# sttts/kcp

Hardware: AMD Instinct MI355X
Metric: object-pair diffs/sec (whole node) + achieved HBM GB/s, 10M objs/100k clusters (higher is better)
Workload: dtype u8; 1 GPU; config3: 10000000 pairs / 100000 logical clusters node-wide, 5% mutated (40% ConfigMap/Secret, 40% Deployment, 20% CRD); pairs_per_rank=10000000, passes_in_flight=2, parallelism=shard-by-logical-cluster x1 (LPT)

## Files before the change

include/gpudiff.h:

```cpp
#ifndef GPUDIFF_H
#define GPUDIFF_H

#include <stddef.h>
#include <stdint.h>

#include "gpudiff_format.h"

#ifdef __cplusplus
extern "C" {
#endif

#define GPUDIFF_ABI_VERSION 6

enum {
    GPUDIFF_OK = 0,
    GPUDIFF_E_INVAL = -1,
    GPUDIFF_E_NOMEM = -2,
    GPUDIFF_E_DEVICE = -3,
    GPUDIFF_E_NODEVICE = -4,
    GPUDIFF_E_CAPACITY = -5,
    GPUDIFF_E_STATE = -6,
    GPUDIFF_E_DECODE = -7,
    GPUDIFF_E_NOTFOUND = -8,
};

#define GPUDIFF_SPEC_DIRTY 0x1u
#define GPUDIFF_STATUS_DIRTY 0x2u
#define GPUDIFF_DECODE_ERROR 0x4u
#define GPUDIFF_SPEC_NOOP 0x8u
#define GPUDIFF_STATUS_NOOP 0x10u

#define GPUDIFF_TOK_OK 0
#define GPUDIFF_TOK_SYNTAX 1
#define GPUDIFF_TOK_NUMBER 2
#define GPUDIFF_TOK_KEY 3
#define GPUDIFF_TOK_STRING 4
#define GPUDIFF_TOK_HASH 5
#define GPUDIFF_TOK_DEPTH 6
#define GPUDIFF_TOK_SIZE 7
#define GPUDIFF_TOK_SPACE 8
#define GPUDIFF_TOK_FLOAT 9
#define GPUDIFF_TOK_WIDE 10
#define GPUDIFF_TOK_FIELD 11
#define GPUDIFF_TOK_LIST 12

#define GPUDIFF_PATH_CHANGED 0u
#define GPUDIFF_PATH_ADDED 1u
#define GPUDIFF_PATH_REMOVED 2u
#define GPUDIFF_PATH_STATUS_ABSENT 3u
#define GPUDIFF_PATH_REGION_STATUS 0x80u

#define GPUDIFF_OPT_TIMING 0x1u
#define GPUDIFF_OPT_K2_ROWS 0x40u
#define GPUDIFF_OPT_ARENA_SHIFT 21u
#define GPUDIFF_OPT_DEVICE_ENCODE 0x2000000u
#define GPUDIFF_OPT_PATH_STRINGS 0x8000000u
#define GPUDIFF_OPT_SMALL_PASS 0x20000000u
#define GPUDIFF_OPT_PATH_VALUES 0x80000000u
#define GPUDIFF_OPT_KNOWN                                                                                         \
    (GPUDIFF_OPT_TIMING | (0xFu << GPUDIFF_OPT_ARENA_SHIFT) | GPUDIFF_OPT_DEVICE_ENCODE | GPUDIFF_OPT_PATH_STRINGS | \
     GPUDIFF_OPT_SMALL_PASS | GPUDIFF_OPT_PATH_VALUES | GPUDIFF_OPT_K2_ROWS)

#define GPUDIFF_SMALL_PASS_MAX_PAIRS 4096u
#define GPUDIFF_SMALL_PASS_MAX_PATHS 32768u

#define GPUDIFF_DEVICE_CURRENT (-1)
#define GPUDIFF_DEVICE_NONE (-2)

typedef struct gpudiff_opts {
    int32_t device;
    uint32_t encode_threads;
    void* stream;
    uint32_t flags;
    uint32_t path_hash_bits;
} gpudiff_opts;

typedef struct gpudiff_json_pair {
    const uint8_t* old_json;
    size_t old_len;
    const uint8_t* new_json;
    size_t new_len;
    uint32_t pair_id;
    uint32_t cluster_id;
} gpudiff_json_pair;

typedef struct gpudiff_ctx gpudiff_ctx;
typedef struct gpudiff_hbatch gpudiff_hbatch;
typedef struct gpudiff_dbatch gpudiff_dbatch;
typedef uint64_t gpudiff_ticket;

typedef struct gpudiff_hbatch_info {
    size_t n_pairs;
    const gpudiff_pair_row* rows;
    const uint8_t* pool;
    uint64_t pool_bytes;
    uint64_t total_leaves;
    uint64_t n_decode_errors;
    uint64_t n_reseeded;
} gpudiff_hbatch_info;

typedef struct gpudiff_result {
    size_t n_pairs;
    const uint8_t* pair_flags;
    size_t n_spec_dirty;
    const uint32_t* spec_dirty_ids;
    size_t n_status_dirty;
    const uint32_t* status_dirty_ids;
    size_t n_dirty;
    const uint32_t* dirty_ids;
    const uint32_t* path_offsets;
    size_t n_paths;
    const uint64_t* path_hashes;
    const uint8_t* path_kinds;
    void* internal_;
} gpudiff_result;

typedef struct gpudiff_path_strings {
    size_t n_paths;
    const uint64_t* offsets;
    const char* bytes;
    size_t n_host;
    size_t n_unresolved;
} gpudiff_path_strings;
int gpudiff_result_path_strings(gpudiff_ctx* ctx, const gpudiff_result* res, gpudiff_path_strings* out);
typedef struct gpudiff_path_stats {
    uint64_t batches;
    uint64_t paths;
    uint64_t bytes;
    uint64_t host_paths;
    double kernel_ms;
    uint64_t timed_batches;
} gpudiff_path_stats;
int gpudiff_path_strings_stats_get(gpudiff_ctx* ctx, gpudiff_path_stats* out);

#define GPUDIFF_VALUE_ABSENT 0xFFu
typedef struct gpudiff_path_values {
    size_t n_paths;
    const uint64_t* offsets;
    const char* bytes;
    const uint8_t* tags;
    size_t n_host;
    size_t n_unresolved;
} gpudiff_path_values;
int gpudiff_result_path_values(gpudiff_ctx* ctx, const gpudiff_result* res, gpudiff_path_values* out);
int gpudiff_path_values_stats_get(gpudiff_ctx* ctx, gpudiff_path_stats* out);
int gpudiff_render_syncs_get(gpudiff_ctx* ctx, uint64_t* out);

typedef struct gpudiff_device_view {
    const uint8_t* pair_flags;
    const uint32_t* spec_dirty_ids;
    const uint32_t* status_dirty_ids;
    const uint32_t* dirty_ids;
    const uint32_t* counts;
} gpudiff_device_view;

typedef struct gpudiff_batch_stats {
    uint64_t n_pairs;
    uint64_t pool_bytes;
    uint64_t total_leaves;
    uint64_t compare_bytes;
    uint64_t value_bytes;
} gpudiff_batch_stats;

typedef struct gpudiff_timings {
    float compare_ms;
    float compact_ms;
    float join_ms;
    float emit_ms;
    float total_ms;
    uint32_t n_passes;
    uint32_t k2_launches;
} gpudiff_timings;

const char* gpudiff_strerror(int err);
int gpudiff_abi_version(void);
const char* gpudiff_build_id(void);
int gpudiff_device_count(int* n);

int gpudiff_open(const gpudiff_opts* opts, gpudiff_ctx** out);
void gpudiff_close(gpudiff_ctx* ctx);

int gpudiff_encode_pairs(gpudiff_ctx* ctx, const gpudiff_json_pair* pairs, size_t n,
                         gpudiff_hbatch** out);
int gpudiff_hbatch_info_get(const gpudiff_hbatch* hb, gpudiff_hbatch_info* info);
int gpudiff_hbatch_create(gpudiff_ctx* ctx, uint64_t pool_bytes, size_t n_pairs, uint64_t total_leaves,
                          gpudiff_hbatch** out, uint8_t** pool, gpudiff_pair_row** rows);
int gpudiff_hbatch_resize(gpudiff_ctx* ctx, gpudiff_hbatch* hb, uint64_t pool_bytes, size_t n_pairs,
                          uint64_t total_leaves, uint8_t** pool, gpudiff_pair_row** rows);
void gpudiff_hbatch_free(gpudiff_ctx* ctx, gpudiff_hbatch* hb);

int gpudiff_dbatch_create(gpudiff_ctx* ctx, uint64_t pool_bytes, uint64_t max_pairs,
                          gpudiff_dbatch** out);
int gpudiff_dbatch_create_view(gpudiff_ctx* ctx, const gpudiff_dbatch* base, gpudiff_dbatch** out);
int gpudiff_dbatch_append(gpudiff_ctx* ctx, gpudiff_dbatch* db, const gpudiff_hbatch* hb);
int gpudiff_dbatch_reset(gpudiff_ctx* ctx, gpudiff_dbatch* db);
int gpudiff_dbatch_stats_get(const gpudiff_dbatch* db, gpudiff_batch_stats* st);
int gpudiff_dbatch_device_view(const gpudiff_dbatch* db, gpudiff_device_view* v);
#define GPUDIFF_EXPORT_COUNTS 0u
#define GPUDIFF_EXPORT_SPEC_IDS 1u
#define GPUDIFF_EXPORT_STATUS_IDS 2u
#define GPUDIFF_EXPORT_DIRTY_IDS 3u
#define GPUDIFF_EXPORT_FLAGS 4u
int gpudiff_dbatch_export(gpudiff_ctx* ctx, const gpudiff_dbatch* db, uint32_t what, void* dst_device,
                          uint64_t max_elems, uint64_t known_count);
int gpudiff_dbatch_bind_gather(gpudiff_ctx* ctx, gpudiff_dbatch* db, void* send_dev, uint32_t cap_spec,
                               uint32_t cap_status);
int gpudiff_dbatch_result_slot(gpudiff_ctx* ctx, gpudiff_dbatch* db, uint32_t slot);
int gpudiff_dbatch_read_pool(gpudiff_ctx* ctx, const gpudiff_dbatch* db, uint64_t off, void* dst,
                             uint64_t bytes);
void gpudiff_dbatch_free(gpudiff_ctx* ctx, gpudiff_dbatch* db);

int gpudiff_cluster_bytes(const gpudiff_pair_row* rows, size_t n, uint32_t n_clusters, uint64_t* out);
int gpudiff_shard_lpt(const uint64_t* weights, uint32_t n_clusters, uint32_t world, int32_t* owner);
int gpudiff_rows_stream_bytes(const gpudiff_pair_row* rows, size_t n, uint64_t* out);
int gpudiff_rows_read_bytes(const gpudiff_pair_row* rows, size_t n, uint64_t* out);

int gpudiff_diff(gpudiff_ctx* ctx, gpudiff_dbatch* db, gpudiff_ticket* ticket);
int gpudiff_wait(gpudiff_ctx* ctx, gpudiff_ticket ticket, gpudiff_result* res);
void gpudiff_result_release(gpudiff_ctx* ctx, gpudiff_result* res);
int gpudiff_last_timings(gpudiff_ctx* ctx, gpudiff_timings* t);
int gpudiff_timing_reset(gpudiff_ctx* ctx);
int gpudiff_sync(gpudiff_ctx* ctx);
typedef struct gpudiff_pass_stats {
    uint64_t passes;
    uint64_t small_passes;
    uint64_t small_redone;
    uint64_t redo_arena, redo_deep, redo_paths;
    uint64_t readback_rounds;
} gpudiff_pass_stats;
int gpudiff_pass_stats_get(gpudiff_ctx* ctx, gpudiff_pass_stats* out);

int gpudiff_submit(gpudiff_ctx* ctx, const gpudiff_json_pair* pairs, size_t n,
                   gpudiff_ticket* ticket);

typedef struct gpudiff_cluster_index {
    size_t n_clusters;
    const uint32_t* cluster_ids;
    const uint32_t* spec_off;
    const uint32_t* status_off;
    size_t n_spec, n_status;
    const uint32_t* spec_ids;
    const uint32_t* status_ids;
    uint32_t sorted_on_device;
    void* internal;
} gpudiff_cluster_index;
int gpudiff_cluster_index_get(gpudiff_ctx* ctx, gpudiff_ticket ticket, gpudiff_cluster_index* out);
void gpudiff_cluster_index_release(gpudiff_ctx* ctx, gpudiff_cluster_index* idx);
int gpudiff_cluster_index_host(const uint8_t* flags, const uint32_t* pair_ids, const uint32_t* cluster_ids, size_t n,
                               gpudiff_cluster_index* out);
typedef struct gpudiff_cluster_index_stats {
    uint64_t calls;
    uint64_t sorted_calls;
    uint64_t syncs;
    uint64_t entries;
    uint64_t d2h_bytes;
    double kernel_ms;
    uint64_t timed_calls;
} gpudiff_cluster_index_stats;
int gpudiff_cluster_index_stats_get(gpudiff_ctx* ctx, gpudiff_cluster_index_stats* out);
int gpudiff_cluster_index_get_final(gpudiff_ctx* ctx, gpudiff_ticket ticket, gpudiff_cluster_index* out);
typedef struct gpudiff_cluster_index_final_stats {
    uint64_t calls;
    uint64_t patched_calls;
    uint64_t compacted_calls;
    uint64_t sorted_calls;
    uint64_t syncs;
    uint64_t entries_in;
    uint64_t entries_live;
    uint64_t patch_rows;
    uint64_t h2d_bytes;
    uint64_t d2h_bytes;
    double kernel_ms;
    uint64_t timed_calls;
} gpudiff_cluster_index_final_stats;
int gpudiff_cluster_index_final_stats_get(gpudiff_ctx* ctx, gpudiff_cluster_index_final_stats* out);

typedef struct gpudiff_store gpudiff_store;

typedef struct gpudiff_event {
    uint32_t slot;
    uint32_t pair_id;
    uint32_t cluster_id;
    uint32_t reserved;
    const uint8_t* new_json;
    size_t new_len;
    const uint8_t* old_json;
    size_t old_len;
} gpudiff_event;

typedef struct gpudiff_store_stats {
    uint64_t max_slots, live_slots;
    uint64_t space_bytes;
    uint64_t used_bytes;
    uint64_t live_bytes;
    uint64_t compactions;
    uint64_t events, old_encoded, reseeded, collisions_unresolved;
    uint64_t last_batch_bytes;
    uint64_t deferred;
// ... 246 lines not shown
```

include/gpudiff_format.h:

```cpp
#ifndef GPUDIFF_FORMAT_H
#define GPUDIFF_FORMAT_H

#include <stdint.h>

#ifdef __HIPCC__
#define GPUDIFF_HD __host__ __device__
#else
#define GPUDIFF_HD
#endif

#define GPUDIFF_TAG_NULL 0u
#define GPUDIFF_TAG_FALSE 1u
#define GPUDIFF_TAG_TRUE 2u
#define GPUDIFF_TAG_INT 3u
#define GPUDIFF_TAG_FLOAT 4u
#define GPUDIFF_TAG_STR 5u
#define GPUDIFF_TAG_EOBJ 6u
#define GPUDIFF_TAG_EARR 7u

#define GPUDIFF_INLINE_MAX 8u
#define GPUDIFF_PATH_HASH_BITS 32u

#define GPUDIFF_OBJ_HAS_STATUS 0x1u
#define GPUDIFF_OBJ_DECODE_ERR 0x2u
#define GPUDIFF_OBJ_FRESH 0x4u
#define GPUDIFF_OBJ_SPEC_KEYS_EQ 0x8u
#define GPUDIFF_OBJ_SPEC_SHAPE_EQ 0x10u
#define GPUDIFF_TAB_INDEX 0x8000000000000000ull
#define GPUDIFF_TAB_NONE 0xFFFFFFFFu
GPUDIFF_HD static inline uint64_t gpudiff_tab_bytes(uint32_t n, uint64_t key_bytes) {
    return (24ull * n + key_bytes + 127u) & ~(uint64_t)127u;
}

#define GPUDIFF_OBJ_SEED_SHIFT 8u

#ifdef __cplusplus
extern "C" {
#endif

typedef struct gpudiff_pair_row {
    uint64_t off_a;
    uint64_t off_b;
    uint32_t spec_l_a, spec_l_b;
    uint32_t spec_ar_a, spec_ar_b;
    uint32_t stat_l_a, stat_l_b;
    uint32_t stat_ar_a, stat_ar_b;
    uint32_t flags_a, flags_b;
    uint32_t pair_id, cluster_id;
} gpudiff_pair_row;

GPUDIFF_HD static inline uint64_t gpudiff_seg_bytes(uint32_t l, uint32_t arena) {
    return (uint64_t)l * 16u + (uint64_t)arena;
}

#define GPUDIFF_BLOB_ALIGN 128u
GPUDIFF_HD static inline uint64_t gpudiff_blob_body(uint32_t sl, uint32_t sar, uint32_t tl, uint32_t tar) {
    return (gpudiff_seg_bytes(sl, sar) + gpudiff_seg_bytes(tl, tar) + (GPUDIFF_BLOB_ALIGN - 1u)) &
           ~(uint64_t)(GPUDIFF_BLOB_ALIGN - 1u);
}

#ifndef GPUDIFF_KEYS_HOLE_UNIT
#define GPUDIFF_KEYS_HOLE_UNIT 128u
#endif
GPUDIFF_HD static inline void gpudiff_keys_hole(uint32_t l, uint32_t* hs, uint32_t* hl) {
    const uint64_t u = GPUDIFF_KEYS_HOLE_UNIT;
    const uint64_t lo = (8ull * l + (u - 1u)) / u * u, hi = 12ull * l / u * u;
    *hs = hi > lo ? (uint32_t)(lo >> 4) : 0u;
    *hl = hi > lo ? (uint32_t)((hi - lo) >> 4) : 0u;
}
GPUDIFF_HD static inline void gpudiff_shape_hole(uint32_t l, uint32_t* hs, uint32_t* hl) {
    const uint64_t u = GPUDIFF_KEYS_HOLE_UNIT;
    const uint64_t lo = (8ull * l + (u - 1u)) / u * u, hi = 16ull * l / u * u;
    *hs = hi > lo ? (uint32_t)(lo >> 4) : 0u;
    *hl = hi > lo ? (uint32_t)((hi - lo) >> 4) : 0u;
}
GPUDIFF_HD static inline uint32_t gpudiff_hole_chunk(uint32_t k, uint32_t hs, uint32_t hl) {
    return k + (k >= hs ? hl : 0u);
}

GPUDIFF_HD static inline uint64_t gpudiff_pair_compare_bytes(const gpudiff_pair_row* r) {
    const uint64_t al = GPUDIFF_BLOB_ALIGN - 1u;
    uint64_t per = 0;
    if ((r->flags_a | r->flags_b) & GPUDIFF_OBJ_DECODE_ERR) return sizeof(gpudiff_pair_row) + 1u;
    {
        const int spec_sz = r->spec_l_a == r->spec_l_b && r->spec_ar_a == r->spec_ar_b;
        const int stat_sz = (r->flags_b & GPUDIFF_OBJ_HAS_STATUS) && r->stat_l_a == r->stat_l_b &&
                            r->stat_ar_a == r->stat_ar_b;
        const uint64_t seg_s = gpudiff_seg_bytes(r->spec_l_a, r->spec_ar_a);
        const uint64_t seg_t = gpudiff_seg_bytes(r->stat_l_a, r->stat_ar_a);
        if (spec_sz && stat_sz) per = (seg_s + seg_t + al) & ~al;
        else if (spec_sz) per = (r->stat_l_a | r->stat_l_b | r->stat_ar_a | r->stat_ar_b) ? seg_s : (seg_s + al) & ~al;
        else if (stat_sz) per = seg_t;
    }
    return sizeof(gpudiff_pair_row) + 1u + 2u * per;
}

#define GPUDIFF_PD_ERR 0x01u
#define GPUDIFF_PD_SPEC_EQ 0x02u
#define GPUDIFF_PD_STAT_EQ 0x04u
#define GPUDIFF_PD_HAS_ST_B 0x08u
#define GPUDIFF_PD_HAS_ST_A 0x10u
#define GPUDIFF_PD_SEED 0x20u
#define GPUDIFF_PD_NO_STAT 0x40u
#define GPUDIFF_PD_SIZE_BITS 19u
#define GPUDIFF_PD_SIZE_MAX 0x7FFFFu
#define GPUDIFF_PD_ESCAPE 0xFFFFFFFFu
#define GPUDIFF_PD_SHAPE_L 0x40000u

typedef struct gpudiff_pair_desc {
    uint32_t w[4];
} gpudiff_pair_desc;

typedef struct gpudiff_pair_geom {
    uint64_t off_a, off_b;
    uint32_t n1, n2, adj_a, adj_b;
    uint32_t bits;
    uint32_t hs, hl;
} gpudiff_pair_geom;

GPUDIFF_HD static inline gpudiff_pair_geom gpudiff_pair_geom_of(uint64_t off_a, uint64_t off_b, uint32_t seg_a,
                                                                uint32_t seg_b, uint32_t seg_t, uint32_t bits,
                                                                uint32_t skip_l, int shape) {
    gpudiff_pair_geom g;
    const int ok = !(bits & GPUDIFF_PD_ERR);
    const int spec_sz = (bits & GPUDIFF_PD_SPEC_EQ) != 0u;
    const int stat_sz = (bits & GPUDIFF_PD_HAS_ST_B) && (bits & GPUDIFF_PD_STAT_EQ);
    const uint32_t r128 = (seg_a + seg_t + 127u) & ~127u;
    g.off_a = off_a;
    g.off_b = off_b;
    g.n1 = (ok && spec_sz) ? ((!stat_sz && (bits & GPUDIFF_PD_NO_STAT)) ? ((seg_a + 127u) & ~127u) : seg_a) >> 4 : 0u;
    g.n2 = (ok && stat_sz) ? (spec_sz ? r128 - seg_a : seg_t) >> 4 : 0u;
    g.hs = g.hl = 0u;
    if (skip_l && (uint64_t)skip_l * (shape ? 16u : 12u) <= 16ull * g.n1) {
        if (shape) gpudiff_shape_hole(skip_l, &g.hs, &g.hl);
        else gpudiff_keys_hole(skip_l, &g.hs, &g.hl);
        g.n1 -= g.hl;
    }
    g.adj_a = seg_a - 16u * g.n1;
    g.adj_b = seg_b - 16u * g.n1;
    g.bits = bits;
    return g;
}

GPUDIFF_HD static inline uint32_t gpudiff_pair_row_bits(const gpudiff_pair_row* r) {
    return (((r->flags_a | r->flags_b) & GPUDIFF_OBJ_DECODE_ERR) ? GPUDIFF_PD_ERR : 0u) |
           ((r->spec_l_a == r->spec_l_b && r->spec_ar_a == r->spec_ar_b) ? GPUDIFF_PD_SPEC_EQ : 0u) |
           ((r->stat_l_a == r->stat_l_b && r->stat_ar_a == r->stat_ar_b) ? GPUDIFF_PD_STAT_EQ : 0u) |
           ((r->flags_b & GPUDIFF_OBJ_HAS_STATUS) ? GPUDIFF_PD_HAS_ST_B : 0u) |
           ((r->flags_a & GPUDIFF_OBJ_HAS_STATUS) ? GPUDIFF_PD_HAS_ST_A : 0u) |
           (((r->flags_a >> GPUDIFF_OBJ_SEED_SHIFT) & 0xFFu) ? GPUDIFF_PD_SEED : 0u) |
           ((r->stat_l_a | r->stat_l_b | r->stat_ar_a | r->stat_ar_b) == 0u ? GPUDIFF_PD_NO_STAT : 0u);
}

GPUDIFF_HD static inline gpudiff_pair_geom gpudiff_pair_row_geom(const gpudiff_pair_row* r) {
    return gpudiff_pair_geom_of(r->off_a, r->off_b, (uint32_t)gpudiff_seg_bytes(r->spec_l_a, r->spec_ar_a),
                                (uint32_t)gpudiff_seg_bytes(r->spec_l_b, r->spec_ar_b),
                                (uint32_t)gpudiff_seg_bytes(r->stat_l_a, r->stat_ar_a), gpudiff_pair_row_bits(r), 0u, 0);
}

GPUDIFF_HD static inline gpudiff_pair_desc gpudiff_pair_desc_pack(const gpudiff_pair_row* r) {
    gpudiff_pair_desc d;
    const uint64_t sa = gpudiff_seg_bytes(r->spec_l_a, r->spec_ar_a), sb = gpudiff_seg_bytes(r->spec_l_b, r->spec_ar_b);
    const uint64_t st = gpudiff_seg_bytes(r->stat_l_a, r->stat_ar_a);
    const uint32_t bits = gpudiff_pair_row_bits(r);
    const uint64_t size_max = (uint64_t)GPUDIFF_PD_SIZE_MAX << 4;
    const int fits = ((r->off_a | r->off_b) & (GPUDIFF_BLOB_ALIGN - 1u)) == 0u && (r->off_a >> 7) <= 0xFFFFFFFFull &&
                     (r->off_b >> 7) <= 0xFFFFFFFFull && ((sa | sb | st) & 15u) == 0u && sa <= size_max &&
                     sb <= size_max && st <= size_max &&
                     ((uint32_t)(r->stat_l_a + r->stat_l_b) == 0u) == ((bits & GPUDIFF_PD_NO_STAT) != 0u);
    if (!fits) {
        d.w[0] = d.w[1] = d.w[2] = d.w[3] = GPUDIFF_PD_ESCAPE;
        return d;
    }
    {
        uint64_t f1 = sb >> 4;
        if (bits & GPUDIFF_PD_SPEC_EQ) {
            uint32_t hs = 0, hl = 0;
            const int keys = (r->flags_b & GPUDIFF_OBJ_SPEC_KEYS_EQ) && !(bits & GPUDIFF_PD_ERR);
            f1 = 0u;
            if (keys && (r->flags_b & GPUDIFF_OBJ_SPEC_SHAPE_EQ) && (sa >> 4) < GPUDIFF_PD_SHAPE_L) {
                gpudiff_shape_hole(r->spec_l_a, &hs, &hl);
                if (hl) f1 = r->spec_l_a | GPUDIFF_PD_SHAPE_L;
            }
            if (keys && !f1) {
                gpudiff_keys_hole(r->spec_l_a, &hs, &hl);
                f1 = hl ? r->spec_l_a : 0u;
            }
        }
        const uint64_t zw = (sa >> 4) | (f1 << GPUDIFF_PD_SIZE_BITS) | ((st >> 4) << (2u * GPUDIFF_PD_SIZE_BITS)) |
                            ((uint64_t)bits << (3u * GPUDIFF_PD_SIZE_BITS));
        d.w[0] = (uint32_t)(r->off_a >> 7);
        d.w[1] = (uint32_t)(r->off_b >> 7);
        d.w[2] = (uint32_t)zw;
        d.w[3] = (uint32_t)(zw >> 32);
    }
    return d;
}

GPUDIFF_HD static inline int gpudiff_pair_desc_is_escape(uint32_t w3) { return w3 == GPUDIFF_PD_ESCAPE; }

GPUDIFF_HD static inline gpudiff_pair_geom gpudiff_pair_desc_unpack(uint32_t w0, uint32_t w1, uint32_t w2, uint32_t w3) {
    const uint64_t zw = ((uint64_t)w3 << 32) | w2;
    const uint32_t bits = w3 >> (3u * GPUDIFF_PD_SIZE_BITS - 32u);
    const uint32_t seg_a = (w2 & GPUDIFF_PD_SIZE_MAX) << 4;
    const uint32_t f1 = (uint32_t)(zw >> GPUDIFF_PD_SIZE_BITS) & GPUDIFF_PD_SIZE_MAX;
    const int eq = (bits & GPUDIFF_PD_SPEC_EQ) != 0u;
    const int shape = eq && f1 >= GPUDIFF_PD_SHAPE_L && (w2 & GPUDIFF_PD_SIZE_MAX) < GPUDIFF_PD_SHAPE_L;
    return gpudiff_pair_geom_of((uint64_t)w0 << 7, (uint64_t)w1 << 7, seg_a, eq ? seg_a : f1 << 4,
                                ((w3 >> (2u * GPUDIFF_PD_SIZE_BITS - 32u)) & GPUDIFF_PD_SIZE_MAX) << 4, bits,
                                eq ? (shape ? f1 & (GPUDIFF_PD_SHAPE_L - 1u) : f1) : 0u, shape);
}

GPUDIFF_HD static inline uint64_t gpudiff_pair_stream_bytes(const gpudiff_pair_row* r) {
    const gpudiff_pair_desc d = gpudiff_pair_desc_pack(r);
    const gpudiff_pair_geom g = gpudiff_pair_desc_is_escape(d.w[3]) ? gpudiff_pair_row_geom(r)
                                                                   : gpudiff_pair_desc_unpack(d.w[0], d.w[1], d.w[2], d.w[3]);
    return sizeof(gpudiff_pair_desc) + 32ull * ((uint64_t)g.n1 + g.n2);
}

GPUDIFF_HD static inline uint32_t gpudiff_meta(uint32_t tag, uint32_t len) { return (len << 3) | tag; }
GPUDIFF_HD static inline uint32_t gpudiff_meta_tag(uint32_t m) { return m & 7u; }
GPUDIFF_HD static inline uint32_t gpudiff_meta_len(uint32_t m) { return m >> 3; }
GPUDIFF_HD static inline int gpudiff_meta_is_long(uint32_t m) {
    return gpudiff_meta_tag(m) == GPUDIFF_TAG_STR && gpudiff_meta_len(m) > GPUDIFF_INLINE_MAX;
}
GPUDIFF_HD static inline uint32_t gpudiff_meta_arena(uint32_t m) {
    return gpudiff_meta_is_long(m) ? ((gpudiff_meta_len(m) - GPUDIFF_INLINE_MAX + 3u) & ~3u) : 0u;
}
GPUDIFF_HD static inline uint32_t gpudiff_arena_bytes(uint32_t sum) { return (sum + 15u) & ~15u; }

#ifdef __cplusplus
}
#endif
#endif
```

integration/go/gpudiff/gpudiff.go:

```go
package gpudiff

import "C"

import (
	"bytes"
	"encoding/json"
	"errors"
	"fmt"
	"math"
	"sort"
	"strconv"
	"sync"
	"time"
	"unicode/utf8"
	"unsafe"

	"k8s.io/apimachinery/pkg/apis/meta/v1/unstructured"
)

type Engine struct {
	mu     sync.Mutex
	ctx    *C.gpudiff_ctx
	devEnc bool
}
// ... 809 lines not shown
	lp := (*[1 << 30]C.size_t)(lens)[:n:n]
	for i, o := range objs {
		dp[i], lp[i] = nil, 0
		if b, ok := jsonOf(o); ok {
			dp[i], lp[i] = cmem(b)
		}
	}
	defer func() {
		for i := range dp {
			C.free(unsafe.Pointer(dp[i]))
		}
	}()
	e.mu.Lock()
	defer e.mu.Unlock()
	var out C.gpudiff_bodies
	if err := errOf(C.gpudiff_upsert_bodies(e.ctx, (**C.uint8_t)(docs), (*C.size_t)(lens), C.size_t(n),
		C.uint32_t(mode), &out)); err != nil {
		return nil, nil, nil, err
	}
	defer C.gpudiff_bodies_release(e.ctx, &out)
	var rv C.gpudiff_rv_splice
	if err := errOf(C.gpudiff_bodies_rv_splice(e.ctx, &out, &rv)); err != nil {
		return nil, nil, nil, err
	}
	offs := (*[1 << 30]C.uint64_t)(unsafe.Pointer(out.offsets))[: n+1 : n+1]
	st := (*[1 << 30]C.int32_t)(unsafe.Pointer(out.status))[:n:n]
	res := make([][]byte, n)
	rvOff, rvForm = make([]uint32, n), make([]uint8, n)
	ro := (*[1 << 30]C.uint32_t)(unsafe.Pointer(rv.off))[:n:n]
	rf := (*[1 << 30]C.uint8_t)(unsafe.Pointer(rv.form))[:n:n]
	for i := 0; i < n; i++ {
		if lp[i] == 0 || st[i] != 0 {
			continue
		}
		res[i] = C.GoBytes(unsafe.Pointer(uintptr(unsafe.Pointer(out.bytes))+uintptr(offs[i])),
			C.int(offs[i+1]-offs[i]))
		rvOff[i], rvForm[i] = uint32(ro[i]), uint8(rf[i])
	}
	return res, rvOff, rvForm, nil
}

const (
	RVNone   = uint8(C.GPUDIFF_RV_NONE)
	RVInsert = uint8(C.GPUDIFF_RV_INSERT)
	RVLead   = uint8(C.GPUDIFF_RV_LEAD)
	RVTrail  = uint8(C.GPUDIFF_RV_TRAIL)
	RVWrap   = uint8(C.GPUDIFF_RV_WRAP)
)

func SpliceRV(body []byte, off uint32, form uint8, rv string) []byte {
	if rv == "" || form&RVInsert == 0 || off == 0 || int(off) >= len(body) {
		return body
	}
	val, err := json.Marshal(rv)
	if err != nil {
		return body
	}
	out := make([]byte, 0, len(body)+len(val)+40)
	out = append(out, body[:off]...)
	if form&RVLead != 0 {
		out = append(out, ',')
	}
	if form&RVWrap != 0 {
		out = append(out, `"metadata":{`...)
	}
	out = append(out, `"resourceVersion":`...)
	out = append(out, val...)
	if form&RVWrap != 0 {
		out = append(out, '}')
	}
	if form&RVTrail != 0 {
		out = append(out, ',')
	}
	return append(out, body[off:]...)
}

const OptDeviceEncode = uint32(C.GPUDIFF_OPT_DEVICE_ENCODE)

const OptSmallPass = uint32(C.GPUDIFF_OPT_SMALL_PASS)

const (
	ObjSpecKeysEq  = uint32(C.GPUDIFF_OBJ_SPEC_KEYS_EQ)
	ObjSpecShapeEq = uint32(C.GPUDIFF_OBJ_SPEC_SHAPE_EQ)
)

func RowsReadBytes(rows unsafe.Pointer, n int) (uint64, error) {
	var out C.uint64_t
	if err := errOf(C.gpudiff_rows_read_bytes((*C.gpudiff_pair_row)(rows), C.size_t(n), &out)); err != nil {
		return 0, err
	}
	return uint64(out), nil
}

type Write struct {
	Pair int
	Kind Mode
	Noop bool
	Body []byte
	RVOff  uint32
	RVForm uint8
	Name      string
	Namespace string
}

const (
	PlanInformer           = uint32(C.GPUDIFF_PLAN_INFORMER)
	PlanSpec               = uint32(C.GPUDIFF_PLAN_SPEC)
	PlanStatus             = uint32(C.GPUDIFF_PLAN_STATUS)
	PlanUpstreamDownstream = uint32(C.GPUDIFF_PLAN_UPSTREAM_DOWNSTREAM)
	PlanTargets            = uint32(C.GPUDIFF_PLAN_TARGETS)
)

func (e *Engine) DiffAndPlan(olds, news [][]byte) ([]uint8, []Write, error) {
	return e.DiffAndPlanMode(olds, news, PlanInformer)
}

func (e *Engine) DiffAndPlanMode(olds, news [][]byte, mode uint32) ([]uint8, []Write, error) {
	n := len(olds)
	if len(news) != n {
		return nil, nil, errOf(C.GPUDIFF_E_INVAL)
	}
	if n == 0 {
		return nil, nil, nil
	}
	pairs := (*[1 << 28]C.gpudiff_json_pair)(C.malloc(C.size_t(n) * C.size_t(unsafe.Sizeof(C.gpudiff_json_pair{}))))[:n:n]
	defer C.free(unsafe.Pointer(&pairs[0]))
	for i := range olds {
		pa, la := cmem(olds[i])
		pb, lb := cmem(news[i])
		pairs[i] = C.gpudiff_json_pair{old_json: pa, old_len: la, new_json: pb, new_len: lb, pair_id: C.uint32_t(i)}
	}
	defer func() {
		for i := range pairs {
			C.free(unsafe.Pointer(pairs[i].old_json))
			C.free(unsafe.Pointer(pairs[i].new_json))
		}
	}()
	e.mu.Lock()
	defer e.mu.Unlock()
	var ticket C.gpudiff_ticket
	if err := errOf(C.gpudiff_submit(e.ctx, &pairs[0], C.size_t(n), &ticket)); err != nil {
		return nil, nil, err
	}
	var res C.gpudiff_result
	if err := errOf(C.gpudiff_wait(e.ctx, ticket, &res)); err != nil {
		return nil, nil, err
	}
	flags := make([]uint8, n)
	copy(flags, (*[1 << 30]uint8)(unsafe.Pointer(res.pair_flags))[:n:n])
	C.gpudiff_result_release(e.ctx, &res)
	var plan C.gpudiff_write_plan
	if err := errOf(C.gpudiff_write_plan_get_ex(e.ctx, ticket, C.uint32_t(mode), &plan)); err != nil {
		return flags, nil, err
	}
	defer C.gpudiff_write_plan_release(e.ctx, &plan)
	return flags, writesOf(&plan), nil
}

func writesOf(plan *C.gpudiff_write_plan) []Write {
	m := int(plan.n)
	writes := make([]Write, m)
	if m == 0 {
		return writes
	}
	idx := (*[1 << 30]C.uint32_t)(unsafe.Pointer(plan.pair_index))[:m:m]
	kind := (*[1 << 30]C.uint8_t)(unsafe.Pointer(plan.kind))[:m:m]
	noop := (*[1 << 30]C.uint8_t)(unsafe.Pointer(plan.noop))[:m:m]
// ... 215 lines not shown
```

kcp_amd/csrc/api.cpp:

```cpp
#include <hip/hip_runtime.h>
#include <stdlib.h>
#include <string.h>

#include <algorithm>
#include <array>
#include <atomic>
#include <memory>
#include <mutex>
#include <new>
#include <string>
#include <thread>
#include <unordered_map>
#include <vector>

#include "../../include/gpudiff.h"
#include "encoder.h"
#include "dstore.h"
#include "engine.h"
#include "kernels.h"
#include "small_pass.h"
#include "xxh64.h"

using namespace gd;

namespace gd {
thread_local std::string g_last_hip_error;
}
using gd::g_last_hip_error;

static int ensure_paths(gpudiff_dbatch* d, uint64_t arena, uint64_t scratch) {
    const bool ok_a = arena <= d->arena_cap && d->arena_h;
    const bool ok_s = scratch <= d->scratch_cap && d->scratch_h;
    if (ok_a && ok_s) return GPUDIFF_OK;
    auto drop = [](auto*& p) {
        if (p) (void)hipFree(p);
        p = nullptr;
    };
    drop(d->out_h);
    drop(d->out_k);
    int rc;
    if (!ok_a) {
        drop(d->arena_h);
        drop(d->arena_k);
        d->arena_cap = 0;
        if ((rc = dalloc(&d->arena_h, arena)) || (rc = dalloc(&d->arena_k, arena))) return rc;
        d->arena_cap = arena;
    }
    if (!ok_s) {
        if (scratch > kMaxScratchEntries) return GPUDIFF_E_CAPACITY;
        scratch = std::min<uint64_t>(std::max<uint64_t>({scratch + scratch / 8, d->scratch_cap, 1u << 16}),
                                     kMaxScratchEntries);
        scratch = (scratch + kJoinSliceHost - 1) / kJoinSliceHost * kJoinSliceHost;
        drop(d->scratch_h);
        drop(d->scratch_k);
        drop(d->slot_owner);
        drop(d->slice_cnt);
        drop(d->slice_weq);
        d->scratch_cap = 0;
        const uint64_t slots = scratch / kJoinSliceHost;
        if ((rc = dalloc(&d->scratch_h, scratch)) || (rc = dalloc(&d->scratch_k, scratch)) ||
            (rc = dalloc(&d->slot_owner, slots)) || (rc = dalloc(&d->slice_cnt, slots)) ||
            (rc = dalloc(&d->slice_weq, slots)))
            return rc;
        d->scratch_cap = scratch;
    }
    const uint64_t out = d->arena_cap + d->scratch_cap;
    if ((rc = dalloc(&d->out_h, out)) || (rc = dalloc(&d->out_k, out))) return rc;
    return GPUDIFF_OK;
}

static DiffBuffers buffers_of(gpudiff_ctx* c, gpudiff_dbatch* d) {
    DiffBuffers b;
    b.rows = d->rows;
    b.desc = (d->desc_gen == d->rows_gen && !(c->flags & GPUDIFF_OPT_K2_ROWS)) ? d->desc : nullptr;
    b.pool = d->pool;
    b.pair_ids = d->pair_ids;
    b.n_pairs = (uint32_t)d->n_pairs;
    b.flags = d->flags;
    b.caps = d->caps;
    b.chunk_counts = d->chunk_counts;
    b.summary = d->summary;
    b.spec_ids = d->spec_ids;
    b.status_ids = d->status_ids;
    b.dirty_ids = d->dirty_ids;
    b.dirty_idx = d->dirty_idx;
    b.scratch_off = d->scratch_off;
    b.path_count = d->path_count;
    b.path_off = d->path_off;
    b.tile_sums = d->tile_sums;
    b.path_src = d->path_src;
    b.path_cnt = d->path_cnt;
    b.nbits = d->nbits;
    b.noop_d = d->noop_d;
    b.arena_h = d->arena_h;
    b.arena_k = d->arena_k;
    b.arena_per_wave = kArenaPerWave >> ((c->flags >> GPUDIFF_OPT_ARENA_SHIFT) & 0xFu);
    b.scratch_h = d->scratch_h;
    b.scratch_k = d->scratch_k;
    b.scratch_cap = d->scratch_cap;
    b.out_h = d->out_h;
    b.out_k = d->out_k;
    b.slot_owner = d->slot_owner;
    b.slice_cnt = d->slice_cnt;
    b.slice_weq = d->slice_weq;
    b.hash_mask = c->hash_mask;
    b.k2_timeline = c->k2_timeline ? 1u : 0u;
    b.k2_shared = 0u;
    b.tail_perm = d->tail_perm;
    b.tail_perm_key = &d->tail_perm_key;
    b.rows_gen = d->rows_gen;
    b.gather_send = d->gather_send;
    b.gather_cap_spec = d->gather_cap_spec;
    b.gather_cap_status = d->gather_cap_status;
    b.avg_pair_bytes = d->n_pairs ? (d->compare_bytes ? d->compare_bytes : d->size_hint_bytes) / d->n_pairs : 0;
    return b;
}


extern "C" {

const char* gpudiff_strerror(int err) {
    switch (err) {
        case GPUDIFF_OK: return "ok";
        case GPUDIFF_E_INVAL: return "invalid argument";
        case GPUDIFF_E_NOMEM: return "out of host memory";
        case GPUDIFF_E_DEVICE: return g_last_hip_error.empty() ? "HIP runtime error" : g_last_hip_error.c_str();
        case GPUDIFF_E_NODEVICE: return "no GPU in this context (there is no CPU fallback)";
        case GPUDIFF_E_CAPACITY: return "device batch capacity exceeded";
        case GPUDIFF_E_STATE: return "invalid call order / unknown ticket";
        case GPUDIFF_E_DECODE: return "input failed to decode as a JSON object";
        case GPUDIFF_E_NOTFOUND: return "path hash not found";
        default: return "unknown error";
    }
}

int gpudiff_abi_version(void) { return GPUDIFF_ABI_VERSION; }

int gpudiff_device_count(int* n) {
    if (!n) return GPUDIFF_E_INVAL;
    *n = 0;
    int c = 0;
    if (hipGetDeviceCount(&c) != hipSuccess) return GPUDIFF_OK;
    *n = c;
    return GPUDIFF_OK;
}

int gpudiff_open(const gpudiff_opts* opts, gpudiff_ctx** out) {
    if (!out) return GPUDIFF_E_INVAL;
    *out = nullptr;
    gpudiff_opts o{};
    o.device = GPUDIFF_DEVICE_CURRENT;
    if (opts) o = *opts;
    if (o.flags & ~GPUDIFF_OPT_KNOWN) return GPUDIFF_E_INVAL;
    std::unique_ptr<gpudiff_ctx> c(new (std::nothrow) gpudiff_ctx());
    if (!c) return GPUDIFF_E_NOMEM;
    uint32_t hw = std::max(1u, std::thread::hardware_concurrency());
    c->threads = o.encode_threads ? o.encode_threads : std::min(hw, 16u);
    c->flags = o.flags;
// ... 182 lines not shown
int gpudiff_hbatch_info_get(const gpudiff_hbatch* hb, gpudiff_hbatch_info* info) {
    if (!hb || !info) return GPUDIFF_E_INVAL;
    info->n_pairs = hb->n;
    info->rows = hb->rows;
    info->pool = hb->pool;
    info->pool_bytes = hb->pool_bytes;
    info->total_leaves = hb->leaves;
    info->n_decode_errors = hb->errors;
    info->n_reseeded = hb->reseeded;
    return GPUDIFF_OK;
}

void gpudiff_hbatch_free(gpudiff_ctx* c, gpudiff_hbatch* hb) {
    if (!hb) return;
    if (c && c->has_device) (void)hipSetDevice(c->device);
    if (hb->used) {
        (void)hipEventSynchronize(hb->used);
        (void)hipEventDestroy(hb->used);
    }
    hb_release_buffers(hb);
    delete hb;
}

static int alloc_outputs(gpudiff_dbatch* d);

int gpudiff_dbatch_create(gpudiff_ctx* c, uint64_t pool_bytes, uint64_t max_pairs, gpudiff_dbatch** out) {
    if (!c || !out) return GPUDIFF_E_INVAL;
    *out = nullptr;
    int rc = set_device(c);
    if (rc) return rc;
    if (max_pairs > 0xFFFFFFF0ull) return GPUDIFF_E_INVAL;
    std::unique_ptr<gpudiff_dbatch> d(new (std::nothrow) gpudiff_dbatch());
    if (!d) return GPUDIFF_E_NOMEM;
    d->pool_cap = (pool_bytes + 15) & ~15ull;
    d->max_pairs = max_pairs;
    d->device = c->device;
    const uint64_t np = std::max<uint64_t>(max_pairs, 1);
    if ((rc = dalloc(&d->pool, d->pool_cap)) || (rc = dalloc(&d->rows, np)) || (rc = dalloc(&d->pair_ids, np)) ||
        (rc = dalloc(&d->desc, np)) || (rc = alloc_outputs(d.get()))) {
        dfree_all(d.get());
        return rc;
    }
    *out = d.release();
    return GPUDIFF_OK;
}

int gpudiff_dbatch_create_view(gpudiff_ctx* c, const gpudiff_dbatch* base, gpudiff_dbatch** out) {
    if (!c || !base || !out || base->base) return GPUDIFF_E_INVAL;
    *out = nullptr;
    int rc = set_device(c);
    if (rc) return rc;
    if (base->device != c->device) return GPUDIFF_E_INVAL;
    std::unique_ptr<gpudiff_dbatch> d(new (std::nothrow) gpudiff_dbatch());
    if (!d) return GPUDIFF_E_NOMEM;
    d->base = base;
    d->pool_borrowed = true;
    d->max_pairs = base->max_pairs;
    d->device = c->device;
    if ((rc = alloc_outputs(d.get()))) {
        dfree_all(d.get());
        return rc;
    }
    base->views.push_back(d.get());
    *out = d.release();
    return GPUDIFF_OK;
}

static void view_sync(gpudiff_dbatch* d) {
    if (!d->base) return;
    const gpudiff_dbatch* b = d->base;
    d->pool = b->pool;
    d->pool_cap = b->pool_cap;
    d->pool_used = b->pool_used;
    d->rows = b->rows;
    d->pair_ids = b->pair_ids;
    d->n_pairs = b->n_pairs;
    d->leaves = b->leaves;
    d->compare_bytes = b->compare_bytes;
    d->value_bytes = b->value_bytes;
    d->size_hint_bytes = b->size_hint_bytes;
    d->rows_gen = b->rows_gen;
    d->desc = b->desc;
    d->desc_gen = b->desc_gen;
}

static int alloc_outputs(gpudiff_dbatch* d) {
    int rc;
    const uint64_t np = std::max<uint64_t>(d->max_pairs, 1);
    const uint64_t nchunks = (np + 63) / 64;
    const uint64_t ntiles = 4 * (np / 4096 + 2);
    uint4* cc = nullptr;
    if ((rc = dalloc(&d->flags, np)) || (rc = dalloc(&d->caps, np)) || (rc = dalloc(&cc, nchunks)) ||
        (rc = dalloc(&d->summary, kSummaryWords)) || (rc = dalloc(&d->spec_ids, np)) || (rc = dalloc(&d->status_ids, np)) ||
        (rc = dalloc(&d->dirty_ids, np)) || (rc = dalloc(&d->dirty_idx, np)) || (rc = dalloc(&d->scratch_off, np)) ||
        (rc = dalloc(&d->path_count, np)) || (rc = dalloc(&d->path_off, np + 1)) ||
        (rc = dalloc(&d->path_src, np)) || (rc = dalloc(&d->path_cnt, np)) || (rc = dalloc(&d->nbits, np)) ||
        (rc = dalloc(&d->noop_d, np)) ||
        (rc = dalloc(&d->tile_sums, ntiles)) ||
        (rc = dalloc(&d->tail_perm, 16384))) {
        d->chunk_counts = cc;
        return rc;
    }
    d->chunk_counts = cc;
    if (hipEventCreateWithFlags(&d->done, hipEventDisableTiming) != hipSuccess) return GPUDIFF_E_DEVICE;
    return GPUDIFF_OK;
}

int gpudiff_dbatch_append(gpudiff_ctx* c, gpudiff_dbatch* d, const gpudiff_hbatch* hb) {
    if (!c || !d || !hb || d->base) return GPUDIFF_E_INVAL;
    int rc = set_device(c);
    if (rc) return rc;
    if (d->pool_used + hb->pool_bytes > d->pool_cap || d->n_pairs + hb->n > d->max_pairs) return GPUDIFF_E_CAPACITY;
    if (hb->n == 0) return GPUDIFF_OK;
    const uint64_t base = d->pool_used;
    const uint32_t begin = (uint32_t)d->n_pairs, end = (uint32_t)(d->n_pairs + hb->n);
    if (hb->pool_bytes)
        HIPCHK(hipMemcpyAsync(d->pool + base, hb->pool, hb->pool_bytes, hipMemcpyHostToDevice, c->stream));
    HIPCHK(hipMemcpyAsync(d->rows + begin, hb->rows, hb->n * sizeof(gpudiff_pair_row), hipMemcpyHostToDevice,
                          c->stream));
    if (hb->used) HIPCHK(hipEventRecord(hb->used, c->stream));
    HIPCHK(launch_rebase(c->stream, d->rows, begin, end, base, d->pair_ids, d->desc));
    uint64_t cb = 0, vb = 0;
    for (size_t i = 0; i < hb->n; i++) {
        const gpudiff_pair_row& r = hb->rows[i];
        cb += pair_compare_bytes(r);
        if ((r.flags_a | r.flags_b) & GPUDIFF_OBJ_DECODE_ERR) continue;
        vb += blob_value_bytes(hb->pool + r.off_a, r.spec_l_a, r.spec_ar_a, r.stat_l_a) +
              blob_value_bytes(hb->pool + r.off_b, r.spec_l_b, r.spec_ar_b, r.stat_l_b);
    }
    d->compare_bytes += cb;
    d->value_bytes += vb;
    d->pool_used += hb->pool_bytes;
    d->n_pairs = end;
    const bool desc_current = begin == 0 || d->desc_gen == d->rows_gen;
    d->rows_gen++;
    d->desc_gen = desc_current ? d->rows_gen : ~0ull;
    d->leaves += hb->leaves;
    return GPUDIFF_OK;
}

int gpudiff_dbatch_reset(gpudiff_ctx* c, gpudiff_dbatch* d) {
    if (!c || !d || d->base) return GPUDIFF_E_INVAL;
    int rc = set_device(c);
    if (rc) return rc;
    HIPCHK(hipStreamSynchronize(c->stream));
    d->pool_used = d->n_pairs = d->leaves = d->compare_bytes = d->value_bytes = d->size_hint_bytes = 0;
    d->ticket = 0;
    d->rows_gen++;
    return GPUDIFF_OK;
}

int gpudiff_dbatch_stats_get(const gpudiff_dbatch* d, gpudiff_batch_stats* st) {
    if (!d || !st) return GPUDIFF_E_INVAL;
    if (d->base) d = d->base;
    st->n_pairs = d->n_pairs;
    st->pool_bytes = d->pool_used;
    st->total_leaves = d->leaves;
    st->compare_bytes = d->compare_bytes;
    st->value_bytes = d->value_bytes;
    return GPUDIFF_OK;
}

int gpudiff_dbatch_device_view(const gpudiff_dbatch* d, gpudiff_device_view* v) {
    if (!d || !v) return GPUDIFF_E_INVAL;
    v->pair_flags = d->flags;
    v->spec_dirty_ids = d->spec_ids;
    v->status_dirty_ids = d->status_ids;
    v->dirty_ids = d->dirty_ids;
    v->counts = d->summary;
    return GPUDIFF_OK;
}

int gpudiff_dbatch_export(gpudiff_ctx* c, const gpudiff_dbatch* d, uint32_t what, void* dst, uint64_t max_elems,
                          uint64_t known_count) {
    if (!c || !d || (!dst && max_elems)) return GPUDIFF_E_INVAL;
    int rc = set_device(c);
    if (rc) return rc;
    const void* src;
    size_t esz = 4;
    uint64_t n = std::min<uint64_t>(max_elems, known_count);
    switch (what) {
        case GPUDIFF_EXPORT_COUNTS: src = d->summary; n = std::min<uint64_t>(max_elems, 8); break;
        case GPUDIFF_EXPORT_SPEC_IDS: src = d->spec_ids; break;
        case GPUDIFF_EXPORT_STATUS_IDS: src = d->status_ids; break;
        case GPUDIFF_EXPORT_DIRTY_IDS: src = d->dirty_ids; break;
        case GPUDIFF_EXPORT_FLAGS: src = d->flags; esz = 1; break;
        default: return GPUDIFF_E_INVAL;
    }
    if (what != GPUDIFF_EXPORT_COUNTS && n > d->n_pairs) n = d->n_pairs;
    if (n) HIPCHK(hipMemcpyAsync(dst, src, n * esz, hipMemcpyDeviceToDevice, c->stream));
    return GPUDIFF_OK;
}

int gpudiff_dbatch_bind_gather(gpudiff_ctx* c, gpudiff_dbatch* d, void* send_dev, uint32_t cap_spec,
                               uint32_t cap_status) {
    if (!c || !d) return GPUDIFF_E_INVAL;
    int rc = set_device(c);
    if (rc) return rc;
    const bool fresh = send_dev && send_dev != (void*)d->gather_send;
    d->gather_send = (uint32_t*)send_dev;
    d->gather_cap_spec = send_dev ? cap_spec : 0;
    d->gather_cap_status = send_dev ? cap_status : 0;
    if (fresh) HIPCHK(hipMemsetAsync((uint32_t*)send_dev + 4, 0, 4 * sizeof(uint32_t), c->stream));
    return GPUDIFF_OK;
}

int gpudiff_dbatch_result_slot(gpudiff_ctx* c, gpudiff_dbatch* d, uint32_t slot) {
    if (!c || !d || slot > 1) return GPUDIFF_E_INVAL;
    int rc = set_device(c);
    if (rc) return rc;
    if (slot == d->res_slot) return GPUDIFF_OK;
    if (!d->summary_alt) {
        const uint64_t np = std::max<uint64_t>(d->max_pairs, 1);
        uint32_t *a = nullptr, *b = nullptr, *sm = nullptr;
        if ((rc = dalloc(&a, np)) || (rc = dalloc(&b, np)) || (rc = dalloc(&sm, kSummaryWords))) {
            for (uint32_t* p : {a, b, sm})
                if (p) (void)hipFree(p);
            return rc;
        }
        if (hipMemset(sm, 0, kSummaryWords * sizeof(uint32_t)) != hipSuccess) {
            for (uint32_t* p : {a, b, sm}) (void)hipFree(p);
            return GPUDIFF_E_DEVICE;
        }
        d->ids_alt[0] = a, d->ids_alt[1] = b, d->summary_alt = sm;
    }
    std::swap(d->spec_ids, d->ids_alt[0]);
    std::swap(d->status_ids, d->ids_alt[1]);
    std::swap(d->summary, d->summary_alt);
    d->res_slot = slot;
    return GPUDIFF_OK;
}

int gpudiff_dbatch_read_pool(gpudiff_ctx* c, const gpudiff_dbatch* d, uint64_t off, void* dst, uint64_t bytes) {
    if (!c || !d || (!dst && bytes)) return GPUDIFF_E_INVAL;
    if (d->base) d = d->base;
    int rc = set_device(c);
    if (rc) return rc;
    if (off > d->pool_used || bytes > d->pool_used - off) return GPUDIFF_E_INVAL;
    HIPCHK(hipStreamSynchronize(c->stream));
    if (bytes) HIPCHK(hipMemcpy(dst, d->pool + off, bytes, hipMemcpyDeviceToHost));
    return GPUDIFF_OK;
}

int gpudiff_cluster_bytes(const gpudiff_pair_row* rows, size_t n, uint32_t n_clusters, uint64_t* out) {
    if ((n && !rows) || (n_clusters && !out)) return GPUDIFF_E_INVAL;
    for (size_t i = 0; i < n; i++)
        if (rows[i].cluster_id >= n_clusters) return GPUDIFF_E_INVAL;
    for (size_t i = 0; i < n; i++) out[rows[i].cluster_id] += gpudiff_pair_compare_bytes(&rows[i]);
    return GPUDIFF_OK;
}

int gpudiff_rows_stream_bytes(const gpudiff_pair_row* rows, size_t n, uint64_t* out) {
    if ((n && !rows) || !out) return GPUDIFF_E_INVAL;
    uint64_t sum = 0;
    for (size_t i = 0; i < n; i++) {
        gpudiff_pair_row r = rows[i];
        r.flags_b &= ~GPUDIFF_OBJ_SPEC_SHAPE_EQ;
        sum += gpudiff_pair_stream_bytes(&r);
    }
    *out = sum;
    return GPUDIFF_OK;
}

int gpudiff_rows_read_bytes(const gpudiff_pair_row* rows, size_t n, uint64_t* out) {
    if ((n && !rows) || !out) return GPUDIFF_E_INVAL;
    uint64_t sum = 0;
    for (size_t i = 0; i < n; i++) sum += gpudiff_pair_stream_bytes(&rows[i]);
    *out = sum;
    return GPUDIFF_OK;
}

int gpudiff_shard_lpt(const uint64_t* weights, uint32_t n_clusters, uint32_t world, int32_t* owner) {
    if (world == 0 || world > 0x7FFFFFFFu || (n_clusters && (!weights || !owner))) return GPUDIFF_E_INVAL;
    try {
        std::vector<uint32_t> order(n_clusters);
        for (uint32_t c = 0; c < n_clusters; c++) order[c] = c;
        std::sort(order.begin(), order.end(), [&](uint32_t x, uint32_t y) {
            return weights[x] != weights[y] ? weights[x] > weights[y] : x < y;
        });
        std::vector<std::pair<uint64_t, uint32_t>> heap;
        heap.reserve(world);
        for (uint32_t r = 0; r < world; r++) heap.emplace_back(0, r);
        auto gt = [](const std::pair<uint64_t, uint32_t>& a, const std::pair<uint64_t, uint32_t>& b) { return a > b; };
        std::make_heap(heap.begin(), heap.end(), gt);
        for (uint32_t c : order) {
            std::pop_heap(heap.begin(), heap.end(), gt);
            auto& top = heap.back();
            owner[c] = (int32_t)top.second;
            top.first += weights[c];
            std::push_heap(heap.begin(), heap.end(), gt);
        }
    } catch (const std::bad_alloc&) {
        return GPUDIFF_E_NOMEM;
    }
    return GPUDIFF_OK;
}

void gpudiff_dbatch_free(gpudiff_ctx* c, gpudiff_dbatch* d) {
    if (!d) return;
    if (d->base) {
        auto& v = d->base->views;
        v.erase(std::remove(v.begin(), v.end(), d), v.end());
    }
    if (c && c->has_device) {
        (void)hipSetDevice(c->device);
        (void)hipStreamSynchronize(c->stream);
        if (d->ticket) c->tickets.erase(d->ticket);
    }
    dfree_all(d);
    delete d;
}

static hipEvent_t* pass_events(gpudiff_ctx* c) {
    if (c->n_pass >= c->pass_ev.size()) {
        std::array<hipEvent_t, 5> a{};
        for (auto& e : a)
            if (hipEventCreate(&e) != hipSuccess) return nullptr;
        c->pass_ev.push_back(a);
    }
    return c->pass_ev[c->n_pass].data();
}

static int enqueue_join_emit(gpudiff_ctx* c, gpudiff_dbatch* d) {
    DiffBuffers b = buffers_of(c, d);
    const uint32_t nchunks = (uint32_t)((d->n_pairs + 63) / 64);
    HIPCHK(launch_slot_owners(c->stream, b));
    HIPCHK(launch_join(c->stream, b, 0, nchunks, nullptr, (const uint4*)d->summary));
    HIPCHK(launch_emit(c->stream, b));
    return GPUDIFF_OK;
}

static int enqueue_ordinary_pass(gpudiff_ctx* c, gpudiff_dbatch* d, const DiffBuffers& b, hipEvent_t* ev) {
    hipStream_t ms = c->stream;
    uint4* total = (uint4*)d->summary;
    const uint32_t nchunks = (uint32_t)((d->n_pairs + 63) / 64);
    HIPCHK(launch_compare(ms, b));
    if (ev) HIPCHK(hipEventRecord(ev[1], ms));
    HIPCHK(launch_compact(ms, b, 0, nchunks, nullptr, total));
    if (ev) HIPCHK(hipEventRecord(ev[2], ms));
    HIPCHK(launch_join(ms, b, 0, nchunks, nullptr, total));
    if (ev) HIPCHK(hipEventRecord(ev[3], ms));
    HIPCHK(launch_emit(ms, b));
// ... 293 lines not shown
    (void)c;
    if (!res || !out) return GPUDIFF_E_INVAL;
    memset(out, 0, sizeof(*out));
    const ResultStore* rs = (const ResultStore*)res->internal_;
    if (!rs || !rs->ps.on) return GPUDIFF_E_STATE;
    out->n_paths = rs->ps.n;
    out->offsets = rs->ps.offsets();
    out->bytes = rs->ps.bytes();
    out->n_host = rs->ps.n_host;
    out->n_unresolved = rs->ps.n_unresolved;
    return GPUDIFF_OK;
}

int gpudiff_path_strings_stats_get(gpudiff_ctx* c, gpudiff_path_stats* out) {
    if (!c || !out) return GPUDIFF_E_INVAL;
    if (!(c->flags & GPUDIFF_OPT_PATH_STRINGS)) return GPUDIFF_E_STATE;
    *out = c->path_stats;
    return GPUDIFF_OK;
}

int gpudiff_result_path_values(gpudiff_ctx* c, const gpudiff_result* res, gpudiff_path_values* out) {
    (void)c;
    if (!res || !out) return GPUDIFF_E_INVAL;
    memset(out, 0, sizeof(*out));
    const ResultStore* rs = (const ResultStore*)res->internal_;
    if (!rs || !rs->pv.on) return GPUDIFF_E_STATE;
    out->n_paths = rs->pv.n;
    out->offsets = rs->pv.offsets();
    out->bytes = rs->pv.bytes();
    out->tags = rs->pv.tags();
    out->n_host = rs->pv.n_host;
    out->n_unresolved = rs->pv.n_unresolved;
    return GPUDIFF_OK;
}

int gpudiff_path_values_stats_get(gpudiff_ctx* c, gpudiff_path_stats* out) {
    if (!c || !out) return GPUDIFF_E_INVAL;
    *out = c->value_stats;
    return GPUDIFF_OK;
}

int gpudiff_render_syncs_get(gpudiff_ctx* c, uint64_t* out) {
    if (!c || !out) return GPUDIFF_E_INVAL;
    *out = c->render_syncs;
    return GPUDIFF_OK;
}

void gpudiff_result_release(gpudiff_ctx* c, gpudiff_result* res) {
    (void)c;
    if (!res) return;
    delete (ResultStore*)res->internal_;
    memset(res, 0, sizeof(*res));
}

int gpudiff_submit(gpudiff_ctx* c, const gpudiff_json_pair* pairs, size_t n, gpudiff_ticket* ticket) {
    if (!c || (n && !pairs)) return GPUDIFF_E_INVAL;
    int rc = set_device(c);
    if (rc) return rc;
    if ((c->flags & GPUDIFF_OPT_DEVICE_ENCODE) && n) {
        rc = dstore_submit_pairs(c, pairs, n, ticket);
        if (rc != GPUDIFF_E_CAPACITY) return rc;
    }
    gpudiff_hbatch* hb = nullptr;
    if ((rc = gpudiff_encode_pairs(c, pairs, n, &hb))) return rc;
    const uint32_t slot = c->ring_next;
    c->ring_next ^= 1u;
    gpudiff_dbatch*& d = c->ring[slot];
    if (d) HIPCHK(hipEventSynchronize(d->done));
    if (c->ring_hb[slot]) {
        gpudiff_hbatch_free(c, c->ring_hb[slot]);
        c->ring_hb[slot] = nullptr;
    }
    if (d && (d->pool_cap < hb->pool_bytes || d->max_pairs < n)) {
        gpudiff_dbatch_free(c, d);
        d = nullptr;
    }
    if (!d) {
        uint64_t pool = std::max<uint64_t>(hb->pool_bytes * 2, 1u << 20);
        uint64_t np = std::max<uint64_t>(n * 2, 1024);
        if ((rc = gpudiff_dbatch_create(c, pool, np, &d))) {
            gpudiff_hbatch_free(c, hb);
            return rc;
        }
    }
    d->pool_used = d->n_pairs = d->leaves = d->compare_bytes = d->value_bytes = d->size_hint_bytes = 0;
    if ((rc = gpudiff_dbatch_append(c, d, hb)) || (rc = gpudiff_diff(c, d, ticket))) {
        gpudiff_hbatch_free(c, hb);
        return rc;
    }
    c->ring_hb[slot] = hb;
    return GPUDIFF_OK;
}

static int single_pair(gpudiff_ctx* c, const uint8_t* a, size_t al, const uint8_t* b, size_t bl, uint32_t bit,
                       int* equal) {
    if (!c || !equal || !a || !b) return GPUDIFF_E_INVAL;
    gpudiff_json_pair p{a, al, b, bl, 0, 0};
    gpudiff_ticket t = 0;
    int rc = gpudiff_submit(c, &p, 1, &t);
    if (rc) return rc;
    gpudiff_result r;
    if ((rc = gpudiff_wait(c, t, &r))) return rc;
    const uint8_t f = r.pair_flags[0];
    gpudiff_result_release(c, &r);
    *equal = (f & bit) ? 0 : 1;
    return (f & GPUDIFF_DECODE_ERROR) ? GPUDIFF_E_DECODE : GPUDIFF_OK;
}

int gpudiff_spec_equal(gpudiff_ctx* c, const uint8_t* a, size_t al, const uint8_t* b, size_t bl, int* equal) {
    return single_pair(c, a, al, b, bl, GPUDIFF_SPEC_DIRTY, equal);
}

int gpudiff_status_equal(gpudiff_ctx* c, const uint8_t* a, size_t al, const uint8_t* b, size_t bl, int* equal) {
    return single_pair(c, a, al, b, bl, GPUDIFF_STATUS_DIRTY, equal);
}

int gpudiff_resolve_path(const uint8_t* a, size_t al, const uint8_t* b, size_t bl, uint64_t h, uint8_t kind,
                         uint32_t bits, char* buf, size_t cap, size_t* out_len) {
    if (!a || !b) return GPUDIFF_E_INVAL;
    EncodeConfig cfg;
    cfg.hash_bits = (bits == 0 || bits >= GPUDIFF_PATH_HASH_BITS) ? GPUDIFF_PATH_HASH_BITS : bits;
    PairEncoder enc(cfg);
    std::vector<uint8_t> pool;
    gpudiff_pair_row row;
    enc.encode_json(a, al, b, bl, 0, 0, pool, row);
    if (row.flags_a & GPUDIFF_OBJ_DECODE_ERR) return GPUDIFF_E_DECODE;
    std::string s;
    bool found = false;
    const bool status = (kind & GPUDIFF_PATH_REGION_STATUS) != 0;
    if ((kind & 3u) != GPUDIFF_PATH_STATUS_ABSENT) {
        for (const FlatObject* o : {&enc.flat_a, &enc.flat_b}) {
            const std::vector<LeafRec>& v = status ? o->stat : o->spec;
            auto it = std::lower_bound(v.begin(), v.end(), h, [](const LeafRec& r, uint64_t x) { return r.h < x; });
            if (it != v.end() && it->h == h) {
                s = render_path(o->paths.data() + it->path_off, it->path_len);
                found = true;
                break;
            }
        }
    } else {
        const uint64_t mask = cfg.hash_bits >= 64 ? ~0ULL : ((1ULL << cfg.hash_bits) - 1);
        const uint32_t seed = (row.flags_a >> GPUDIFF_OBJ_SEED_SHIFT) & 0xFF;
        const std::string& sp = status_path_bytes();
        if ((chain_hash(sp.data(), sp.size(), seed) & mask) == h) {
            s = "status";
            found = true;
        }
    }
    if (!found) return GPUDIFF_E_NOTFOUND;
    if (out_len) *out_len = s.size();
    if (buf && cap) {
        size_t k = std::min(cap - 1, s.size());
        memcpy(buf, s.data(), k);
        buf[k] = 0;
    }
    return GPUDIFF_OK;
}

}
```

kcp_amd/csrc/encoder.cpp:

```cpp
#include "encoder.h"

#include <string.h>

#include <algorithm>

#include "xxh64.h"

namespace gd {

static const Node* find_member(const Node& obj, const char* key, uint32_t klen) {
    if (obj.t != J_OBJ) return nullptr;
    for (uint32_t i = 0; i < obj.n; i++) {
        const Member& m = obj.u.mem[i];
        if (m.klen == klen && memcmp(m.k, key, klen) == 0) return &m.v;
    }
    return nullptr;
}

static inline void push_key(std::string& p, const char* k, uint32_t n) {
    char hdr[5];
    hdr[0] = 0x01;
    memcpy(hdr + 1, &n, 4);
    p.append(hdr, 5);
    p.append(k, n);
// ... 183 lines not shown
    const uint64_t hs = chain_hash(sp.data(), sp.size(), seed) & mask;
    return sentinel_check(a, a.stat, hs) && sentinel_check(b, b.stat, hs);
}

bool PairEncoder::assign_seed(FlatObject& a, FlatObject& b, uint32_t* seed_out) {
    for (uint32_t seed = 0; seed <= 255; seed++)
        if (pair_valid(a, b, seed)) {
            *seed_out = seed;
            return true;
        }
    return false;
}

static inline void pool_align(std::vector<uint8_t>& pool) {
    size_t n = (pool.size() + GPUDIFF_BLOB_ALIGN - 1) & ~(size_t)(GPUDIFF_BLOB_ALIGN - 1);
    pool.resize(n, 0);
}

void PairEncoder::write_blob(const FlatObject& o, std::vector<uint8_t>& pool, uint64_t* off, uint32_t* sl,
                             uint32_t* sar, uint32_t* tl, uint32_t* tar) {
    pool_align(pool);
    *off = pool.size();
    auto seg = [&](const std::vector<LeafRec>& v, uint32_t* L, uint32_t* AR) {
        const size_t n = v.size();
        uint32_t arena = 0;
        for (const LeafRec& r : v)
            arena += gpudiff_meta_arena(r.meta);
        arena = gpudiff_arena_bytes(arena);
        const size_t head = n * 16;
        const size_t base = pool.size();
        pool.resize(base + head + arena, 0);
        uint8_t* p = pool.data() + base;
        uint8_t* vals = p;
        uint8_t* keys = p + 8 * n;
        uint8_t* metas = p + 12 * n;
        uint8_t* ar = p + head;
        uint32_t aoff = 0;
        for (size_t i = 0; i < n; i++) {
            const LeafRec& r = v[i];
            uint64_t val = r.val;
            if (gpudiff_meta_is_long(r.meta)) {
                memcpy(&val, r.vptr, GPUDIFF_INLINE_MAX);
                memcpy(ar + aoff, r.vptr + GPUDIFF_INLINE_MAX, r.vlen - GPUDIFF_INLINE_MAX);
                aoff += gpudiff_meta_arena(r.meta);
            }
            const uint32_t k32 = (uint32_t)r.h;
            memcpy(keys + 4 * i, &k32, 4);
            memcpy(vals + 8 * i, &val, 8);
            memcpy(metas + 4 * i, &r.meta, 4);
        }
        *L = (uint32_t)n;
        *AR = arena;
        leaves_written += n;
    };
    seg(o.spec, sl, sar);
    seg(o.stat, tl, tar);
    pool_align(pool);
}

void PairEncoder::encode_flat(FlatObject* fa, FlatObject* fb, uint32_t pair_id, uint32_t cluster_id,
                              std::vector<uint8_t>& pool, gpudiff_pair_row& row) {
    memset(&row, 0, sizeof(row));
    row.pair_id = pair_id;
    row.cluster_id = cluster_id;
    uint32_t seed = 0;
    if (!fa || !fb || !assign_seed(*fa, *fb, &seed)) {
        decode_errors++;
        pool_align(pool);
        row.off_a = row.off_b = pool.size();
        row.flags_a = row.flags_b = GPUDIFF_OBJ_DECODE_ERR;
        return;
    }
    if (seed) reseeded++;
    write_blob(*fa, pool, &row.off_a, &row.spec_l_a, &row.spec_ar_a, &row.stat_l_a, &row.stat_ar_a);
    write_blob(*fb, pool, &row.off_b, &row.spec_l_b, &row.spec_ar_b, &row.stat_l_b, &row.stat_ar_b);
    row.flags_a = fa->flags | (seed << GPUDIFF_OBJ_SEED_SHIFT);
    row.flags_b = fb->flags | (seed << GPUDIFF_OBJ_SEED_SHIFT);
    bool keys_eq = fa->spec.size() == fb->spec.size();
    for (size_t i = 0; keys_eq && i < fa->spec.size(); i++) keys_eq = (uint32_t)fa->spec[i].h == (uint32_t)fb->spec[i].h;
    if (keys_eq) row.flags_b |= GPUDIFF_OBJ_SPEC_KEYS_EQ;
    bool shape_eq = keys_eq;
    for (size_t i = 0; shape_eq && i < fa->spec.size(); i++) shape_eq = fa->spec[i].meta == fb->spec[i].meta;
    if (shape_eq) row.flags_b |= GPUDIFF_OBJ_SPEC_SHAPE_EQ;
}

void PairEncoder::encode_nodes(const Node* a, const Node* b, uint32_t pair_id, uint32_t cluster_id,
                               std::vector<uint8_t>& pool, gpudiff_pair_row& row) {
    FlatObject* fa = nullptr;
    FlatObject* fb = nullptr;
    if (a && b) {
        flatten_object(*a, flat_a);
        flatten_object(*b, flat_b);
        fa = &flat_a;
        fb = &flat_b;
    }
    encode_flat(fa, fb, pair_id, cluster_id, pool, row);
}

void PairEncoder::encode_json(const uint8_t* a, size_t alen, const uint8_t* b, size_t blen, uint32_t pair_id,
                              uint32_t cluster_id, std::vector<uint8_t>& pool, gpudiff_pair_row& row) {
    arena_a.reset();
    arena_b.reset();
    Node na, nb;
    bool oka = a && parser.parse_object(a, alen, arena_a, &na) && !decodes_as_list(na);
    bool okb = oka && b && parser.parse_object(b, blen, arena_b, &nb) && !decodes_as_list(nb);
    encode_nodes(oka ? &na : nullptr, okb ? &nb : nullptr, pair_id, cluster_id, pool, row);
}


bool PairEncoder::flatten_json(const uint8_t* json, size_t len, Arena& arena, FlatObject& o) {
    arena.reset();
    Node n;
    if (!json || !parser.parse_object(json, len, arena, &n) || decodes_as_list(n)) return false;
    flatten_object(n, o);
    return true;
}

bool PairEncoder::path_table(FlatObject& o, uint32_t seed) {
    using PN = TabNode;
    const uint64_t mask = cfg_.hash_bits >= 64 ? ~0ULL : ((1ULL << cfg_.hash_bits) - 1);
    const uint64_t root = (uint64_t)seed & mask;
    std::vector<PN>& v = tab_scratch_;
    v.clear();
    const char* P = o.paths.data();
    for (const std::vector<LeafRec>* lv : {&o.spec, &o.stat})
        for (const LeafRec& r : *lv) {
            uint64_t hp = seed;
            uint32_t i = 0;
            while (i + 5 <= r.path_len) {
                const char* c = P + r.path_off + i;
                uint32_t x;
                memcpy(&x, c + 1, 4);
                const bool key = c[0] == 0x01;
                const uint32_t len = key ? 5u + x : 5u;
                const uint64_t h = xxh64_host(c, len, hp);
                PN n;
                n.h = h & mask;
                n.ph = hp & mask;
                n.c = key ? ((uint64_t)x << 32) : (GPUDIFF_TAB_INDEX | x);
                n.poff = r.path_off;
                n.pend = r.path_off + i + len;
                n.koff = r.path_off + i + 5;
                if (n.h == root) {
                    o.tab.n = GPUDIFF_TAB_NONE;
                    o.tab.data.clear();
                    return false;
                }
                v.push_back(n);
                hp = h;
                i += len;
            }
        }
    std::sort(v.begin(), v.end(), [](const PN& a, const PN& b) { return a.h < b.h; });
    size_t u = 0, kb = 0;
    for (size_t i = 0; i < v.size(); i++) {
        if (u && v[u - 1].h == v[i].h) {
            const PN& a = v[u - 1];
            const PN& b = v[i];
            if (a.pend - a.poff != b.pend - b.poff || memcmp(P + a.poff, P + b.poff, a.pend - a.poff) != 0) {
                o.tab.n = GPUDIFF_TAB_NONE;
                o.tab.data.clear();
                return false;
            }
            continue;
        }
        v[u++] = v[i];
// ... 169 lines not shown
```

kcp_amd/csrc/engine.h:

```cpp
#pragma once
#include <hip/hip_runtime.h>
#include <string.h>

#include <algorithm>
#include <array>
#include <functional>
#include <memory>
#include <string>
#include <unordered_map>
#include <vector>

#include "../../include/gpudiff.h"
#include "encoder.h"
#include "pool.h"
#include "kernels.h"

using gd::PairEncoder;
using gd::EncodeConfig;

namespace gd {
extern thread_local std::string g_last_hip_error;
}

#define HIPCHK(x)                                             \
// ... 11 lines not shown
    std::vector<gpudiff_pair_row> rows;
    uint64_t leaves = 0, errors = 0, reseeded = 0;
};
}

inline constexpr uint32_t kArenaPerWave = 16384;

struct gpudiff_hbatch {
    uint8_t* pool = nullptr;
    gpudiff_pair_row* rows = nullptr;
    size_t n = 0;
    uint64_t pool_bytes = 0;
    uint64_t leaves = 0, errors = 0, reseeded = 0;
    uint64_t pool_cap = 0;
    size_t rows_cap = 0;
    bool pinned = false;
    hipEvent_t used = nullptr;
};

struct WaitedMark {
    gpudiff_ticket ticket = 0;
    uint32_t n_spec = 0, n_status = 0, n_dirty = 0;
    uint32_t n_dev_dirty = 0;
};
namespace gd {
struct PlanPatch;
}
struct FanBuffers;
void fan_buffers_release(FanBuffers* f);
struct FanCtx;
void fan_ctx_release(FanCtx* f);

struct gpudiff_dbatch {
    uint64_t pool_cap = 0, pool_used = 0;
    uint64_t max_pairs = 0, n_pairs = 0;
    uint64_t leaves = 0, compare_bytes = 0, value_bytes = 0;
    uint64_t size_hint_bytes = 0;
    uint8_t* pool = nullptr;
    bool pool_borrowed = false;
    gpudiff_pair_row* rows = nullptr;
    uint32_t* pair_ids = nullptr;
    uint8_t* flags = nullptr;
    uint32_t* caps = nullptr;
    void* chunk_counts = nullptr;
    uint32_t* summary = nullptr;
    uint32_t* spec_ids = nullptr;
    uint32_t* status_ids = nullptr;
    uint32_t* dirty_ids = nullptr;
    uint32_t* dirty_idx = nullptr;
    uint32_t* scratch_off = nullptr;
    uint32_t* path_count = nullptr;
    uint32_t* path_off = nullptr;
    uint32_t* tile_sums = nullptr;
    uint32_t* path_src = nullptr;
    uint32_t* path_cnt = nullptr;
    uint8_t* nbits = nullptr;
    uint8_t* noop_d = nullptr;
    uint64_t arena_cap = 0;
    uint64_t* arena_h = nullptr;
    uint8_t* arena_k = nullptr;
    uint64_t scratch_cap = 0;
    uint64_t* scratch_h = nullptr;
    uint8_t* scratch_k = nullptr;
    uint32_t* slot_owner = nullptr;
    uint32_t* slice_cnt = nullptr;
    uint8_t* slice_weq = nullptr;
    uint64_t* out_h = nullptr;
    uint8_t* out_k = nullptr;
    hipEvent_t done = nullptr;
    gpudiff_ticket ticket = 0;
    uint32_t* gather_send = nullptr;
    uint32_t gather_cap_spec = 0, gather_cap_status = 0;
    uint32_t* ids_alt[2] = {nullptr, nullptr};
    uint32_t* summary_alt = nullptr;
    uint32_t res_slot = 0;
    const gpudiff_dbatch* base = nullptr;
    mutable std::vector<gpudiff_dbatch*> views;
    int device = -1;
    uint32_t* tail_perm = nullptr;
    gd::TailPermKey tail_perm_key;
    uint64_t rows_gen = 0;
    uint4* desc = nullptr;
    uint64_t desc_gen = ~0ull;
    uint8_t* small_image = nullptr;
    bool small_pending = false;
    WaitedMark waited;
    FanBuffers* fan = nullptr;
    bool host_resolves = false;
    const std::vector<gd::PlanPatch>* final_patch = nullptr;
};

struct DStore;

struct PathStrs {
    bool on = false;
    size_t n = 0;
    std::vector<uint64_t> words;
    size_t n_host = 0, n_unresolved = 0;
    const uint64_t* offsets() const { return words.data(); }
    const char* bytes() const { return (const char*)(words.data() + n + 1); }
    void begin() {
        words.assign(1, 0);
        tail.clear();
        n = 0;
    }
    void push(const char* p, size_t len) {
        tail.append(p, len);
        words.push_back(tail.size());
        n++;
    }
    void finish() {
        const size_t w = (tail.size() + 7) / 8;
        words.resize(n + 1 + w, 0);
        if (!tail.empty()) memcpy(words.data() + n + 1, tail.data(), tail.size());
        tail.clear();
        tail.shrink_to_fit();
    }
    std::string tail;
};

struct PathVals {
    bool on = false;
    size_t n = 0;
    std::vector<uint64_t> words;
    size_t n_host = 0, n_unresolved = 0;
    static size_t tag_words(size_t n) { return (2 * n + 7) / 8; }
    const uint64_t* offsets() const { return words.data(); }
    const uint8_t* tags() const { return (const uint8_t*)(words.data() + 2 * n + 1); }
    const char* bytes() const { return (const char*)(words.data() + 2 * n + 1 + tag_words(n)); }
    void begin() {
        offs.assign(1, 0);
        tg.clear();
        tail.clear();
        n = 0;
    }
    void push(uint8_t tag, const char* p, size_t len) {
        tail.append(p, len);
        offs.push_back(tail.size());
        tg.push_back(tag);
    }
    void finish() {
        n = tg.size() / 2;
        words.assign(2 * n + 1 + tag_words(n) + (tail.size() + 7) / 8, 0);
        memcpy(words.data(), offs.data(), offs.size() * 8);
        if (!tg.empty()) memcpy(words.data() + 2 * n + 1, tg.data(), tg.size());
        if (!tail.empty()) memcpy(words.data() + 2 * n + 1 + tag_words(n), tail.data(), tail.size());
        offs = {};
        tg = {};
        tail = {};
    }
    std::vector<uint64_t> offs;
    std::vector<uint8_t> tg;
    std::string tail;
};

struct ResultStore {
    std::vector<uint8_t> flags;
    std::vector<uint32_t> spec, status, dirty, off;
    std::vector<uint64_t> hashes;
    std::vector<uint8_t> kinds;
    PathStrs ps;
    PathVals pv;
};

struct gpudiff_ctx {
    int device = GPUDIFF_DEVICE_NONE;
    bool has_device = false;
    hipStream_t stream = nullptr;
    bool own_stream = false;
    uint32_t threads = 1;
    uint32_t flags = 0;
    bool k2_timeline = false;
    EncodeConfig ecfg;
    uint64_t hash_mask = ~0ULL;
    std::vector<std::unique_ptr<PairEncoder>> encoders;
    std::vector<gd::Part> parts;
    gpudiff_ticket next_ticket = 1;
    std::unordered_map<gpudiff_ticket, gpudiff_dbatch*> tickets;
    std::vector<std::array<hipEvent_t, 5>> pass_ev;
    size_t n_pass = 0;
    hipStream_t rb = nullptr;
    gpudiff_pass_stats pass_stats{};
    uint8_t* small_rb = nullptr;
    std::unordered_map<gpudiff_ticket, std::function<int(ResultStore&)>> finishers;
    DStore* pair_store = nullptr;
    gpudiff_path_stats path_stats{};
    gpudiff_path_stats value_stats{};
    uint64_t render_syncs = 0;
    FanCtx* fan = nullptr;
    gpudiff_dbatch* ring[2] = {nullptr, nullptr};
    gpudiff_hbatch* ring_hb[2] = {nullptr, nullptr};
    uint32_t ring_next = 0;
    std::unique_ptr<gd::WorkerPool> pool;
};

inline gd::WorkerPool& workers(gpudiff_ctx* c) {
    if (!c->pool) c->pool.reset(new gd::WorkerPool(c->threads));
    return *c->pool;
}

template <class F>
inline void for_deferred(gpudiff_ctx* c, size_t n_def, F&& fn) {
    if (!n_def) return;
    const uint32_t T = std::max<uint32_t>(1, std::min<uint32_t>(c->threads, (uint32_t)((n_def + 63) / 64)));
    workers(c).run(T, [&](uint32_t t) {
        for (size_t k = t; k < n_def; k += T) fn(k);
    });
}

inline int set_device(gpudiff_ctx* c) {
    if (!c->has_device) return GPUDIFF_E_NODEVICE;
    HIPCHK(hipSetDevice(c->device));
    return GPUDIFF_OK;
}

template <class T>
inline int dalloc(T** p, uint64_t count) {
    *p = nullptr;
    size_t bytes = (size_t)std::max<uint64_t>(count, 1) * sizeof(T);
    HIPCHK(hipMalloc((void**)p, bytes));
    return GPUDIFF_OK;
}

inline void dfree_all(gpudiff_dbatch* d) {
    if (d->pool && !d->pool_borrowed) (void)hipFree(d->pool);
    if (d->base) d->rows = nullptr, d->pair_ids = nullptr, d->desc = nullptr;
    void* ps[] = {d->rows, d->pair_ids, d->desc, d->flags, d->caps, d->chunk_counts, d->summary, d->spec_ids,
                  d->status_ids, d->dirty_ids, d->dirty_idx, d->scratch_off, d->path_count, d->path_off,
                  d->tile_sums, d->path_src, d->path_cnt, d->arena_h, d->arena_k,
                  d->scratch_h, d->scratch_k, d->out_h, d->out_k, d->nbits, d->noop_d, d->slot_owner,
                  d->slice_cnt, d->slice_weq, d->ids_alt[0], d->ids_alt[1], d->summary_alt, d->tail_perm,
                  d->small_image};
    for (void* p : ps)
        if (p) (void)hipFree(p);
    if (d->done) (void)hipEventDestroy(d->done);
    if (d->fan) fan_buffers_release(d->fan);
}

int collect_results(gpudiff_ctx* c, gpudiff_dbatch* d, ResultStore& rs);

inline uint64_t blob_value_bytes(const uint8_t* blob, uint32_t spec_l, uint32_t spec_ar, uint32_t stat_l) {
    uint64_t v = 0;
    const uint32_t* m = (const uint32_t*)(blob + 12ull * spec_l);
    for (uint32_t i = 0; i < spec_l; i++)
        if (gpudiff_meta_is_long(m[i])) v += gpudiff_meta_len(m[i]);
    m = (const uint32_t*)(blob + gpudiff_seg_bytes(spec_l, spec_ar) + 12ull * stat_l);
    for (uint32_t i = 0; i < stat_l; i++)
        if (gpudiff_meta_is_long(m[i])) v += gpudiff_meta_len(m[i]);
    return v;
}

inline uint64_t pair_compare_bytes(const gpudiff_pair_row& r) { return gpudiff_pair_compare_bytes(&r); }
```

kcp_amd/csrc/kernels.h:

```cpp
#pragma once
#include <hip/hip_runtime.h>
#include <stdint.h>

#include "../../include/gpudiff_format.h"

namespace gd {

constexpr uint32_t kJoinSliceHost = 1024;
constexpr uint64_t kMaxScratchEntries = 1ull << 31;

struct DiffBuffers {
    const gpudiff_pair_row* rows;
    const uint4* desc;
    const uint8_t* pool;
    const uint32_t* pair_ids;
    uint32_t n_pairs;
    uint8_t* flags;
    uint32_t* caps;
    uint32_t* path_src;
    uint32_t* path_cnt;
    uint8_t* nbits;
    uint8_t* noop_d;
    void* chunk_counts;
    uint32_t* summary;
    uint32_t* spec_ids;
    uint32_t* status_ids;
    uint32_t* dirty_ids;
    uint32_t* dirty_idx;
    uint32_t* scratch_off;
    uint32_t* path_count;
    uint32_t* path_off;
    uint32_t* tile_sums;
    uint64_t* arena_h;
    uint8_t* arena_k;
    uint32_t arena_per_wave;
    uint64_t* scratch_h;
    uint8_t* scratch_k;
    uint64_t scratch_cap;
    uint32_t* slot_owner;
    uint32_t* slice_cnt;
    uint8_t* slice_weq;
    uint64_t* out_h;
    uint8_t* out_k;
    uint64_t hash_mask;
    uint32_t k2_timeline;
    uint32_t k2_shared;
    uint32_t* tail_perm;
    struct TailPermKey* tail_perm_key;
    uint64_t rows_gen;
    uint64_t avg_pair_bytes;
    uint32_t* gather_send;
    uint32_t gather_cap_spec, gather_cap_status;
};

struct TailPermKey {
    const void* rows = nullptr;
    uint64_t rows_gen = ~0ull;
    uint32_t n_pairs = 0, lpt = 0, sub = 0, r2 = 0;
    bool operator==(const TailPermKey& o) const {
        return rows == o.rows && rows_gen == o.rows_gen && n_pairs == o.n_pairs && lpt == o.lpt && sub == o.sub &&
               r2 == o.r2;
    }
};

constexpr uint32_t kK2TailCounters = 8, kSummaryWords = 8 + 2 * kK2TailCounters;
constexpr uint32_t kK2TailQuarters = 2;

uint32_t k2_grid_waves(const DiffBuffers& b, uint32_t nchunks);

hipError_t launch_rebase(hipStream_t s, gpudiff_pair_row* rows, uint32_t begin, uint32_t end, uint64_t base,
                         uint32_t* pair_ids, uint4* desc);
struct BlobMove {
    uint64_t src, dst, bytes;
};
hipError_t launch_move_blobs(hipStream_t s, const uint8_t* src, uint8_t* dst, const BlobMove* moves, uint32_t n);
hipError_t launch_compare(hipStream_t s, const DiffBuffers& b);
hipError_t launch_compact(hipStream_t s, const DiffBuffers& b, uint32_t c0, uint32_t c1, const uint4* before,
                          uint4* after);
hipError_t launch_slot_owners(hipStream_t s, const DiffBuffers& b);
hipError_t launch_join(hipStream_t s, const DiffBuffers& b, uint32_t c0, uint32_t c1, const uint4* before,
                       const uint4* after);
hipError_t launch_emit(hipStream_t s, const DiffBuffers& b);
hipError_t launch_small_pass(hipStream_t s, const DiffBuffers& b, uint64_t arena_cap, uint8_t* image);
hipError_t k2_profile(uint64_t* dev_buf, uint32_t cap_waves);

}
```

kcp_amd/csrc/kernels.hip:

```cpp
#include <hip/hip_runtime.h>
#include <stdint.h>

#include "../../include/gpudiff.h"
#include "join_dev.h"
#include "kernels.h"
#include "stream_paths.h"
#include "wave_dev.h"
#include "xxh64.h"

namespace gd {


constexpr uint32_t SCAN_TILE = 4096;

struct V4 {
    uint32_t x, y, z, w;
};
__device__ __forceinline__ uint32_t vadd(uint32_t a, uint32_t b) { return a + b; }
__device__ __forceinline__ V4 vadd(const V4& a, const V4& b) {
    return V4{a.x + b.x, a.y + b.y, a.z + b.z, sat_add(a.w, b.w)};
}
template <class V> __device__ __forceinline__ V vzero() { return V{}; }
__device__ __forceinline__ uint32_t vshfl(uint32_t v, uint32_t src) { return shfl32(v, src); }
__device__ __forceinline__ V4 vshfl(const V4& v, uint32_t src) {
    return V4{shfl32(v.x, src), shfl32(v.y, src), shfl32(v.z, src), shfl32(v.w, src)};
}
template <class V>
__device__ __forceinline__ V wave_incl_scan_v(V v) {
    const uint32_t lane = lane_id();
#pragma unroll
    for (uint32_t d = 1; d < 64; d <<= 1) {
        V o = vshfl(v, lane >= d ? lane - d : lane);
        if (lane >= d) v = vadd(v, o);
    }
    return v;
}

__device__ __forceinline__ uint32_t scan_n(const uint32_t* n_dev, uint32_t n_host) { return n_dev ? *n_dev : n_host; }

template <class V>
__global__ __launch_bounds__(256) void k_scan_tiles(const V* __restrict__ in, const uint32_t* __restrict__ n_dev,
                                                    uint32_t n_host, V* __restrict__ tile_sums) {
    __shared__ V red[4];
    const uint32_t n = scan_n(n_dev, n_host);
    const uint32_t base = blockIdx.x * SCAN_TILE;
    if (base >= n) return;
    V s = vzero<V>();
    for (uint32_t i = threadIdx.x; i < SCAN_TILE; i += 256)
        if (base + i < n) s = vadd(s, in[base + i]);
    s = vshfl(wave_incl_scan_v(s), 63);
    if (lane_id() == 0) red[threadIdx.x >> 6] = s;
    __syncthreads();
    if (threadIdx.x == 0) tile_sums[blockIdx.x] = vadd(vadd(red[0], red[1]), vadd(red[2], red[3]));
}

__device__ __forceinline__ void mirror_store(uint32_t* m, const V4& v) {
    m[0] = v.x;
    m[1] = v.y;
    m[2] = v.z;
    m[3] = v.w;
}
__device__ __forceinline__ void mirror_store(uint32_t* m, uint32_t v) { m[0] = v; }

template <class V>
__global__ __launch_bounds__(256) void k_scan_apply(const V* in, const uint32_t* __restrict__ n_dev, uint32_t n_host,
                                                    const V* __restrict__ tile_sums, const V* base_in, V* total,
                                                    V* out, bool write_terminal, uint32_t* __restrict__ mirror) {
    __shared__ V wsum[4];
    __shared__ V wpre[4];
    const uint32_t n = scan_n(n_dev, n_host);
    const uint32_t last = n ? (n - 1) / SCAN_TILE : 0;
    if (blockIdx.x > last) return;
    const uint32_t base = blockIdx.x * SCAN_TILE;
    const uint32_t t = threadIdx.x;
    V p = vzero<V>();
    for (uint32_t i = t; i < blockIdx.x; i += 256) p = vadd(p, tile_sums[i]);
    p = vshfl(wave_incl_scan_v(p), 63);
    if (lane_id() == 0) wpre[t >> 6] = p;
    V v[16];
    V s = vzero<V>();
#pragma unroll
    for (int k = 0; k < 16; k++) {
        const uint32_t i = base + t * 16 + k;
        v[k] = i < n ? in[i] : vzero<V>();
        s = vadd(s, v[k]);
    }
    const V incl = wave_incl_scan_v(s);
    if (lane_id() == 63) wsum[t >> 6] = incl;
    __syncthreads();
    V run = vadd(vadd(wpre[0], wpre[1]), vadd(wpre[2], wpre[3]));
    if (base_in) run = vadd(run, *base_in);
    for (uint32_t w = 0; w < (t >> 6); w++) run = vadd(run, wsum[w]);
    const V excl_thread = vshfl(incl, lane_id() ? lane_id() - 1 : 0);
    if (lane_id()) run = vadd(run, excl_thread);
#pragma unroll
    for (int k = 0; k < 16; k++) {
        const uint32_t i = base + t * 16 + k;
        if (i < n) out[i] = run;
        run = vadd(run, v[k]);
    }
    if (blockIdx.x == last && t == 255) {
        *total = run;
        if (write_terminal) out[n] = run;
        if (mirror) mirror_store(mirror, run);
    }
}


struct StreamLog {
    uint32_t cnt[2][64];
    uint32_t ent[2][64][kSpLogCap];
    uint32_t first[64], n1[64];
    uint32_t hole[64];
};

__device__ uint32_t stream_region(const RegionView& A, const RegionView& B, uint64_t seg, const uint32_t* ent,
                                  uint32_t c, uint32_t g0, uint32_t hole, uint8_t region_bit,
                                  uint64_t* __restrict__ out_h, uint8_t* __restrict__ out_k, uint32_t out_base,
                                  uint32_t lane, bool* weq_all) {
    const uint32_t nc = 4u * c;
    const uint32_t e = lane < nc ? sp_entry_unhole(ent[lane >> 2] - sp_entry(g0, 0u), hole) : 0u;
    const bool cand = lane < nc && ((sp_entry_dwords(e) >> (lane & 3u)) & 1u);
    const uint64_t b = sp_entry_byte(e, lane & 3u);
    const SpWhere w = sp_classify(b, A.L);
    if (ballot(cand && (b >= seg || w.cls == SP_KEY))) return kSpRefuse;
    uint32_t leaf = w.idx;
    const bool ar = cand && w.cls == SP_ARENA;
    if (ballot(ar)) {
        bool found = false;
        uint32_t run = 0;
        for (uint32_t i0 = 0; i0 < A.L; i0 += 64u) {
            const uint32_t n = min(64u, A.L - i0);
            const uint32_t as = lane < n ? meta_arena(A.metas[i0 + lane]) : 0u;
            const uint32_t inc = wave_incl_scan(as);
            const uint32_t tot = shfl32(inc, 63);
            const uint32_t rel = w.idx - run;
            uint32_t o = 0;
#pragma unroll
            for (uint32_t s = 32; s >= 1; s >>= 1)
                if (shfl32(inc, o + s - 1u) <= rel) o += s;
            if (ar && !found && w.idx >= run && rel < tot) {
                leaf = i0 + o;
                found = true;
            }
            run += tot;
            if (!ballot(ar && !found)) break;
        }
        if (ballot(ar && !found)) return kSpRefuse;
    }
    bool dup = false;
    for (uint32_t j = 0; j < nc; j++) {
        const uint32_t xj = (uint32_t)__builtin_amdgcn_readlane((int)leaf, (int)j);
        const bool cj = __builtin_amdgcn_readlane((int)(cand ? 1 : 0), (int)j) != 0;
        if (cj && j < lane && xj == leaf) dup = true;
    }
    const bool uq = cand && !dup;
    const uint64_t um = ballot(uq);
    uint32_t rank = 0;
    for (uint32_t j = 0; j < nc; j++) {
        const uint32_t xj = (uint32_t)__builtin_amdgcn_readlane((int)leaf, (int)j);
        if (((um >> j) & 1ull) && xj < leaf) rank++;
    }
    uint32_t key = 0, ma = 0, mb = 0;
    uint64_t xa = 0, xb = 0;
    if (uq) {
        key = A.keys[leaf];
        ma = A.metas[leaf];
        mb = B.metas[leaf];
        xa = A.vals[leaf];
        xb = B.vals[leaf];
    }
    if (ballot(uq && meta_arena(ma) != meta_arena(mb))) return kSpRefuse;
    if (uq) {
        out_h[out_base + rank] = key;
        out_k[out_base + rank] = region_bit | GPUDIFF_PATH_CHANGED;
    }
    *weq_all = !ballot(uq && !wire_equal_number(ma, xa, mb, xb));
    return popc64(um);
}

__device__ uint32_t stream_pair(const gpudiff_pair_row& r, uint32_t f, const uint8_t* pool, uint64_t mask,
                                uint64_t* out_h, uint8_t* out_k, uint32_t base, uint32_t lane, uint32_t* noop,
                                const StreamLog* log, uint32_t k, bool log_ok, uint32_t* n_stream) {
    uint32_t n = 0;
    bool spec_weq = true, stat_weq = true;
    if (f & F_JSPEC) {
        RegionView A = region_view(pool, r.off_a, r.spec_l_a, r.spec_ar_a, false, r.spec_l_a);
        RegionView B = region_view(pool, r.off_b, r.spec_l_b, r.spec_ar_b, false, r.spec_l_b);
        const uint32_t c = log_ok ? uni(log->cnt[0][k]) : 0u;
        const uint32_t g0 = uni(log->first[k]);
        uint32_t got = kSpRefuse;
        if (c >= 1u && c <= kSpLogCap)
            got = stream_region(A, B, seg_bytes(r.spec_l_a, r.spec_ar_a), log->ent[0][k], c, g0, uni(log->hole[k]), 0,
                                out_h, out_k, base + n, lane, &spec_weq);
        if (got == kSpRefuse) got = join_region<true>(A, B, 0, out_h, out_k, base + n, lane, &spec_weq);
        else (*n_stream)++;
        n += got;
    }
    if (f & F_JSTAT) {
        RegionView A = region_view(pool, r.off_a, r.spec_l_a, r.spec_ar_a, true, r.stat_l_a);
        RegionView B = region_view(pool, r.off_b, r.spec_l_b, r.spec_ar_b, true, r.stat_l_b);
        const uint32_t c = log_ok ? uni(log->cnt[1][k]) : 0u;
        const uint32_t g0 = uni(log->first[k]) + uni(log->n1[k]);
        uint32_t got = kSpRefuse;
        if (c >= 1u && c <= kSpLogCap)
            got = stream_region(A, B, seg_bytes(r.stat_l_a, r.stat_ar_a), log->ent[1][k], c, g0, 0u,
                                GPUDIFF_PATH_REGION_STATUS, out_h, out_k, base + n, lane, &stat_weq);
        if (got == kSpRefuse)
            got = join_region<true>(A, B, GPUDIFF_PATH_REGION_STATUS, out_h, out_k, base + n, lane, &stat_weq);
        else (*n_stream)++;
        n += got;
    }
    const bool stat_ok = stat_weq && (!(f & F_SENT) || !(r.flags_a & GPUDIFF_OBJ_HAS_STATUS));
    *noop = (((f & F_SPEC) && spec_weq) ? NOOP_SPEC : 0u) | (((f & F_STATUS) && stat_ok) ? NOOP_STATUS : 0u);
    if (f & F_SENT) {
        if (lane == 0) {
            out_h[base + n] = status_sentinel_hash((r.flags_a >> GPUDIFF_OBJ_SEED_SHIFT) & 0xFFu, mask);
            out_k[base + n] = GPUDIFF_PATH_REGION_STATUS | GPUDIFF_PATH_STATUS_ABSENT;
        }
        n += 1;
    }
    return n;
}

__device__ __forceinline__ bool place_deferred(uint32_t d, uint64_t so, uint32_t cap, uint64_t scratch_cap,
                                               uint32_t* __restrict__ slot_owner) {
    if (so > scratch_cap || cap > scratch_cap - so) return false;
    const uint32_t b0 = (uint32_t)((so + kJoinSlice - 1u) / kJoinSlice);
    const uint32_t b1 = (uint32_t)((so + cap + kJoinSlice - 1u) / kJoinSlice);
    if (cap > kJoinSlice) {
        for (uint32_t q = b0; q < b1; q++) slot_owner[q] = d;
    } else if (b0 < b1) {
        slot_owner[b0] = kNoOwner;
    }
    return true;
}

__device__ __forceinline__ void join_whole(uint64_t wm, uint32_t p, uint32_t d, uint32_t so, uint32_t f,
                                           const gpudiff_pair_row* __restrict__ rows, const uint8_t* __restrict__ pool,
                                           uint64_t mask, uint64_t* __restrict__ sh, uint8_t* __restrict__ sk,
                                           uint32_t* __restrict__ path_count, uint8_t* __restrict__ noop_d,
                                           uint32_t lane) {
    for (; wm; wm &= wm - 1) {
        const uint32_t k = (uint32_t)__builtin_ctzll(wm);
        const uint32_t pk = (uint32_t)__builtin_amdgcn_readlane((int)p, (int)k);
        const uint32_t dk = (uint32_t)__builtin_amdgcn_readlane((int)d, (int)k);
        const uint32_t sok = (uint32_t)__builtin_amdgcn_readlane((int)so, (int)k);
        const uint32_t fk = (uint32_t)__builtin_amdgcn_readlane((int)f, (int)k);
        const gpudiff_pair_row r = rows[pk];
        uint32_t nb = 0;
        const uint32_t cnt = join_pair<true>(r, fk, pool, mask, sh, sk, sok, lane, &nb);
        if (lane == 0) {
            path_count[dk] = cnt;
            noop_d[dk] = (uint8_t)nb;
        }
    }
}

__global__ __launch_bounds__(256) void k_compact(const uint8_t* __restrict__ flags, const uint32_t* __restrict__ caps,
                                                 const uint32_t* __restrict__ pair_ids, uint32_t n,
                                                 const uint4* __restrict__ cbase, uint32_t* __restrict__ spec_ids,
                                                 uint32_t* __restrict__ status_ids, uint32_t* __restrict__ dirty_ids,
                                                 uint32_t* __restrict__ dirty_idx, uint32_t* __restrict__ scratch_off,
                                                 uint32_t c_begin, uint32_t c_end, const uint32_t* __restrict__ path_src,
                                                 const uint32_t* __restrict__ path_cnt,
                                                 uint32_t* __restrict__ path_count, const uint8_t* __restrict__ nbits,
                                                 uint8_t* __restrict__ noop_d, uint32_t* __restrict__ slot_owner,
                                                 uint64_t scratch_cap, const gpudiff_pair_row* __restrict__ rows,
                                                 const uint8_t* __restrict__ pool, uint64_t mask,
                                                 uint64_t* __restrict__ sh, uint8_t* __restrict__ sk,
                                                 uint32_t* __restrict__ gsend, uint32_t gcap_s, uint32_t gcap_t) {
    const uint32_t lane = lane_id();
    const uint32_t wave = uni((blockIdx.x * blockDim.x + threadIdx.x) >> 6);
    const uint32_t nwaves = (gridDim.x * blockDim.x) >> 6;
    const uint64_t lt = mask_lt(lane);
    for (uint32_t c = c_begin + wave; c < c_end; c += nwaves) {
        const uint32_t p = (c << 6) + lane;
        const bool valid = p < n;
        const uint32_t f = valid ? flags[p] : 0u;
        const uint64_t bs = ballot(f & F_SPEC), bt = ballot(f & F_STATUS), bd = ballot(f & (F_SPEC | F_STATUS));
        if (bd == 0) continue;
        const uint4 base = cbase[c];
        const bool dirty = (f & (F_SPEC | F_STATUS)) != 0u;
        const uint32_t id = dirty ? pair_ids[p] : 0u;
        const uint32_t cap = dirty ? caps[p] : 0u;
        const uint32_t cincl = wave_incl_scan(cap);
        if (f & F_SPEC) {
            const uint32_t q = base.x + popc64(bs & lt);
            spec_ids[q] = id;
            if (gsend && q < gcap_s) gsend[8u + q] = id;
// ... 383 lines not shown
                        (&slog->ent[0][0][0])[q * kSpLogCap + idx] = sp_entry(base + (uint32_t)u * 64u + l, info[u] >> 7);
                }
                while (m) {
                    const uint32_t j = (uint32_t)__builtin_ctzll(m);
                    m &= m - 1;
                    const uint32_t w = (uint32_t)__builtin_amdgcn_readlane((int)info[u], (int)j);
                    if (w & 64u) mis_t |= 1ull << (w & 63u);
                    else mis_s |= 1ull << (w & 63u);
                }
            }
        }
    };
    [[maybe_unused]] uint64_t tp_start = 0, tp_first = 0, tp_last = 0, tp_stream = 0, tp_join = 0, tp_items = 0;
    [[maybe_unused]] uint64_t tp_rows = 0, tp_pre = 0, tp_post = 0, tp_adv = 0, tp_e = 0, tp_r = 0, tp_je = 0;
    if constexpr (PROF) tp_start = wall_clock64();
    const uint32_t nch = c_end - c_begin;
    const uint32_t tail_c = k2_tail_chunks(nch, nwaves, sub_shift, tail_q);
    const uint32_t n_full = (nch - tail_c) << sub_shift;
    const uint32_t lpt_rounds = (sub_arg >> 20) & 3u;
    const uint32_t lpt_r = (tail_perm && tail_c == 0u && lpt_rounds) ? k2_lpt_round(n_full, nwaves, lpt_rounds) : 0u;
    const uint32_t n_main = n_full - lpt_r;
    const uint32_t r2 = (lpt_r && ((sub_arg >> 22) & 1u)) ? k2_item_round(n_main, nwaves) : 0u;
    const uint32_t n_main2 = n_main - r2;
    const uint32_t lpt_pairs = lpt_r << (6u - sub_shift);
    const uint32_t lpt_p0 = ((c_begin + (n_main >> sub_shift)) << 6) + (n_main & ((1u << sub_shift) - 1u)) * (64u >> sub_shift);
    const uint32_t nitems = lpt_r ? n_main + (lpt_r << (6u - sub_shift)) : n_full + (tail_c << tail_ish);
    uint32_t* const ctr = summary + 8u + (arena_per_wave ? arena_off / arena_per_wave : 0u);
    uint32_t* const ctr_tail = ctr + kK2TailCounters;
    const uint32_t tail0 = max(n_main, nwaves);
    auto advance = [&](uint32_t cur, uint32_t tk) -> uint32_t {
        if (cur < n_main) {
            const uint32_t nx = uni(__builtin_amdgcn_readlane(tk, 0)) + nwaves;
            if (nx < n_main) return nx;
        }
        uint32_t tt = 0;
        if (lane == 0) tt = atomicAdd(ctr_tail, 1u);
        return tail0 + uni(__builtin_amdgcn_readlane(tt, 0));
    };
    for (uint32_t it = wave, tk = 0; it < nitems; it = advance(it, tk)) {
        const bool lpt = lpt_r && it >= n_main;
        const bool tail_round = lpt_r && it >= n_main2;
        const uint32_t im = lpt ? 0u : (r2 && it >= n_main2) ? n_main2 + tail_perm[lpt_pairs + (it - n_main2)] : it;
        const bool tail = !lpt && im >= n_full;
        if (HELP && it < n_main && lane == 0) tk = atomicAdd(ctr, 1u);
        [[maybe_unused]] uint64_t tp_i = 0;
        if constexpr (PROF) {
            tp_i = wall_clock64();
            if (tp_e) tp_adv += tp_i - tp_e;
            tp_last = tp_i;
            tp_items++;
        }
        const uint32_t ish = lpt ? 6u : tail ? tail_ish : sub_shift;
        const uint32_t j = tail ? im - n_full : im;
        const uint32_t lp = lpt ? lpt_p0 + tail_perm[it - n_main] : 0u;
        const uint32_t c = lpt ? lp >> 6 : c_begin + (tail ? nch - tail_c : 0u) + (j >> ish);
        const uint32_t per = 64u >> ish;
        const uint32_t p0 = lpt ? lp : (c << 6) + (j & ((1u << ish) - 1u)) * per;
        if (p0 >= n) {
            if (!HELP && it < n_main && lane == 0) tk = atomicAdd(ctr, 1u);
            continue;
        }
        const uint32_t cnt = min(per, n - p0);
        const bool valid = lane < cnt;
        u32x4 v0 = {0, 0, 0, 0}, v1 = v0, v2 = v0, v3 = v0;
        [[maybe_unused]] u32x4 dv = v0;
        if constexpr (DESC) {
            if (valid) dv = *(const u32x4*)(desc + p0 + lane);
        } else if (valid) {
            const u32x4* rp = (const u32x4*)(rows + p0 + lane);
            v0 = rp[0];
            v1 = rp[1];
            v2 = rp[2];
            v3 = rp[3];
        }
        if constexpr (PROF) {
            tp_r = wall_clock64();
            tp_rows += tp_r - tp_i;
        }
        uint64_t off_a, off_b;
        bool err, spec_sz, has_st_b, stat_sz;
        uint32_t n1, n2, adj_a, adj_b;
        [[maybe_unused]] uint32_t hole = 0;
        [[maybe_unused]] uint32_t dbits = 0;
        constexpr uint32_t kPdRow = 0x80u;
        if constexpr (DESC) {
            gpudiff_pair_geom g = gpudiff_pair_desc_unpack(dv.x, dv.y, dv.z, dv.w);
            if (valid && gpudiff_pair_desc_is_escape(dv.w)) {
                const gpudiff_pair_row r = rows[p0 + lane];
                g = gpudiff_pair_row_geom(&r);
                g.bits |= kPdRow;
            }
            dbits = g.bits;
            off_a = g.off_a, off_b = g.off_b;
            err = valid && (dbits & GPUDIFF_PD_ERR) != 0u;
            spec_sz = (dbits & GPUDIFF_PD_SPEC_EQ) != 0u;
            has_st_b = (dbits & GPUDIFF_PD_HAS_ST_B) != 0u;
            stat_sz = has_st_b && (dbits & GPUDIFF_PD_STAT_EQ) != 0u;
            n1 = valid ? g.n1 : 0u, n2 = valid ? g.n2 : 0u;
            off_b += (uint64_t)g.adj_b - (uint64_t)g.adj_a;
            adj_a = adj_b = g.adj_a;
            hole = sp_hole_word(g.hs, g.hl);
        } else {
            off_a = ((uint64_t)v0.y << 32) | v0.x, off_b = ((uint64_t)v0.w << 32) | v0.z;
            err = valid && ((v3.x | v3.y) & GPUDIFF_OBJ_DECODE_ERR) != 0u;
            const bool ok = valid && !err;
            spec_sz = v1.x == v1.y && v1.z == v1.w;
            has_st_b = (v3.y & GPUDIFF_OBJ_HAS_STATUS) != 0u;
            stat_sz = has_st_b && v2.x == v2.y && v2.z == v2.w;
            const uint32_t seg_a = (uint32_t)seg_bytes(v1.x, v1.z), seg_b = (uint32_t)seg_bytes(v1.y, v1.w);
            const uint32_t seg_t = (uint32_t)seg_bytes(v2.x, v2.z);
            const uint32_t r128 = ((seg_a + seg_t + 127u) & ~127u);
            const bool no_stat = (v2.x | v2.y | v2.z | v2.w) == 0u;
            n1 = (ok && spec_sz) ? ((!stat_sz && no_stat) ? ((seg_a + 127u) & ~127u) : seg_a) >> 4 : 0u;
            n2 = (ok && stat_sz) ? (spec_sz ? r128 - seg_a : seg_t) >> 4 : 0u;
            adj_a = seg_a - 16u * n1, adj_b = seg_b - 16u * n1;
        }
        const uint32_t tot = n1 + n2;
        const uint32_t incl = wave_incl_scan(tot);
        const uint32_t total = uni(shfl32(incl, 63));
        const uint32_t first = incl - tot;
        uint64_t mis_s = 0, mis_t = 0;
        [[maybe_unused]] uint64_t tp_s0 = 0;
        if constexpr (PROF) {
            tp_s0 = wall_clock64();
            tp_pre += tp_s0 - tp_r;
        }
        if constexpr (HELP) {
            if (lane == 0) lds_st(&my->gen, lds_ld(&my->gen) + 1u);
            while (uni(lds_ld(&my->helpers)) != 0u) __builtin_amdgcn_s_sleep(1);
            if (lane == 0) {
                lds_st(&my->p0, p0);
                lds_st(&my->cnt, cnt);
                lds_st(&my->total, total);
                __hip_atomic_store(&my->mis_s, 0ull, __ATOMIC_RELAXED, __HIP_MEMORY_SCOPE_WORKGROUP);
                __hip_atomic_store(&my->mis_t, 0ull, __ATOMIC_RELAXED, __HIP_MEMORY_SCOPE_WORKGROUP);
                lds_st(&my->cursor, 64u * U);
                lds_st(&my->gen, lds_ld(&my->gen) + 1u);
            }
            for (uint32_t base = 0; base < total;) {
                uint32_t nb = 0;
                if (lane == 0) nb = lds_add(&my->cursor, 64u * U);
                stream_pass(base, total, incl, first, n1, adj_a, adj_b, off_a, off_b, mis_s, mis_t);
                base = uni(__builtin_amdgcn_readlane(nb, 0));
            }
            if (lane == 0) {
                lds_or64(&my->mis_s, mis_s);
                lds_or64(&my->mis_t, mis_t);
            }
            while (uni(lds_ld(&my->helpers)) != 0u) __builtin_amdgcn_s_sleep(1);
            const uint64_t ms = lds_ld64(&my->mis_s), mt = lds_ld64(&my->mis_t);
            mis_s = ((uint64_t)uni((uint32_t)(ms >> 32)) << 32) | uni((uint32_t)ms);
            mis_t = ((uint64_t)uni((uint32_t)(mt >> 32)) << 32) | uni((uint32_t)mt);
        } else {
            slog->cnt[0][lane] = 0u;
            slog->cnt[1][lane] = 0u;
            slog->first[lane] = first;
            slog->n1[lane] = n1;
            slog->hole[lane] = hole;
            uint32_t pass = 0;
            for (uint32_t base = 0; base < total; base += 64u * U, pass++) {
                stream_pass(base, total, incl, first, n1, adj_a, adj_b, off_a, off_b, mis_s, mis_t, hole);
                if (pass == 0 && it < n_main && lane == 0) tk = atomicAdd(ctr, 1u);
            }
            if (pass == 0 && it < n_main && lane == 0) tk = atomicAdd(ctr, 1u);
        }
        [[maybe_unused]] uint64_t tp_s1 = 0;
        if constexpr (PROF) {
            tp_s1 = wall_clock64();
            tp_stream += tp_s1 - tp_s0;
        }
        if constexpr (DESC) {
            v3.x = ((dbits & GPUDIFF_PD_HAS_ST_A) ? GPUDIFF_OBJ_HAS_STATUS : 0u) |
                   ((dbits & GPUDIFF_PD_SEED) ? 1u << GPUDIFF_OBJ_SEED_SHIFT : 0u);
            const bool sd = !spec_sz || ((mis_s >> lane) & 1ull), td = !stat_sz || ((mis_t >> lane) & 1ull);
            const bool plain_sent = !sd && !has_st_b && (dbits & GPUDIFF_PD_NO_STAT) && !(dbits & (GPUDIFF_PD_SEED | kPdRow));
            if (valid && !err && (sd || td) && !plain_sent) {
                const uint32_t* rp = (const uint32_t*)(rows + p0 + lane);
                const uint2 ls = *(const uint2*)(rp + 4), lt = *(const uint2*)(rp + 8);
                v1.x = ls.x, v1.y = ls.y;
                v2.x = lt.x, v2.y = lt.y;
                v3.x = rp[12];
            }
        }
        uint32_t myflag = 0, mycap = 0, mysrc = 0, mycnt = 0, mynoop = 0;
        if (err) {
            myflag = F_SPEC | F_STATUS | F_ERR;
        } else if (valid) {
            const bool spec_dirty = !spec_sz || ((mis_s >> lane) & 1ull);
            const bool stat_dirty = !stat_sz || ((mis_t >> lane) & 1ull);
            const bool stat_join = stat_dirty && (v2.x + v2.y) != 0u;
            myflag = (spec_dirty ? F_SPEC | F_JSPEC : 0u) | (stat_dirty ? F_STATUS : 0u) | (stat_join ? F_JSTAT : 0u) |
                     (stat_dirty && !has_st_b ? F_SENT : 0u) | (((v3.x >> GPUDIFF_OBJ_SEED_SHIFT) & 0xFFu) ? F_SEED : 0u);
            mycap = (spec_dirty ? v1.x + v1.y : 0u) + (stat_dirty ? v2.x + v2.y + (has_st_b ? 0u : 1u) : 0u);
        }
        const bool sent_only = valid && !err && (myflag & F_SENT) && !(myflag & (F_JSPEC | F_JSTAT));
        const uint64_t sm = ballot(sent_only);
        uint64_t done = 0;
        if (sm && used + popc64(sm) <= arena_per_wave) {
            if (sent_only) {
                const uint32_t src = wbase + used + popc64(sm & mask_lt(lane));
                ah[src] = (myflag & F_SEED) ? status_sentinel_hash((v3.x >> GPUDIFF_OBJ_SEED_SHIFT) & 0xFFu, mask) : sent0;
                ak[src] = GPUDIFF_PATH_REGION_STATUS | GPUDIFF_PATH_STATUS_ABSENT;
                mycap = 0;
                mysrc = src;
                mycnt = 1;
                mynoop = sentinel_noop_bits(v3.x);
            }
            used += popc64(sm);
            done = sm;
        }
        for (uint64_t dm = ballot((myflag & (F_SPEC | F_STATUS)) != 0u) & ~done; dm; dm &= dm - 1) {
            const uint32_t k = (uint32_t)__builtin_ctzll(dm);
            const uint32_t fk = (uint32_t)__builtin_amdgcn_readlane((int)myflag, (int)k);
            const uint32_t ck = (uint32_t)__builtin_amdgcn_readlane((int)mycap, (int)k);
            uint32_t src = 0, pc = 0, nb = 0;
            bool defer = false;
            if (used + ck <= arena_per_wave && ck <= (tail_round ? kTailJoinMax : kDeepJoin)) {
                src = wbase + used;
                if (fk & (F_JSPEC | F_JSTAT)) {
                    const gpudiff_pair_row r = rows[p0 + k];
                    if constexpr (HELP) pc = join_pair<true>(r, fk, pool, mask, ah, ak, src, lane, &nb);
                    else pc = stream_pair(r, fk, pool, mask, ah, ak, src, lane, &nb, slog, k, total < (1u << 28), &n_stream);
                } else if (fk & F_SENT) {
                    const uint32_t fa = (uint32_t)__builtin_amdgcn_readlane((int)v3.x, (int)k);
                    nb = sentinel_noop_bits(fa);
                    if (lane == 0) {
                        ah[src] = (fk & F_SEED) ? status_sentinel_hash((fa >> GPUDIFF_OBJ_SEED_SHIFT) & 0xFFu, mask)
                                                : sent0;
                        ak[src] = GPUDIFF_PATH_REGION_STATUS | GPUDIFF_PATH_STATUS_ABSENT;
                    }
                    pc = 1;
                }
                used += pc;
            } else {
                defer = true;
                deferred = true;
            }
            if (lane == k) {
                if (defer) {
                    myflag |= F_DEFER;
                    mycap = defer_cap(v1.x, v1.y, v2.x, v2.y, myflag);
                } else {
                    mycap = 0;
                    mysrc = src;
                    mycnt = pc;
                    mynoop = nb;
                }
            }
        }
        if constexpr (PROF) {
            const uint64_t t = wall_clock64();
            tp_join += t - tp_s1;
            if (tp_items == 1) tp_first = t;
            tp_je = t;
        }
        const bool dirty = (myflag & (F_SPEC | F_STATUS)) != 0u;
        const uint32_t ns = popc64(ballot(myflag & F_SPEC));
        const uint32_t nt = popc64(ballot(myflag & F_STATUS));
        const uint32_t nd = popc64(ballot(dirty));
        const uint32_t cs = wave_sum(dirty ? mycap : 0u);
        if (valid) {
            flags[p0 + lane] = (uint8_t)myflag;
            if (dirty) {
                caps[p0 + lane] = mycap;
                path_src[p0 + lane] = mysrc;
                path_cnt[p0 + lane] = mycnt;
                nbits[p0 + lane] = (uint8_t)mynoop;
            }
        }
        if (lane == 0) {
            if (!ish) {
                chunk_counts[c] = make_uint4(ns, nt, nd, cs);
            } else if (ns | nt | nd | cs) {
                uint32_t* cc = (uint32_t*)(chunk_counts + c);
                atomicAdd(cc + 0, ns);
                atomicAdd(cc + 1, nt);
                atomicAdd(cc + 2, nd);
                atomicAdd(cc + 3, cs);
            }
        }
        if constexpr (PROF) {
            tp_e = wall_clock64();
            tp_post += tp_e - tp_je;
        }
    }
    if constexpr (HELP) {
        const uint32_t wib = threadIdx.x >> 6;
        for (bool any = true; any;) {
            any = false;
            for (uint32_t q = 1; q < 4; q++) {
                HelpSlot* const h = &help_slots[(wib + q) & 3u];
                const uint32_t g = uni(lds_ld(&h->gen));
                if ((g & 1u) || uni(lds_ld(&h->cursor)) >= uni(lds_ld(&h->total))) continue;
                any = true;
                if (lane == 0) lds_add(&h->helpers, 1u);
                const uint32_t g1 = uni(lds_ld(&h->gen));
                const uint32_t hp0 = uni(lds_ld(&h->p0)), hcnt = uni(lds_ld(&h->cnt)), htot = uni(lds_ld(&h->total));
                const uint32_t g2 = uni(lds_ld(&h->gen));
                if (g1 == g && g2 == g) {
                    u32x4 v0 = {0, 0, 0, 0}, v1 = v0, v2 = v0, v3 = v0;
                    const bool valid = lane < hcnt;
                    if (valid) {
                        const u32x4* rp = (const u32x4*)(rows + hp0 + lane);
                        v0 = rp[0];
                        v1 = rp[1];
// ... 59 lines not shown

hipError_t k2_profile(uint64_t* dev_buf, uint32_t cap_waves) {
    hipError_t e = hipMemcpyToSymbol(HIP_SYMBOL(g_k2_prof), &dev_buf, sizeof(dev_buf));
    if (e != hipSuccess) return e;
    return hipMemcpyToSymbol(HIP_SYMBOL(g_k2_prof_cap), &cap_waves, sizeof(cap_waves));
}

__global__ __launch_bounds__(256) void k_copy_paths(const uint32_t* __restrict__ summary,
                                                    const uint32_t* __restrict__ scratch_off,
                                                    const uint32_t* __restrict__ path_off,
                                                    const uint32_t* __restrict__ path_count,
                                                    const uint64_t* __restrict__ sh, const uint8_t* __restrict__ sk,
                                                    const uint64_t* __restrict__ ah, const uint8_t* __restrict__ ak,
                                                    uint64_t* __restrict__ oh, uint8_t* __restrict__ ok) {
    const uint32_t lane = lane_id();
    const uint32_t wave = uni((blockIdx.x * blockDim.x + threadIdx.x) >> 6);
    const uint32_t nwaves = (gridDim.x * blockDim.x) >> 6;
    const uint32_t ndirty = summary[2];
    if (summary[4]) return;
    const uint32_t nchunks = (ndirty + 63u) >> 6;
    for (uint32_t c = wave; c < nchunks; c += nwaves) {
        const uint32_t d = (c << 6) + lane;
        const bool valid = d < ndirty;
        const uint32_t sraw = valid ? scratch_off[d] : 0u;
        const bool arena = (sraw & ARENA_BIT) != 0u;
        const uint32_t so = sraw & ~ARENA_BIT;
        const uint32_t po = valid ? path_off[d] : 0u;
        const uint32_t cnt = valid ? path_count[d] : 0u;
        const uint64_t* srch = arena ? ah : sh;
        const uint8_t* srck = arena ? ak : sk;
        const bool big = cnt > 16u;
        if (!big)
            for (uint32_t i = 0; i < cnt; i++) {
                oh[po + i] = srch[so + i];
                ok[po + i] = srck[so + i];
            }
        uint64_t m = ballot(big);
        while (m) {
            const uint32_t k = (uint32_t)__builtin_ctzll(m);
            m &= m - 1;
            const uint32_t sok = uni(shfl32(so, k)), pok = uni(shfl32(po, k)), ck = uni(shfl32(cnt, k));
            const bool ak_ = uni(shfl32(arena ? 1u : 0u, k)) != 0u;
            const uint64_t* bh = ak_ ? ah : sh;
            const uint8_t* bk = ak_ ? ak : sk;
            for (uint32_t i = lane; i < ck; i += 64) {
                oh[pok + i] = bh[sok + i];
                ok[pok + i] = bk[sok + i];
            }
        }
    }
}

__global__ __launch_bounds__(256) void k_move_blobs(const uint8_t* __restrict__ src, uint8_t* __restrict__ dst,
                                                    const BlobMove* __restrict__ moves, uint32_t n) {
    const uint32_t lane = lane_id();
    const uint32_t wave = uni((blockIdx.x * blockDim.x + threadIdx.x) >> 6);
    const uint32_t nwaves = (gridDim.x * blockDim.x) >> 6;
    for (uint32_t i = wave; i < n; i += nwaves) {
        const BlobMove m = moves[i];
        const u32x4* s4 = (const u32x4*)(src + m.src);
        u32x4* d4 = (u32x4*)(dst + m.dst);
        const uint64_t n16 = m.bytes >> 4;
        for (uint64_t k = lane; k < n16; k += 64) d4[k] = __builtin_nontemporal_load(s4 + k);
    }
}

__global__ __launch_bounds__(256) void k_rebase_rows(gpudiff_pair_row* __restrict__ rows, uint32_t begin, uint32_t end,
                                                     uint64_t base, uint32_t* __restrict__ pair_ids,
                                                     uint4* __restrict__ desc) {
    const uint32_t i = begin + blockIdx.x * blockDim.x + threadIdx.x;
    if (i >= end) return;
    gpudiff_pair_row r = rows[i];
    r.off_a += base;
    r.off_b += base;
    rows[i].off_a = r.off_a;
    rows[i].off_b = r.off_b;
    pair_ids[i] = r.pair_id;
    if (desc) {
        const gpudiff_pair_desc d = gpudiff_pair_desc_pack(&r);
        desc[i] = make_uint4(d.w[0], d.w[1], d.w[2], d.w[3]);
    }
}

static inline uint32_t grid_for(uint64_t waves_wanted, uint32_t cap_blocks) {
    uint64_t blocks = (waves_wanted + 3) / 4;
    if (blocks < 1) blocks = 1;
    return (uint32_t)(blocks < cap_blocks ? blocks : cap_blocks);
}

static constexpr uint32_t kPersistBlocks = 256 * 8;

hipError_t launch_rebase(hipStream_t s, gpudiff_pair_row* rows, uint32_t begin, uint32_t end, uint64_t base,
                         uint32_t* pair_ids, uint4* desc) {
    if (end <= begin) return hipSuccess;
    k_rebase_rows<<<(end - begin + 255) / 256, 256, 0, s>>>(rows, begin, end, base, pair_ids, desc);
    return hipGetLastError();
}



hipError_t launch_move_blobs(hipStream_t s, const uint8_t* src, uint8_t* dst, const BlobMove* moves, uint32_t n) {
    if (!n) return hipSuccess;
    k_move_blobs<<<grid_for(n, kPersistBlocks), 256, 0, s>>>(src, dst, moves, n);
    return hipGetLastError();
}

typedef void (*K2Fn)(const gpudiff_pair_row*, const uint8_t*, uint32_t, uint8_t*, uint32_t*, uint4*, uint32_t, uint32_t,
                     uint64_t*, uint8_t*, uint32_t, uint32_t, uint32_t, uint32_t*, uint32_t*, uint8_t*, uint64_t,
                     uint32_t*, uint32_t, const uint32_t*, const uint4*);
constexpr uint32_t kK2Kernels = 8;
static K2Fn k2_kernel(uint32_t k) {
    switch (k) {
        case 1: case 5: return k_compare_flat<16, 1, false, true>;
        case 2: return k_compare_flat<8, 1, true>;
        case 3: case 7: return k_compare_flat<16, 1, true, true>;
        case 4: return k_compare_flat<8, 1, false, false, true>;
        case 6: return k_compare_flat<8, 1, true, false, true>;
        default: return k_compare_flat<8, 1>;
    }
}

constexpr uint64_t kK2BigPairBytes = 16384;
static uint32_t k2_variant_of(const DiffBuffers& b) {
    return (b.avg_pair_bytes >= kK2BigPairBytes ? 1u : 0u) | (b.k2_timeline ? 2u : 0u) | (b.desc ? 4u : 0u);
}

constexpr uint32_t kK2LptMax = 16384;
constexpr uint32_t kK2LptRounds = 1;
constexpr uint32_t kK2MaxSubShift = 3;
constexpr uint32_t kK2ItemsPerWave = 6;

static uint32_t k2_cap_blocks(const DiffBuffers& b) {
    static int occ[kK2Kernels] = {0};
    const uint32_t v = k2_variant_of(b);
    if (!occ[v]) {
        int n = 0;
        if (hipOccupancyMaxActiveBlocksPerMultiprocessor(&n, reinterpret_cast<const void*>(k2_kernel(v)), 256, 0) !=
                hipSuccess || n <= 0)
            n = 4;
        occ[v] = n;
    }
    return 256u * (uint32_t)((b.k2_shared && !(v & 1u)) ? std::max(1, occ[v] / 2) : occ[v]);
}

constexpr uint32_t kK2ItemsPerWaveBig = 8, kK2MaxSubShiftBig = 6;

static uint32_t k2_sub_shift(const DiffBuffers& b, uint32_t nchunks) {
    const bool big = b.avg_pair_bytes >= kK2BigPairBytes;
    const uint64_t want = (uint64_t)(big ? kK2ItemsPerWaveBig : kK2ItemsPerWave) * 4u * k2_cap_blocks(b);
    const uint32_t max_shift = big ? kK2MaxSubShiftBig : kK2MaxSubShift;
    uint32_t k = 0;
    while (k < max_shift && (uint64_t)nchunks << k < want) k++;
    return k;
}

uint32_t k2_grid_waves(const DiffBuffers& b, uint32_t nchunks) {
    const uint64_t items = (uint64_t)nchunks << k2_sub_shift(b, nchunks);
    return grid_for(items, k2_cap_blocks(b)) * 4u;
}

__global__ __launch_bounds__(256) void k_pass_reset(uint32_t* __restrict__ summary, uint32_t nwords,
                                                    uint4* __restrict__ cc, uint32_t ncc) {
    const uint32_t i = blockIdx.x * 256u + threadIdx.x;
    if (summary && i < nwords) summary[i] = 0u;
    for (uint32_t j = i; j < ncc; j += gridDim.x * 256u) cc[j] = make_uint4(0u, 0u, 0u, 0u);
}

__device__ __forceinline__ uint64_t pair_stream_bytes(const gpudiff_pair_row& r) {
    if ((r.flags_a | r.flags_b) & GPUDIFF_OBJ_DECODE_ERR) return 65u;
    const bool spec_sz = r.spec_l_a == r.spec_l_b && r.spec_ar_a == r.spec_ar_b;
    const bool stat_sz = (r.flags_b & GPUDIFF_OBJ_HAS_STATUS) && r.stat_l_a == r.stat_l_b && r.stat_ar_a == r.stat_ar_b;
    const uint64_t seg_s = seg_bytes(r.spec_l_a, r.spec_ar_a), seg_t = seg_bytes(r.stat_l_a, r.stat_ar_a);
    uint64_t per = 0;
    if (spec_sz && stat_sz) per = (seg_s + seg_t + 127u) & ~127ull;
    else if (spec_sz) per = (r.stat_l_a | r.stat_l_b | r.stat_ar_a | r.stat_ar_b) ? seg_s : (seg_s + 127u) & ~127ull;
    else if (stat_sz) per = seg_t;
    return 65u + 2u * per;
}

__device__ void block_sort_u32(uint32_t* key, uint32_t r) {
    uint32_t m2 = 1;
    while (m2 < r) m2 <<= 1;
    for (uint32_t t = r + threadIdx.x; t < m2; t += blockDim.x) key[t] = ~0u;
    __syncthreads();
    for (uint32_t k = 2; k <= m2; k <<= 1)
        for (uint32_t j = k >> 1; j > 0; j >>= 1) {
            for (uint32_t i = threadIdx.x; i < m2; i += blockDim.x) {
                const uint32_t l = i ^ j;
                if (l > i) {
                    const uint32_t a = key[i], bb = key[l];
                    if (((i & k) == 0) == (a > bb)) {
                        key[i] = bb;
                        key[l] = a;
                    }
                }
            }
            __syncthreads();
        }
}

__global__ __launch_bounds__(1024) void k_tail_order(const gpudiff_pair_row* __restrict__ rows, uint32_t n,
                                                     uint32_t p_first, uint32_t r, uint32_t c_begin, uint32_t n_main2,
                                                     uint32_t r2, uint32_t sub_shift, uint32_t* __restrict__ perm) {
    __shared__ uint32_t key[kK2LptMax];
    for (uint32_t t = threadIdx.x; t < r; t += blockDim.x) {
        const uint32_t p = p_first + t;
        const uint64_t bytes = p < n ? pair_stream_bytes(rows[p]) : 0u;
        const uint32_t b16 = (uint32_t)min(bytes >> 4, (uint64_t)0xFFFFu);
        key[t] = ((0xFFFFu - b16) << 16) | t;
    }
    block_sort_u32(key, r);
    for (uint32_t t = threadIdx.x; t < r; t += blockDim.x) perm[t] = key[t] & 0xFFFFu;
    __syncthreads();
    const uint32_t per = 64u >> sub_shift;
    for (uint32_t t = threadIdx.x; t < r2; t += blockDim.x) {
        const uint32_t m = n_main2 + t;
        const uint32_t p0 = ((c_begin + (m >> sub_shift)) << 6) + (m & ((1u << sub_shift) - 1u)) * per;
        uint64_t bytes = 0;
        for (uint32_t p = p0; p < min(p0 + per, n); p++) bytes += pair_stream_bytes(rows[p]);
        const uint32_t b32 = (uint32_t)min(bytes >> 5, (uint64_t)0xFFFFu);
        key[t] = ((0xFFFFu - b32) << 16) | t;
    }
    if (r2) {
        block_sort_u32(key, r2);
        for (uint32_t t = threadIdx.x; t < r2; t += blockDim.x) perm[r + t] = key[t] & 0xFFFFu;
    }
}

static uint32_t k2_lpt_items(const DiffBuffers& b, uint32_t nch, uint32_t nwaves, uint32_t sub, uint32_t tail) {
    if (!b.tail_perm || tail || b.avg_pair_bytes < kK2BigPairBytes) return 0;
    const uint32_t r = k2_lpt_round(nch << sub, nwaves, kK2LptRounds);
    return (r << (6u - sub)) + k2_item_round((nch << sub) - r, nwaves) <= kK2LptMax ? r : 0;
}

hipError_t launch_compare(hipStream_t s, const DiffBuffers& b) {
    const uint32_t nch = (b.n_pairs + 63u) / 64u;
    const dim3 grid(k2_grid_waves(b, nch) / 4u);
    uint4* cc = (uint4*)b.chunk_counts;
    const uint32_t sub = k2_sub_shift(b, nch);
    const uint32_t v = k2_variant_of(b);
    const uint32_t tq = kK2TailQuarters;
    const uint32_t tail = k2_tail_chunks(nch, grid.x * 4u, sub, tq);
    const uint32_t lpt = k2_lpt_items(b, nch, grid.x * 4u, sub, tail);
    const uint32_t* perm = nullptr;
    if (lpt) {
        const uint32_t n_main = (nch << sub) - lpt;
        const uint32_t p_first = ((n_main >> sub) << 6) + (n_main & ((1u << sub) - 1u)) * (64u >> sub);
        const uint32_t r2 = k2_item_round(n_main, grid.x * 4u);
        const TailPermKey key{b.rows, b.rows_gen, b.n_pairs, lpt, sub, r2};
        if (!(*b.tail_perm_key == key)) {
            k_tail_order<<<1, 1024, 0, s>>>(b.rows, b.n_pairs, p_first, lpt << (6u - sub), 0u, n_main - r2, r2, sub,
                                            b.tail_perm);
            *b.tail_perm_key = key;
        }
        perm = b.tail_perm;
    }
    {
        const uint32_t z0 = sub ? 0u : lpt ? (((nch << sub) - lpt) >> sub) : nch - tail;
        const uint32_t ncc = nch - z0;
        k_pass_reset<<<std::max(1u, std::min(1024u, (ncc + 255u) / 256u)), 256, 0, s>>>(b.summary, kSummaryWords,
                                                                                        cc + z0, ncc);
    }
    const uint32_t sub_arg = sub | (tq << 8) | (lpt ? kK2LptRounds << 20 | 1u << 22 : 0u);
    k2_kernel(v)<<<grid, 256, 0, s>>>(b.rows, b.pool, b.n_pairs, b.flags, b.caps, cc, 0u, nch, b.arena_h, b.arena_k, 0u,
                                      b.arena_per_wave, b.arena_per_wave, b.path_src, b.path_cnt, b.nbits, b.hash_mask,
                                      b.summary, sub_arg, perm, (v & 1u) ? nullptr : b.desc);
    return hipGetLastError();
}

static uint32_t compact_cap_blocks() {
    static int occ = 0;
    if (!occ) {
        int n = 0;
        if (hipOccupancyMaxActiveBlocksPerMultiprocessor(&n, reinterpret_cast<const void*>(k_compact), 256, 0) !=
                hipSuccess || n <= 0)
            n = 4;
        occ = n;
    }
    return std::min<uint32_t>(kPersistBlocks, 256u * (uint32_t)occ);
}

hipError_t launch_compact(hipStream_t s, const DiffBuffers& b, uint32_t c0, uint32_t c1, const uint4* before,
                          uint4* after) {
    const uint32_t n = c1 - c0;
    const uint32_t ntiles = (n + SCAN_TILE - 1) / SCAN_TILE;
    V4* cc = (V4*)b.chunk_counts + c0;
    V4* ts = (V4*)b.tile_sums;
    if (ntiles) k_scan_tiles<V4><<<ntiles, 256, 0, s>>>(cc, nullptr, n, ts);
    uint32_t* mirror = (b.gather_send && (const void*)after == (const void*)b.summary) ? b.gather_send : nullptr;
    k_scan_apply<V4><<<std::max(ntiles, 1u), 256, 0, s>>>(cc, nullptr, n, ts, (const V4*)before, (V4*)after, cc,
                                                          false, mirror);
    k_compact<<<grid_for(n, compact_cap_blocks()), 256, 0, s>>>(
        b.flags, b.caps, b.pair_ids, b.n_pairs, (const uint4*)b.chunk_counts, b.spec_ids, b.status_ids, b.dirty_ids,
        b.dirty_idx, b.scratch_off, c0, c1, b.path_src, b.path_cnt, b.path_count, b.nbits, b.noop_d, b.slot_owner,
        b.scratch_cap, b.rows, b.pool, b.hash_mask, b.scratch_h, b.scratch_k, b.gather_send, b.gather_cap_spec,
        b.gather_cap_status);
    return hipGetLastError();
}

hipError_t launch_join(hipStream_t s, const DiffBuffers& b, uint32_t c0, uint32_t c1, const uint4* before,
                       const uint4* after) {
    const uint32_t k4_blocks = (uint32_t)std::min<uint64_t>(kPersistBlocks,
                                                            (b.scratch_cap / kJoinSlice + 3u) / 4u + 1u);
    (void)c0;
    (void)c1;
    k_join_slices<<<k4_blocks, 256, 0, s>>>(b.rows, b.pool, b.flags, b.dirty_idx, b.scratch_off, b.slot_owner,
                                                 b.summary, before, after, b.scratch_cap, b.scratch_h, b.scratch_k,
                                                 b.slice_cnt, b.slice_weq);
    k_join_gather<<<k4_blocks, 256, 0, s>>>(b.rows, b.flags, b.dirty_idx, b.scratch_off, b.slot_owner,
                                                                     b.summary, before, after, b.hash_mask,
                                                                     b.scratch_h, b.scratch_k, b.slice_cnt,
                                                                     b.slice_weq, b.path_count, b.noop_d);
    return hipGetLastError();
}

hipError_t launch_slot_owners(hipStream_t s, const DiffBuffers& b) {
    k_slot_owners<<<compact_cap_blocks(), 256, 0, s>>>(b.flags, b.caps, b.dirty_idx, b.scratch_off, b.summary,
                                                       b.scratch_cap, b.slot_owner, b.rows, b.pool, b.hash_mask,
                                                       b.scratch_h, b.scratch_k, b.path_count, b.noop_d);
    return hipGetLastError();
}

hipError_t launch_emit(hipStream_t s, const DiffBuffers& b) {
    const uint32_t ntiles = b.n_pairs / SCAN_TILE + 1;
    const uint32_t* nd = b.summary + 2;
    k_scan_tiles<uint32_t><<<ntiles, 256, 0, s>>>(b.path_count, nd, 0, b.tile_sums);
    k_scan_apply<uint32_t><<<ntiles, 256, 0, s>>>(b.path_count, nd, 0, b.tile_sums, nullptr, b.summary + 5,
                                                  b.path_off, true, nullptr);
    k_copy_paths<<<grid_for((b.n_pairs + 63) / 64, kPersistBlocks), 256, 0, s>>>(
        b.summary, b.scratch_off, b.path_off, b.path_count, b.scratch_h, b.scratch_k, b.arena_h, b.arena_k, b.out_h,
        b.out_k);
    return hipGetLastError();
}

}
```

kcp_amd/csrc/stream_paths.h:

```cpp
#pragma once
#include <stdint.h>

#include "../../include/gpudiff_format.h"

#if defined(__HIPCC__)
#define GD_SP_HD __host__ __device__
#else
#define GD_SP_HD
#endif

namespace gd {

constexpr uint32_t kSpLogCap = 4;
constexpr uint32_t kSpMaxLeaves = 64;
constexpr uint32_t kSpRefuse = 0xFFFFFFFFu;

GD_SP_HD inline uint32_t sp_entry(uint32_t chunk, uint32_t dwords) { return (chunk << 4) | (dwords & 15u); }
GD_SP_HD inline uint32_t sp_entry_dwords(uint32_t e) { return e & 15u; }
GD_SP_HD inline uint64_t sp_entry_byte(uint32_t e, uint32_t d) { return 16ull * (e >> 4) + 4u * d; }

static_assert(GPUDIFF_KEYS_HOLE_UNIT % 128u == 0u, "sp_hole_word keeps the hole in 128-B lines");
GD_SP_HD inline uint32_t sp_hole_word(uint32_t hs, uint32_t hl) { return (hs >> 3) | ((hl >> 3) << 16); }
GD_SP_HD inline uint32_t sp_hole_start(uint32_t w) { return (w & 0xFFFFu) << 3; }
GD_SP_HD inline uint32_t sp_hole_chunks(uint32_t w) { return (w >> 16) << 3; }
GD_SP_HD inline uint32_t sp_hole_bytes(uint32_t w) { return (w >> 16) << 7; }
GD_SP_HD inline uint32_t sp_entry_unhole(uint32_t e, uint32_t w) {
    return e + ((e >> 4) >= sp_hole_start(w) ? sp_entry(sp_hole_chunks(w), 0u) : 0u);
}

GD_SP_HD inline uint32_t sp_meta_arena(uint32_t m) {
    return ((m & 7u) == GPUDIFF_TAG_STR && (m >> 3) > GPUDIFF_INLINE_MAX) ? (((m >> 3) - GPUDIFF_INLINE_MAX + 3u) & ~3u)
                                                                          : 0u;
}

enum SpClass : uint32_t { SP_VAL = 0, SP_KEY = 1, SP_META = 2, SP_ARENA = 3 };
struct SpWhere {
    uint32_t cls;
    uint32_t idx;
};
GD_SP_HD inline SpWhere sp_classify(uint64_t b, uint32_t L) {
    const uint64_t l = L;
    if (b < 8u * l) return SpWhere{SP_VAL, (uint32_t)(b >> 3)};
    if (b < 12u * l) return SpWhere{SP_KEY, (uint32_t)((b - 8u * l) >> 2)};
    if (b < 16u * l) return SpWhere{SP_META, (uint32_t)((b - 12u * l) >> 2)};
    return SpWhere{SP_ARENA, (uint32_t)(b - 16u * l)};
}

GD_SP_HD inline uint32_t sp_arena_owner(const uint32_t* metas, uint32_t L, uint32_t ao) {
    uint32_t off = 0;
    for (uint32_t i = 0; i < L; i++) {
        const uint32_t n = sp_meta_arena(metas[i]);
        if (ao - off < n) return i;
        off += n;
    }
    return L;
}

GD_SP_HD inline uint32_t sp_region_rule(const uint8_t* seg_a, const uint8_t* seg_b, uint32_t L, uint64_t seg_bytes,
                                        const uint32_t* entries, uint32_t n, uint32_t leaves[kSpMaxLeaves]) {
    const uint32_t* ma = (const uint32_t*)(seg_a + 12ull * L);
    const uint32_t* mb = (const uint32_t*)(seg_b + 12ull * L);
    uint32_t ns = 0;
    for (uint32_t q = 0; q < n; q++)
        for (uint32_t d = 0; d < 4; d++) {
            if (!((sp_entry_dwords(entries[q]) >> d) & 1u)) continue;
            const uint64_t b = sp_entry_byte(entries[q], d);
            if (b >= seg_bytes) return kSpRefuse;
            const SpWhere w = sp_classify(b, L);
            if (w.cls == SP_KEY) return kSpRefuse;
            const uint32_t leaf = w.cls == SP_ARENA ? sp_arena_owner(ma, L, w.idx) : w.idx;
            if (leaf >= L) return kSpRefuse;
            uint32_t at = 0;
            while (at < ns && leaves[at] < leaf) at++;
            if (at < ns && leaves[at] == leaf) continue;
            if (ns == kSpMaxLeaves) return kSpRefuse;
            for (uint32_t k = ns; k > at; k--) leaves[k] = leaves[k - 1];
            leaves[at] = leaf;
            ns++;
        }
    for (uint32_t k = 0; k < ns; k++)
        if (sp_meta_arena(ma[leaves[k]]) != sp_meta_arena(mb[leaves[k]])) return kSpRefuse;
    return ns;
}

}
```

kcp_amd/gpudiff.py:

```python
from __future__ import annotations

import ctypes as C
import json
import os
from dataclasses import dataclass
from typing import Any, Iterable, List, Optional, Sequence, Tuple, Union

import numpy as np

from . import buildinfo

_HERE = os.path.dirname(os.path.abspath(__file__))
LIB_PATH = os.path.join(_HERE, "libgpudiff.so")

ABI_VERSION = 6
OK = 0
E_INVAL, E_NOMEM, E_DEVICE, E_NODEVICE, E_CAPACITY, E_STATE, E_DECODE, E_NOTFOUND = range(-1, -9, -1)

SPEC_DIRTY, STATUS_DIRTY, DECODE_ERROR, SPEC_NOOP, STATUS_NOOP = 0x1, 0x2, 0x4, 0x8, 0x10
PATH_CHANGED, PATH_ADDED, PATH_REMOVED, PATH_STATUS_ABSENT = 0, 1, 2, 3
PATH_REGION_STATUS = 0x80
TAG_NULL, TAG_FALSE, TAG_TRUE, TAG_INT, TAG_FLOAT, TAG_STR, TAG_EOBJ, TAG_EARR = range(8)
VALUE_ABSENT = 0xFF
OPT_TIMING = 0x1
OPT_DEVICE_ENCODE = 0x2000000
OPT_PATH_STRINGS = 0x8000000
OPT_PATH_VALUES = 0x80000000
OPT_K2_ROWS = 0x40
OPT_ARENA_SHIFT = 21
OPT_SMALL_PASS = 0x20000000
SMALL_PASS_MAX_PAIRS = 4096
SMALL_PASS_MAX_PATHS = 32768
DEVICE_CURRENT, DEVICE_NONE = -1, -2

PATH_HASH_BITS = 32
OBJ_HAS_STATUS, OBJ_DECODE_ERR, OBJ_FRESH, OBJ_SEED_SHIFT = 0x1, 0x2, 0x4, 8
OBJ_SPEC_KEYS_EQ = 0x8
OBJ_SPEC_SHAPE_EQ = 0x10
STORE_DEVICE_ENCODE = 0x1
EXPORT_COUNTS, EXPORT_SPEC_IDS, EXPORT_STATUS_IDS, EXPORT_DIRTY_IDS, EXPORT_FLAGS = range(5)


class GpuDiffError(RuntimeError):
    def __init__(self, code: int, where: str):
        self.code = code
        super().__init__("%s: %s (%d)" % (where, _lib.gpudiff_strerror(code).decode(), code))


class Opts(C.Structure):
    _fields_ = [("device", C.c_int32), ("encode_threads", C.c_uint32), ("stream", C.c_void_p),
                ("flags", C.c_uint32), ("path_hash_bits", C.c_uint32)]


class JsonPair(C.Structure):
    _fields_ = [("old_json", C.c_void_p), ("old_len", C.c_size_t), ("new_json", C.c_void_p),
                ("new_len", C.c_size_t), ("pair_id", C.c_uint32), ("cluster_id", C.c_uint32)]


JSON_PAIR_DTYPE = np.dtype([("old_json", "<u8"), ("old_len", "<u8"), ("new_json", "<u8"), ("new_len", "<u8"),
                            ("pair_id", "<u4"), ("cluster_id", "<u4")])
assert JSON_PAIR_DTYPE.itemsize == C.sizeof(JsonPair)


def json_pair_array(buf: np.ndarray, offs: np.ndarray, ids=None, clusters=None) -> np.ndarray:
    n = (len(offs) - 1) // 2
    base = buf.ctypes.data
    o = offs.astype(np.uint64)
    arr = np.zeros(n, dtype=JSON_PAIR_DTYPE)
    arr["old_json"] = base + o[0:2 * n:2]
    arr["old_len"] = o[1:2 * n + 1:2] - o[0:2 * n:2]
    arr["new_json"] = base + o[1:2 * n + 1:2]
    arr["new_len"] = o[2:2 * n + 2:2] - o[1:2 * n + 1:2]
    arr["pair_id"] = np.arange(n, dtype=np.uint32) if ids is None else ids
    arr["cluster_id"] = 0 if clusters is None else clusters
    return arr


ZC_SLACK = 32


def zero_copy_layout(lens: np.ndarray):
    span = (lens.astype(np.uint64) + ZC_SLACK + 15) & ~np.uint64(15)
    offs = np.zeros(lens.size, np.uint64)
    np.cumsum(span[:-1], out=offs[1:])
    return offs, int(offs[-1] + span[-1]) + ZC_SLACK if lens.size else ZC_SLACK


class PinnedJson:

    def __init__(self, eng: "Engine", buf: np.ndarray, offs: np.ndarray, ids=None, clusters=None):
        n = (len(offs) - 1) // 2
        o = offs.astype(np.int64)
        lens = np.diff(o)
        doffs, nbytes = zero_copy_layout(lens)
        p = C.c_void_p()
        _chk(_lib.gpudiff_host_alloc(eng.ctx, nbytes, C.byref(p)), "gpudiff_host_alloc")
        self.eng, self.ptr, self.nbytes = eng, p.value, nbytes
        dst = np.ctypeslib.as_array(C.cast(self.ptr, C.POINTER(C.c_uint8)), (nbytes,))
        src = np.ascontiguousarray(buf)
        for k in range(2 * n):
            a, ln, d = int(o[k]), int(lens[k]), int(doffs[k])
            dst[d:d + ln] = src[a:a + ln]
        self.pairs = np.zeros(n, dtype=JSON_PAIR_DTYPE)
        self.pairs["old_json"] = self.ptr + doffs[0:2 * n:2]
        self.pairs["old_len"] = lens[0:2 * n:2]
        self.pairs["new_json"] = self.ptr + doffs[1:2 * n:2]
        self.pairs["new_len"] = lens[1:2 * n:2]
        self.pairs["pair_id"] = np.arange(n, dtype=np.uint32) if ids is None else ids
        self.pairs["cluster_id"] = 0 if clusters is None else clusters

    def free(self):
        if self.ptr:
            _chk(_lib.gpudiff_host_free(self.eng.ctx, self.ptr), "gpudiff_host_free")
            self.ptr = None


class PinnedDocs:

    def __init__(self, eng: "Engine", lens):
        lens = np.asarray(lens, dtype=np.uint64)
# ... 128 lines not shown


class RBatchStats(C.Structure):
    _fields_ = [("n_docs", C.c_uint64), ("json_bytes", C.c_uint64), ("scratch_bytes", C.c_uint64),
                ("k11_ms", C.c_double), ("k12_ms", C.c_double), ("runs", C.c_uint64)]


class NBatchStats(C.Structure):
    _fields_ = [("n_pairs", C.c_uint64), ("json_bytes", C.c_uint64), ("scratch_bytes", C.c_uint64),
                ("n_host", C.c_uint64), ("k13_ms", C.c_double), ("k14_ms", C.c_double), ("runs", C.c_uint64)]


class HBatchInfo(C.Structure):
    _fields_ = [("n_pairs", C.c_size_t), ("rows", C.c_void_p), ("pool", C.c_void_p), ("pool_bytes", C.c_uint64),
                ("total_leaves", C.c_uint64), ("n_decode_errors", C.c_uint64), ("n_reseeded", C.c_uint64)]


class Result(C.Structure):
    _fields_ = [("n_pairs", C.c_size_t), ("pair_flags", C.c_void_p),
                ("n_spec_dirty", C.c_size_t), ("spec_dirty_ids", C.c_void_p),
                ("n_status_dirty", C.c_size_t), ("status_dirty_ids", C.c_void_p),
                ("n_dirty", C.c_size_t), ("dirty_ids", C.c_void_p), ("path_offsets", C.c_void_p),
                ("n_paths", C.c_size_t), ("path_hashes", C.c_void_p), ("path_kinds", C.c_void_p),
                ("internal_", C.c_void_p)]


class PathStringsC(C.Structure):
    _fields_ = [("n_paths", C.c_size_t), ("offsets", C.c_void_p), ("bytes", C.c_void_p), ("n_host", C.c_size_t),
                ("n_unresolved", C.c_size_t)]


class PathValuesC(C.Structure):
    _fields_ = [("n_paths", C.c_size_t), ("offsets", C.c_void_p), ("bytes", C.c_void_p), ("tags", C.c_void_p),
                ("n_host", C.c_size_t), ("n_unresolved", C.c_size_t)]


class PathStats(C.Structure):
    _fields_ = [("batches", C.c_uint64), ("paths", C.c_uint64), ("bytes", C.c_uint64), ("host_paths", C.c_uint64),
                ("kernel_ms", C.c_double), ("timed_batches", C.c_uint64)]


class PassStats(C.Structure):
    _fields_ = [("passes", C.c_uint64), ("small_passes", C.c_uint64), ("small_redone", C.c_uint64),
                ("redo_arena", C.c_uint64), ("redo_deep", C.c_uint64), ("redo_paths", C.c_uint64),
                ("readback_rounds", C.c_uint64)]

    def as_dict(self):
        return {n: int(getattr(self, n)) for n, _ in self._fields_}


class ClusterIndexC(C.Structure):
    _fields_ = [("n_clusters", C.c_size_t), ("cluster_ids", C.c_void_p), ("spec_off", C.c_void_p),
                ("status_off", C.c_void_p), ("n_spec", C.c_size_t), ("n_status", C.c_size_t),
                ("spec_ids", C.c_void_p), ("status_ids", C.c_void_p), ("sorted_on_device", C.c_uint32),
                ("internal", C.c_void_p)]


class ClusterIndexStats(C.Structure):
    _fields_ = [("calls", C.c_uint64), ("sorted_calls", C.c_uint64), ("syncs", C.c_uint64), ("entries", C.c_uint64),
                ("d2h_bytes", C.c_uint64), ("kernel_ms", C.c_double), ("timed_calls", C.c_uint64)]

    def as_dict(self):
        return {n: getattr(self, n) for n, _ in self._fields_}


class ClusterIndexFinalStats(C.Structure):
    _fields_ = [("calls", C.c_uint64), ("patched_calls", C.c_uint64), ("compacted_calls", C.c_uint64),
                ("sorted_calls", C.c_uint64), ("syncs", C.c_uint64), ("entries_in", C.c_uint64),
                ("entries_live", C.c_uint64), ("patch_rows", C.c_uint64), ("h2d_bytes", C.c_uint64),
                ("d2h_bytes", C.c_uint64), ("kernel_ms", C.c_double), ("timed_calls", C.c_uint64)]

    def as_dict(self):
        return {n: getattr(self, n) for n, _ in self._fields_}


class DeviceView(C.Structure):
    _fields_ = [("pair_flags", C.c_void_p), ("spec_dirty_ids", C.c_void_p), ("status_dirty_ids", C.c_void_p),
                ("dirty_ids", C.c_void_p), ("counts", C.c_void_p)]


class BatchStats(C.Structure):
    _fields_ = [("n_pairs", C.c_uint64), ("pool_bytes", C.c_uint64), ("total_leaves", C.c_uint64),
                ("compare_bytes", C.c_uint64), ("value_bytes", C.c_uint64)]


class Timings(C.Structure):
    _fields_ = [("compare_ms", C.c_float), ("compact_ms", C.c_float),
                ("join_ms", C.c_float), ("emit_ms", C.c_float), ("total_ms", C.c_float),
                ("n_passes", C.c_uint32), ("k2_launches", C.c_uint32)]


_P = C.c_void_p
SIGNATURES = [
    ("gpudiff_strerror", C.c_char_p, [C.c_int]),
    ("gpudiff_abi_version", C.c_int, []),
    ("gpudiff_build_id", C.c_char_p, []),
    ("gpudiff_device_count", C.c_int, [C.POINTER(C.c_int)]),
    ("gpudiff_open", C.c_int, [C.POINTER(Opts), C.POINTER(_P)]),
    ("gpudiff_close", None, [_P]),
    ("gpudiff_encode_pairs", C.c_int, [_P, C.POINTER(JsonPair), C.c_size_t, C.POINTER(_P)]),
    ("gpudiff_hbatch_info_get", C.c_int, [_P, C.POINTER(HBatchInfo)]),
    ("gpudiff_hbatch_free", None, [_P, _P]),
    ("gpudiff_dbatch_create", C.c_int, [_P, C.c_uint64, C.c_uint64, C.POINTER(_P)]),
    ("gpudiff_dbatch_append", C.c_int, [_P, _P, _P]),
    ("gpudiff_dbatch_reset", C.c_int, [_P, _P]),
    ("gpudiff_dbatch_stats_get", C.c_int, [_P, C.POINTER(BatchStats)]),
    ("gpudiff_dbatch_device_view", C.c_int, [_P, C.POINTER(DeviceView)]),
    ("gpudiff_dbatch_read_pool", C.c_int, [_P, _P, C.c_uint64, C.c_void_p, C.c_uint64]),
    ("gpudiff_dbatch_export", C.c_int, [_P, _P, C.c_uint32, C.c_void_p, C.c_uint64, C.c_uint64]),
    ("gpudiff_dbatch_free", None, [_P, _P]),
    ("gpudiff_dbatch_bind_gather", C.c_int, [_P, _P, C.c_void_p, C.c_uint32, C.c_uint32]),
    ("gpudiff_dbatch_result_slot", C.c_int, [_P, _P, C.c_uint32]),
    ("gpudiff_dbatch_create_view", C.c_int, [_P, _P, C.POINTER(_P)]),
    ("gpudiff_cluster_bytes", C.c_int, [C.c_void_p, C.c_size_t, C.c_uint32, C.c_void_p]),
    ("gpudiff_shard_lpt", C.c_int, [C.c_void_p, C.c_uint32, C.c_uint32, C.c_void_p]),
    ("gpudiff_rows_stream_bytes", C.c_int, [C.c_void_p, C.c_size_t, C.POINTER(C.c_uint64)]),
    ("gpudiff_rows_read_bytes", C.c_int, [C.c_void_p, C.c_size_t, C.POINTER(C.c_uint64)]),
    ("gpudiff_diff", C.c_int, [_P, _P, C.POINTER(C.c_uint64)]),
    ("gpudiff_wait", C.c_int, [_P, C.c_uint64, C.POINTER(Result)]),
    ("gpudiff_result_release", None, [_P, C.POINTER(Result)]),
    ("gpudiff_result_path_strings", C.c_int, [_P, C.POINTER(Result), C.POINTER(PathStringsC)]),
    ("gpudiff_path_strings_stats_get", C.c_int, [_P, C.POINTER(PathStats)]),
    ("gpudiff_result_path_values", C.c_int, [_P, C.POINTER(Result), C.POINTER(PathValuesC)]),
    ("gpudiff_path_values_stats_get", C.c_int, [_P, C.POINTER(PathStats)]),
    ("gpudiff_render_syncs_get", C.c_int, [_P, C.POINTER(C.c_uint64)]),
    ("gpudiff_render_value_from_blob", C.c_int, [C.c_char_p, C.POINTER(ObjInfo), C.c_uint32, C.c_uint64,
                                                 C.POINTER(C.c_uint8), C.c_void_p, C.c_size_t, C.POINTER(C.c_size_t)]),
    ("gpudiff_last_timings", C.c_int, [_P, C.POINTER(Timings)]),
    ("gpudiff_pass_stats_get", C.c_int, [_P, C.POINTER(PassStats)]),
    ("gpudiff_sync", C.c_int, [_P]),
    ("gpudiff_timing_reset", C.c_int, [_P]),
    ("gpudiff_hbatch_create", C.c_int, [_P, C.c_uint64, C.c_size_t, C.c_uint64, C.POINTER(_P), C.POINTER(_P),
                                        C.POINTER(_P)]),
    ("gpudiff_hbatch_resize", C.c_int, [_P, _P, C.c_uint64, C.c_size_t, C.c_uint64, C.POINTER(_P),
                                        C.POINTER(_P)]),
    ("gpudiff_submit", C.c_int, [_P, C.POINTER(JsonPair), C.c_size_t, C.POINTER(C.c_uint64)]),
    ("gpudiff_cluster_index_get", C.c_int, [_P, C.c_uint64, C.POINTER(ClusterIndexC)]),
    ("gpudiff_cluster_index_release", None, [_P, C.POINTER(ClusterIndexC)]),
    ("gpudiff_cluster_index_host", C.c_int, [C.c_void_p, C.c_void_p, C.c_void_p, C.c_size_t,
                                             C.POINTER(ClusterIndexC)]),
    ("gpudiff_cluster_index_stats_get", C.c_int, [_P, C.POINTER(ClusterIndexStats)]),
    ("gpudiff_cluster_index_get_final", C.c_int, [_P, C.c_uint64, C.POINTER(ClusterIndexC)]),
    ("gpudiff_cluster_index_final_stats_get", C.c_int, [_P, C.POINTER(ClusterIndexFinalStats)]),
    ("gpudiff_store_create", C.c_int, [_P, C.c_uint32, C.c_uint64, C.c_uint32, C.POINTER(_P)]),
    ("gpudiff_store_create_ex", C.c_int, [_P, C.c_uint32, C.c_uint64, C.c_uint32, C.c_uint32, C.POINTER(_P)]),
    ("gpudiff_store_submit", C.c_int, [_P, _P, C.POINTER(Event), C.c_size_t, C.POINTER(C.c_uint64)]),
    ("gpudiff_store_forget", C.c_int, [_P, _P, C.c_uint32]),
    ("gpudiff_store_stats_get", C.c_int, [_P, C.POINTER(StoreStats)]),
    ("gpudiff_submit_stats_get", C.c_int, [_P, C.POINTER(StoreStats)]),
    ("gpudiff_host_alloc", C.c_int, [_P, C.c_size_t, C.POINTER(C.c_void_p)]),
    ("gpudiff_host_free", C.c_int, [_P, C.c_void_p]),
    ("gpudiff_store_free", None, [_P, _P]),
    ("gpudiff_encode_objects", C.c_int, [_P, C.POINTER(C.c_void_p), C.POINTER(C.c_size_t), C.POINTER(C.c_uint32),
                                         C.c_size_t, C.c_void_p, C.c_uint64, C.POINTER(ObjInfo)]),
    ("gpudiff_encode_object_host", C.c_int, [C.c_char_p, C.c_size_t, C.c_uint32, C.c_uint32, C.c_void_p, C.c_uint64,
                                             C.POINTER(ObjInfo)]),
    ("gpudiff_render_path_from_blob", C.c_int, [C.c_char_p, C.POINTER(ObjInfo), C.c_uint32, C.c_uint64, C.c_void_p,
                                                C.c_size_t, C.POINTER(C.c_size_t)]),
    ("gpudiff_k0_profile", C.c_int, [_P, C.c_int, C.POINTER(C.c_uint64)]),
    ("gpudiff_k2_profile", C.c_int, [_P, C.c_void_p, C.c_uint32]),
    ("gpudiff_upsert_bodies", C.c_int, [_P, C.POINTER(C.c_void_p), C.POINTER(C.c_size_t), C.c_size_t, C.c_uint32,
                                        C.POINTER(Bodies)]),
    ("gpudiff_bodies_release", None, [_P, C.POINTER(Bodies)]),
    ("gpudiff_write_plan_get", C.c_int, [_P, C.c_uint64, C.POINTER(WritePlanC)]),
    ("gpudiff_write_plan_get_ex", C.c_int, [_P, C.c_uint64, C.c_uint32, C.POINTER(WritePlanC)]),
    ("gpudiff_write_plan_release", None, [_P, C.POINTER(WritePlanC)]),
    ("gpudiff_store_write_plan_get", C.c_int, [_P, _P, C.c_uint64, C.c_uint32, C.POINTER(WritePlanC)]),
    ("gpudiff_store_plan_stats_get", C.c_int, [_P, C.POINTER(StorePlanStats)]),
    ("gpudiff_wbatch_create", C.c_int, [_P, C.POINTER(C.c_void_p), C.POINTER(C.c_size_t), C.c_size_t, C.c_uint32,
                                        C.POINTER(_P)]),
    ("gpudiff_wbatch_run", C.c_int, [_P, _P]),
    ("gpudiff_wbatch_fetch", C.c_int, [_P, _P, C.POINTER(Bodies)]),
    ("gpudiff_wbatch_stats_get", C.c_int, [_P, C.POINTER(WBatchStats)]),
    ("gpudiff_wbatch_free", None, [_P, _P]),
    ("gpudiff_upsert_body_host", C.c_int, [C.c_char_p, C.c_size_t, C.c_uint32, C.c_void_p, C.c_size_t,
                                           C.POINTER(C.c_size_t)]),
    ("gpudiff_bodies_rv_splice", C.c_int, [_P, C.POINTER(Bodies), C.POINTER(RvSpliceC)]),
    ("gpudiff_splice_resource_version", C.c_int, [C.c_char_p, C.c_size_t, C.c_uint32, C.c_uint32, C.c_char_p,
                                                  C.c_size_t, C.c_void_p, C.c_size_t, C.POINTER(C.c_size_t)]),
    ("gpudiff_upsert_body_host_rv", C.c_int, [C.c_char_p, C.c_size_t, C.c_uint32, C.c_void_p, C.c_size_t,
                                              C.POINTER(C.c_size_t), C.POINTER(C.c_uint32),
                                              C.POINTER(C.c_uint32)]),
    ("gpudiff_update_body_host", C.c_int, [C.c_char_p, C.c_size_t, C.c_uint32, C.c_char_p, C.c_size_t,
                                           C.c_void_p, C.c_size_t, C.POINTER(C.c_size_t)]),
    ("gpudiff_bodies_targets", C.c_int, [_P, C.POINTER(Bodies), C.POINTER(TargetsC)]),
    ("gpudiff_target_decode", C.c_int, [C.c_char_p, C.c_size_t, C.c_uint32, C.c_uint32, C.c_void_p, C.c_size_t,
                                        C.POINTER(C.c_size_t)]),
    ("gpudiff_target_host", C.c_int, [C.c_char_p, C.c_size_t, C.c_void_p, C.c_size_t, C.POINTER(C.c_size_t),
                                      C.c_void_p, C.c_size_t, C.POINTER(C.c_size_t)]),
    ("gpudiff_targets_namespaces", C.c_int, [C.POINTER(Bodies), C.POINTER(TargetsC), C.c_void_p, C.c_void_p,
                                             C.c_void_p, C.c_void_p, C.POINTER(C.c_size_t)]),
    ("gpudiff_upsert_body_host_targets", C.c_int, [C.c_char_p, C.c_size_t, C.c_uint32, C.c_void_p, C.c_size_t,
                                                   C.POINTER(C.c_size_t), C.POINTER(C.c_uint32),
                                                   C.POINTER(C.c_uint32), C.POINTER(C.c_uint32)]),
    ("gpudiff_rbatch_create", C.c_int, [_P, C.POINTER(C.c_void_p), C.POINTER(C.c_size_t), C.c_size_t,
                                        C.POINTER(_P)]),
    ("gpudiff_rbatch_run", C.c_int, [_P, _P]),
    ("gpudiff_rbatch_fetch", C.c_int, [_P, _P, C.POINTER(Rollup)]),
    ("gpudiff_rbatch_stats_get", C.c_int, [_P, C.POINTER(RBatchStats)]),
    ("gpudiff_rbatch_free", None, [_P, _P]),
# ... 17 lines not shown
                                                 C.POINTER(C.c_int32)]),
    ("gpudiff_classify_updates_host_kinds", C.c_int, [C.c_void_p, C.POINTER(C.c_void_p), C.POINTER(C.c_size_t),
                                                      C.POINTER(C.c_void_p), C.POINTER(C.c_size_t), C.c_size_t,
                                                      C.c_uint32, C.POINTER(C.c_int32)]),
    ("gpudiff_negotiate_pair_host_kind", C.c_int, [C.c_uint32, C.c_char_p, C.c_size_t, C.c_char_p, C.c_size_t,
                                                   C.POINTER(C.c_int32)]),
    ("gpudiff_classify_updates_host", C.c_int, [C.POINTER(C.c_void_p), C.POINTER(C.c_size_t), C.POINTER(C.c_void_p),
                                                C.POINTER(C.c_size_t), C.c_size_t, C.c_uint32, C.POINTER(C.c_int32)]),
    ("gpudiff_negotiate_pair_host", C.c_int, [C.c_char_p, C.c_size_t, C.c_char_p, C.c_size_t,
                                              C.POINTER(C.c_int32)]),
    ("gpudiff_spec_equal", C.c_int, [_P, C.c_char_p, C.c_size_t, C.c_char_p, C.c_size_t, C.POINTER(C.c_int)]),
    ("gpudiff_status_equal", C.c_int, [_P, C.c_char_p, C.c_size_t, C.c_char_p, C.c_size_t, C.POINTER(C.c_int)]),
    ("gpudiff_resolve_path", C.c_int, [C.c_char_p, C.c_size_t, C.c_char_p, C.c_size_t, C.c_uint64, C.c_uint8,
                                       C.c_uint32, C.c_char_p, C.c_size_t, C.POINTER(C.c_size_t)]),
]


def _load() -> C.CDLL:
    if not os.path.exists(LIB_PATH):
        raise ImportError("libgpudiff.so not built (run `python kcp_amd/build.py`); there is no CPU fallback")
    from . import _hiprt
    _hiprt.preload()
    lib = C.CDLL(LIB_PATH)
    for name, res, args in SIGNATURES:
        f = getattr(lib, name)
        f.restype = res
        f.argtypes = args
    got = lib.gpudiff_abi_version()
    if got != ABI_VERSION:
        raise ImportError("%s has ABI %d, this binding needs %d (rebuild with kcp_amd/build.py)"
                          % (LIB_PATH, got, ABI_VERSION))
    global BUILD_ID, BUILD_VERIFIED
    BUILD_ID = lib.gpudiff_build_id().decode()
    if buildinfo.sources_present():
        want = buildinfo.source_id()
        if BUILD_ID != want:
            raise ImportError("%s was built from other sources (build ID %s, the shipped sources hash to %s): "
                              "rebuild with kcp_amd/build.py" % (LIB_PATH, BUILD_ID, want))
        BUILD_VERIFIED = True
    return lib


BUILD_ID = ""
BUILD_VERIFIED = False
_lib = _load()


def lib() -> C.CDLL:
    return _lib


def _chk(rc: int, where: str):
    if rc != OK:
        raise GpuDiffError(rc, where)


def device_count() -> int:
    n = C.c_int(0)
    _chk(_lib.gpudiff_device_count(C.byref(n)), "gpudiff_device_count")
    return n.value


def cluster_bytes(rows: np.ndarray, n_clusters: int) -> np.ndarray:
    rows = np.ascontiguousarray(rows, dtype=ROW_DTYPE)
    out = np.zeros(n_clusters, dtype=np.uint64)
    _chk(_lib.gpudiff_cluster_bytes(rows.ctypes.data, rows.size, n_clusters, out.ctypes.data), "gpudiff_cluster_bytes")
    return out


def stream_bytes(rows: np.ndarray) -> int:
    rows = np.ascontiguousarray(rows, dtype=ROW_DTYPE)
    out = C.c_uint64()
    _chk(_lib.gpudiff_rows_stream_bytes(rows.ctypes.data, rows.size, C.byref(out)), "gpudiff_rows_stream_bytes")
    return int(out.value)


def read_bytes(rows: np.ndarray) -> int:
    rows = np.ascontiguousarray(rows, dtype=ROW_DTYPE)
    out = C.c_uint64()
    _chk(_lib.gpudiff_rows_read_bytes(rows.ctypes.data, rows.size, C.byref(out)), "gpudiff_rows_read_bytes")
    return int(out.value)


def shard_lpt(weights, world: int) -> np.ndarray:
    w = np.ascontiguousarray(weights, dtype=np.uint64)
    owner = np.zeros(w.size, dtype=np.int32)
    _chk(_lib.gpudiff_shard_lpt(w.ctypes.data, w.size, world, owner.ctypes.data), "gpudiff_shard_lpt")
    return owner


def to_json_bytes(obj: Union[bytes, bytearray, str, dict]) -> bytes:
    if isinstance(obj, (bytes, bytearray)):
        return bytes(obj)
    if isinstance(obj, str):
        return obj.encode()
    return json.dumps(obj, separators=(",", ":")).encode()


@dataclass
class DiffResult:
    pair_flags: np.ndarray
    spec_dirty_ids: np.ndarray
    status_dirty_ids: np.ndarray
    dirty_ids: np.ndarray
    path_offsets: np.ndarray
    path_hashes: np.ndarray
    path_kinds: np.ndarray
    path_strings: Optional[List[bytes]] = None
    paths_host: int = 0
    paths_unresolved: int = 0
    path_values: Optional[List[Tuple[int, Optional[bytes], int, Optional[bytes]]]] = None
    values_host: int = 0
    values_unresolved: int = 0

    def paths_of(self, k: int) -> List[Tuple[int, int]]:
        b, e = int(self.path_offsets[k]), int(self.path_offsets[k + 1])
        return list(zip(self.path_hashes[b:e].tolist(), self.path_kinds[b:e].tolist()))

    def rendered_paths_of(self, k: int) -> List[Tuple[int, int, str]]:
        if self.path_strings is None:
            raise GpuDiffError(E_STATE, "DiffResult.rendered_paths_of")
        b, e = int(self.path_offsets[k]), int(self.path_offsets[k + 1])
        return [(h, kd, s.decode("utf-8", "surrogateescape")) for h, kd, s in
                zip(self.path_hashes[b:e].tolist(), self.path_kinds[b:e].tolist(), self.path_strings[b:e])]


def _changed_values_of(self, k: int):
    if self.path_values is None:
        raise GpuDiffError(E_STATE, "DiffResult.changed_values_of")
    b, e = int(self.path_offsets[k]), int(self.path_offsets[k + 1])
    return [(h, kd) + v for h, kd, v in
            zip(self.path_hashes[b:e].tolist(), self.path_kinds[b:e].tolist(), self.path_values[b:e])]


DiffResult.changed_values_of = _changed_values_of


def _arr(ptr, n, dtype):
    if n == 0 or not ptr:
        return np.zeros(0, dtype=dtype)
    ct = np.ctypeslib.as_ctypes_type(np.dtype(dtype))
    return np.ctypeslib.as_array(C.cast(ptr, C.POINTER(ct)), shape=(n,)).copy()


@dataclass
class ClusterIndex:
    cluster_ids: np.ndarray
    spec_off: np.ndarray
    status_off: np.ndarray
    spec_ids: np.ndarray
    status_ids: np.ndarray
    sorted_on_device: int = 0

    def of(self, cluster_id: int) -> Tuple[np.ndarray, np.ndarray]:
        j = int(np.searchsorted(self.cluster_ids, np.uint32(cluster_id)))
        if j >= self.cluster_ids.size or int(self.cluster_ids[j]) != int(cluster_id):
            return self.spec_ids[:0], self.status_ids[:0]
        return (self.spec_ids[int(self.spec_off[j]):int(self.spec_off[j + 1])],
                self.status_ids[int(self.status_off[j]):int(self.status_off[j + 1])])


def _take_cluster_index(ctx, ci: ClusterIndexC) -> ClusterIndex:
    try:
        return ClusterIndex(cluster_ids=_arr(ci.cluster_ids, ci.n_clusters, np.uint32),
                            spec_off=_arr(ci.spec_off, ci.n_clusters + 1, np.uint32),
                            status_off=_arr(ci.status_off, ci.n_clusters + 1, np.uint32),
                            spec_ids=_arr(ci.spec_ids, ci.n_spec, np.uint32),
                            status_ids=_arr(ci.status_ids, ci.n_status, np.uint32),
                            sorted_on_device=int(ci.sorted_on_device))
    finally:
        _lib.gpudiff_cluster_index_release(ctx, C.byref(ci))


def cluster_index_host(flags, pair_ids, cluster_ids) -> ClusterIndex:
    f = np.ascontiguousarray(flags, dtype=np.uint8)
    p = np.ascontiguousarray(pair_ids, dtype=np.uint32)
    c = np.ascontiguousarray(cluster_ids, dtype=np.uint32)
    if not f.size == p.size == c.size:
        raise ValueError("cluster_index_host: flags, pair_ids and cluster_ids differ in length")
    ci = ClusterIndexC()
    _chk(_lib.gpudiff_cluster_index_host(f.ctypes.data, p.ctypes.data, c.ctypes.data, f.size, C.byref(ci)),
         "gpudiff_cluster_index_host")
    return _take_cluster_index(None, ci)


class HostBatch:
    def __init__(self, engine: "Engine", handle: int, keep: Any):
        self.engine = engine
        self.h = C.c_void_p(handle)
        self._keep = keep

    def info(self) -> HBatchInfo:
        inf = HBatchInfo()
        _chk(_lib.gpudiff_hbatch_info_get(self.h, C.byref(inf)), "gpudiff_hbatch_info_get")
        return inf

    def rows(self) -> np.ndarray:
        inf = self.info()
        if inf.n_pairs == 0:
            return np.zeros(0, dtype=ROW_DTYPE)
        buf = (C.c_uint8 * (inf.n_pairs * 64)).from_address(inf.rows)
        return np.frombuffer(bytes(buf), dtype=ROW_DTYPE)

    def pool(self) -> bytes:
        inf = self.info()
        return C.string_at(inf.pool, inf.pool_bytes) if inf.pool_bytes else b""

    def pool_view(self) -> np.ndarray:
        inf = self.info()
        if not inf.pool_bytes:
            return np.zeros(0, np.uint8)
        return np.ctypeslib.as_array((C.c_uint8 * inf.pool_bytes).from_address(inf.pool))

    def free(self):
        if self.h:
            _lib.gpudiff_hbatch_free(self.engine.ctx, self.h)
            self.h = C.c_void_p(0)

    def __del__(self):
        try:
            self.free()
        except Exception:
            pass


class DeviceBatch:
    def __init__(self, engine: "Engine", pool_bytes: int, max_pairs: int, _view_of: "DeviceBatch" = None):
        self.engine = engine
        h = C.c_void_p()
        if _view_of is None:
            _chk(_lib.gpudiff_dbatch_create(engine.ctx, pool_bytes, max_pairs, C.byref(h)), "gpudiff_dbatch_create")
        else:
            _chk(_lib.gpudiff_dbatch_create_view(engine.ctx, _view_of.h, C.byref(h)), "gpudiff_dbatch_create_view")
        self.base = _view_of
        self.h = h

    def view(self, engine: "Engine") -> "DeviceBatch":
        return DeviceBatch(engine, 0, 0, _view_of=self)

    def append(self, hb: HostBatch):
        _chk(_lib.gpudiff_dbatch_append(self.engine.ctx, self.h, hb.h), "gpudiff_dbatch_append")

    def reset(self):
        _chk(_lib.gpudiff_dbatch_reset(self.engine.ctx, self.h), "gpudiff_dbatch_reset")

    def stats(self) -> BatchStats:
        st = BatchStats()
        _chk(_lib.gpudiff_dbatch_stats_get(self.h, C.byref(st)), "gpudiff_dbatch_stats_get")
        return st

    def device_view(self) -> DeviceView:
        v = DeviceView()
        _chk(_lib.gpudiff_dbatch_device_view(self.h, C.byref(v)), "gpudiff_dbatch_device_view")
        return v

    def export(self, what: int, dst_device_ptr: int, max_elems: int, known_count: int = 1 << 62):
        _chk(_lib.gpudiff_dbatch_export(self.engine.ctx, self.h, what, dst_device_ptr, max_elems, known_count),
             "gpudiff_dbatch_export")

    def bind_gather(self, send_device_ptr: int, cap_spec: int, cap_status: int):
        _chk(_lib.gpudiff_dbatch_bind_gather(self.engine.ctx, self.h, send_device_ptr or None, cap_spec, cap_status),
             "gpudiff_dbatch_bind_gather")

    def result_slot(self, slot: int):
        _chk(_lib.gpudiff_dbatch_result_slot(self.engine.ctx, self.h, slot), "gpudiff_dbatch_result_slot")

    def read_pool(self, off: int, nbytes: int) -> bytes:
        buf = C.create_string_buffer(max(nbytes, 1))
        _chk(_lib.gpudiff_dbatch_read_pool(self.engine.ctx, self.h, off, buf, nbytes), "gpudiff_dbatch_read_pool")
        return buf.raw[:nbytes]

    def free(self):
        if self.h:
            _lib.gpudiff_dbatch_free(self.engine.ctx, self.h)
            self.h = C.c_void_p(0)

    def __del__(self):
        try:
            self.free()
        except Exception:
            pass


def _take_write_plan(ctx, wp: WritePlanC) -> "WritePlan":
    try:
        n = wp.n
        b = wp.bodies
        offs = np.ctypeslib.as_array(C.cast(b.offsets, C.POINTER(C.c_uint64)), (n + 1,)).copy()
        st = _arr(b.status, n, np.int32)
        src = _arr(b.source, n, np.uint8)
        total = int(offs[-1]) if n else 0
        raw = C.string_at(b.bytes, total) if total else b""
        return WritePlan(pair_index=_arr(wp.pair_index, n, np.uint32), kind=_arr(wp.kind, n, np.uint8),
                         noop=_arr(wp.noop, n, np.uint8),
                         bodies=[None if st[i] != OK else raw[int(offs[i]):int(offs[i + 1])] for i in range(n)],
                         source=src, n_host=int(b.n_host), rv=_take_rv_splice(ctx, b), tgt=_take_targets(ctx, b))
    finally:
        _lib.gpudiff_write_plan_release(ctx, C.byref(wp))


class ObjectStore:

    def __init__(self, engine: "Engine", max_slots: int, space_bytes: int, max_events: int,
                 device_encode: bool = False):
        self.engine = engine
        self.device_encode = device_encode
        h = C.c_void_p()
        _chk(_lib.gpudiff_store_create_ex(engine.ctx, max_slots, space_bytes, max_events,
                                          STORE_DEVICE_ENCODE if device_encode else 0, C.byref(h)),
             "gpudiff_store_create_ex")
        self.h = h
        self._keep = [None, None]
        self._k = 0

    @staticmethod
    def events(items):
        n = len(items)
        arr = (Event * max(n, 1))()
        keep = []
        for i, it in enumerate(items):
            slot, new, old = it[0], it[1], it[2]
            nb = to_json_bytes(new)
            cn = C.create_string_buffer(nb, len(nb)) if nb else C.create_string_buffer(1)
            keep.append(cn)
            arr[i].slot = slot
            arr[i].pair_id = it[3] if len(it) > 3 else i
            arr[i].cluster_id = it[4] if len(it) > 4 else 0
# ... 894 lines not shown
```

Baseline: 1.417 billion pairs/s.

## Build compact per-pair device image at append time for shape-equal pairs

At dbatch append, a scan plus a build kernel copy, for pairs whose spec (and optionally status) shape is equal, only the value chunks into a separate compact device image, dropping the duplicated key/meta chunks. The pair descriptors are repacked to point at this image, so the diff kernel streams fewer bytes per pair. The image is placed at an offset from the pool that is stored in the summary buffer. The cost is an extra image allocation the size of the pool, a scan and copy pass at append time, and a new image-aware descriptor encoding that the kernels must decode correctly.

```diff
diff --git a/include/gpudiff.h b/include/gpudiff.h
--- a/include/gpudiff.h
+++ b/include/gpudiff.h
@@ -52,6 +52,7 @@
 
 #define GPUDIFF_OPT_TIMING 0x1u
 #define GPUDIFF_OPT_K2_ROWS 0x40u
+#define GPUDIFF_OPT_NO_IMAGE 0x20u
 #define GPUDIFF_OPT_ARENA_SHIFT 21u
 #define GPUDIFF_OPT_DEVICE_ENCODE 0x2000000u
 #define GPUDIFF_OPT_PATH_STRINGS 0x8000000u
@@ -59,7 +60,7 @@
 #define GPUDIFF_OPT_PATH_VALUES 0x80000000u
 #define GPUDIFF_OPT_KNOWN                                                                                         \
     (GPUDIFF_OPT_TIMING | (0xFu << GPUDIFF_OPT_ARENA_SHIFT) | GPUDIFF_OPT_DEVICE_ENCODE | GPUDIFF_OPT_PATH_STRINGS | \
-     GPUDIFF_OPT_SMALL_PASS | GPUDIFF_OPT_PATH_VALUES | GPUDIFF_OPT_K2_ROWS)
+     GPUDIFF_OPT_SMALL_PASS | GPUDIFF_OPT_PATH_VALUES | GPUDIFF_OPT_K2_ROWS | GPUDIFF_OPT_NO_IMAGE)
 
 #define GPUDIFF_SMALL_PASS_MAX_PAIRS 4096u
 #define GPUDIFF_SMALL_PASS_MAX_PATHS 32768u
@@ -194,6 +195,13 @@
 int gpudiff_dbatch_create_view(gpudiff_ctx* ctx, const gpudiff_dbatch* base, gpudiff_dbatch** out);
 int gpudiff_dbatch_append(gpudiff_ctx* ctx, gpudiff_dbatch* db, const gpudiff_hbatch* hb);
 int gpudiff_dbatch_reset(gpudiff_ctx* ctx, gpudiff_dbatch* db);
+int gpudiff_dbatch_set_image_capacity(gpudiff_dbatch* db, uint64_t bytes);
+typedef struct gpudiff_image_stats {
+    uint64_t bytes_used;
+    uint64_t capacity;
+    uint64_t pairs;
+} gpudiff_image_stats;
+int gpudiff_dbatch_image_stats(const gpudiff_dbatch* db, gpudiff_image_stats* st);
 int gpudiff_dbatch_stats_get(const gpudiff_dbatch* db, gpudiff_batch_stats* st);
 int gpudiff_dbatch_device_view(const gpudiff_dbatch* db, gpudiff_device_view* v);
 #define GPUDIFF_EXPORT_COUNTS 0u
@@ -214,6 +222,7 @@
 int gpudiff_shard_lpt(const uint64_t* weights, uint32_t n_clusters, uint32_t world, int32_t* owner);
 int gpudiff_rows_stream_bytes(const gpudiff_pair_row* rows, size_t n, uint64_t* out);
 int gpudiff_rows_read_bytes(const gpudiff_pair_row* rows, size_t n, uint64_t* out);
+int gpudiff_rows_image_read_bytes(const gpudiff_pair_row* rows, size_t n, uint64_t* out);
 
 int gpudiff_diff(gpudiff_ctx* ctx, gpudiff_dbatch* db, gpudiff_ticket* ticket);
 int gpudiff_wait(gpudiff_ctx* ctx, gpudiff_ticket ticket, gpudiff_result* res);
diff --git a/include/gpudiff_format.h b/include/gpudiff_format.h
--- a/include/gpudiff_format.h
+++ b/include/gpudiff_format.h
@@ -26,6 +26,7 @@
 #define GPUDIFF_OBJ_FRESH 0x4u
 #define GPUDIFF_OBJ_SPEC_KEYS_EQ 0x8u
 #define GPUDIFF_OBJ_SPEC_SHAPE_EQ 0x10u
+#define GPUDIFF_OBJ_STAT_SHAPE_EQ 0x20u
 #define GPUDIFF_TAB_INDEX 0x8000000000000000ull
 #define GPUDIFF_TAB_NONE 0xFFFFFFFFu
 GPUDIFF_HD static inline uint64_t gpudiff_tab_bytes(uint32_t n, uint64_t key_bytes) {
@@ -106,6 +107,8 @@
 #define GPUDIFF_PD_SIZE_MAX 0x7FFFFu
 #define GPUDIFF_PD_ESCAPE 0xFFFFFFFFu
 #define GPUDIFF_PD_SHAPE_L 0x40000u
+#define GPUDIFF_PD_IMAGE 0x80u
+#define GPUDIFF_PD_IMAGE_SPEC_MAX 0x3FFFFu
 
 typedef struct gpudiff_pair_desc {
     uint32_t w[4];
@@ -206,9 +209,13 @@
     const uint32_t f1 = (uint32_t)(zw >> GPUDIFF_PD_SIZE_BITS) & GPUDIFF_PD_SIZE_MAX;
     const int eq = (bits & GPUDIFF_PD_SPEC_EQ) != 0u;
     const int shape = eq && f1 >= GPUDIFF_PD_SHAPE_L && (w2 & GPUDIFF_PD_SIZE_MAX) < GPUDIFF_PD_SHAPE_L;
-    return gpudiff_pair_geom_of((uint64_t)w0 << 7, (uint64_t)w1 << 7, seg_a, eq ? seg_a : f1 << 4,
-                                ((w3 >> (2u * GPUDIFF_PD_SIZE_BITS - 32u)) & GPUDIFF_PD_SIZE_MAX) << 4, bits,
-                                eq ? (shape ? f1 & (GPUDIFF_PD_SHAPE_L - 1u) : f1) : 0u, shape);
+    const int image = eq && f1 == GPUDIFF_PD_SIZE_MAX && (w2 & GPUDIFF_PD_SIZE_MAX) < GPUDIFF_PD_IMAGE_SPEC_MAX;
+    gpudiff_pair_geom g =
+        gpudiff_pair_geom_of((uint64_t)w0 << 7, (uint64_t)w1 << 7, seg_a, eq ? seg_a : f1 << 4,
+                             ((w3 >> (2u * GPUDIFF_PD_SIZE_BITS - 32u)) & GPUDIFF_PD_SIZE_MAX) << 4, bits,
+                             (eq && !image) ? (shape ? f1 & (GPUDIFF_PD_SHAPE_L - 1u) : f1) : 0u, shape && !image);
+    if (image) g.bits |= GPUDIFF_PD_IMAGE;
+    return g;
 }
 
 GPUDIFF_HD static inline uint64_t gpudiff_pair_stream_bytes(const gpudiff_pair_row* r) {
@@ -218,6 +225,59 @@
     return sizeof(gpudiff_pair_desc) + 32ull * ((uint64_t)g.n1 + g.n2);
 }
 
+GPUDIFF_HD static inline int gpudiff_pair_image_parts(const gpudiff_pair_row* r, uint32_t* spec, uint32_t* stat) {
+    const uint32_t need = GPUDIFF_OBJ_SPEC_KEYS_EQ | GPUDIFF_OBJ_SPEC_SHAPE_EQ;
+    *spec = *stat = 0u;
+    if ((r->flags_a | r->flags_b) & GPUDIFF_OBJ_DECODE_ERR) return 0;
+    if (r->spec_l_a != r->spec_l_b || r->spec_ar_a != r->spec_ar_b || (r->flags_b & need) != need) return 0;
+    {
+        const gpudiff_pair_desc d = gpudiff_pair_desc_pack(r);
+        const uint64_t s = 16ull * (((uint64_t)r->spec_l_a + 1u) >> 1) + r->spec_ar_a;
+        const int stat_sz = (r->flags_b & GPUDIFF_OBJ_HAS_STATUS) && r->stat_l_a == r->stat_l_b &&
+                            r->stat_ar_a == r->stat_ar_b;
+        if (gpudiff_pair_desc_is_escape(d.w[3]) || (s >> 4) >= GPUDIFF_PD_IMAGE_SPEC_MAX) return 0;
+        *spec = (uint32_t)s;
+        if (stat_sz)
+            *stat = (r->flags_b & GPUDIFF_OBJ_STAT_SHAPE_EQ)
+                        ? (uint32_t)(16ull * (((uint64_t)r->stat_l_a + 1u) >> 1) + r->stat_ar_a)
+                        : (uint32_t)gpudiff_seg_bytes(r->stat_l_a, r->stat_ar_a);
+    }
+    return 1;
+}
+GPUDIFF_HD static inline uint64_t gpudiff_pair_image_side(const gpudiff_pair_row* r) {
+    uint32_t s, t;
+    if (!gpudiff_pair_image_parts(r, &s, &t)) return 0u;
+    return ((uint64_t)s + t + (GPUDIFF_BLOB_ALIGN - 1u)) & ~(uint64_t)(GPUDIFF_BLOB_ALIGN - 1u);
+}
+GPUDIFF_HD static inline gpudiff_pair_desc gpudiff_pair_desc_pack_image(const gpudiff_pair_row* r, uint64_t img_a,
+                                                                        uint64_t img_b) {
+    gpudiff_pair_desc d;
+    uint32_t s, t;
+    if (!gpudiff_pair_image_parts(r, &s, &t) || ((img_a | img_b) & (GPUDIFF_BLOB_ALIGN - 1u)) != 0u ||
+        (img_a >> 7) > 0xFFFFFFFFull || (img_b >> 7) > 0xFFFFFFFFull) {
+        d.w[0] = d.w[1] = d.w[2] = d.w[3] = GPUDIFF_PD_ESCAPE;
+        return d;
+    }
+    {
+        const uint64_t zw = (uint64_t)(s >> 4) | ((uint64_t)GPUDIFF_PD_SIZE_MAX << GPUDIFF_PD_SIZE_BITS) |
+                            ((uint64_t)(t >> 4) << (2u * GPUDIFF_PD_SIZE_BITS)) |
+                            ((uint64_t)gpudiff_pair_row_bits(r) << (3u * GPUDIFF_PD_SIZE_BITS));
+        d.w[0] = (uint32_t)(img_a >> 7);
+        d.w[1] = (uint32_t)(img_b >> 7);
+        d.w[2] = (uint32_t)zw;
+        d.w[3] = (uint32_t)(zw >> 32);
+    }
+    return d;
+}
+GPUDIFF_HD static inline uint64_t gpudiff_pair_image_bytes(const gpudiff_pair_row* r) {
+    const gpudiff_pair_desc d = gpudiff_pair_desc_pack_image(r, 0u, 0u);
+    if (gpudiff_pair_desc_is_escape(d.w[3])) return gpudiff_pair_stream_bytes(r);
+    {
+        const gpudiff_pair_geom g = gpudiff_pair_desc_unpack(d.w[0], d.w[1], d.w[2], d.w[3]);
+        return sizeof(gpudiff_pair_desc) + 32ull * ((uint64_t)g.n1 + g.n2);
+    }
+}
+
 GPUDIFF_HD static inline uint32_t gpudiff_meta(uint32_t tag, uint32_t len) { return (len << 3) | tag; }
 GPUDIFF_HD static inline uint32_t gpudiff_meta_tag(uint32_t m) { return m & 7u; }
 GPUDIFF_HD static inline uint32_t gpudiff_meta_len(uint32_t m) { return m >> 3; }
diff --git a/integration/go/gpudiff/gpudiff.go b/integration/go/gpudiff/gpudiff.go
--- a/integration/go/gpudiff/gpudiff.go
+++ b/integration/go/gpudiff/gpudiff.go
@@ -915,7 +915,18 @@
 const (
 	ObjSpecKeysEq  = uint32(C.GPUDIFF_OBJ_SPEC_KEYS_EQ)
 	ObjSpecShapeEq = uint32(C.GPUDIFF_OBJ_SPEC_SHAPE_EQ)
+	ObjStatShapeEq = uint32(C.GPUDIFF_OBJ_STAT_SHAPE_EQ)
 )
+
+const OptNoImage = uint32(C.GPUDIFF_OPT_NO_IMAGE)
+
+func RowsImageReadBytes(rows unsafe.Pointer, n int) (uint64, error) {
+	var out C.uint64_t
+	if err := errOf(C.gpudiff_rows_image_read_bytes((*C.gpudiff_pair_row)(rows), C.size_t(n), &out)); err != nil {
+		return 0, err
+	}
+	return uint64(out), nil
+}
 
 func RowsReadBytes(rows unsafe.Pointer, n int) (uint64, error) {
 	var out C.uint64_t
diff --git a/kcp_amd/csrc/api.cpp b/kcp_amd/csrc/api.cpp
--- a/kcp_amd/csrc/api.cpp
+++ b/kcp_amd/csrc/api.cpp
@@ -74,6 +74,7 @@
     b.rows = d->rows;
     b.desc = (d->desc_gen == d->rows_gen && !(c->flags & GPUDIFF_OPT_K2_ROWS)) ? d->desc : nullptr;
     b.pool = d->pool;
+    b.image = b.desc ? d->image : nullptr;
     b.pair_ids = d->pair_ids;
     b.n_pairs = (uint32_t)d->n_pairs;
     b.flags = d->flags;
@@ -422,6 +423,8 @@
     d->rows_gen = b->rows_gen;
     d->desc = b->desc;
     d->desc_gen = b->desc_gen;
+    d->image = b->image;
+    d->image_cap = b->image_cap;
 }
 
 static int alloc_outputs(gpudiff_dbatch* d) {
@@ -431,7 +434,7 @@
     const uint64_t ntiles = 4 * (np / 4096 + 2);
     uint4* cc = nullptr;
     if ((rc = dalloc(&d->flags, np)) || (rc = dalloc(&d->caps, np)) || (rc = dalloc(&cc, nchunks)) ||
-        (rc = dalloc(&d->summary, kSummaryWords)) || (rc = dalloc(&d->spec_ids, np)) || (rc = dalloc(&d->status_ids, np)) ||
+        (rc = dalloc(&d->summary, kSummaryAlloc)) || (rc = dalloc(&d->spec_ids, np)) || (rc = dalloc(&d->status_ids, np)) ||
         (rc = dalloc(&d->dirty_ids, np)) || (rc = dalloc(&d->dirty_idx, np)) || (rc = dalloc(&d->scratch_off, np)) ||
         (rc = dalloc(&d->path_count, np)) || (rc = dalloc(&d->path_off, np + 1)) ||
         (rc = dalloc(&d->path_src, np)) || (rc = dalloc(&d->path_cnt, np)) || (rc = dalloc(&d->nbits, np)) ||
@@ -443,6 +446,53 @@
     }
     d->chunk_counts = cc;
     if (hipEventCreateWithFlags(&d->done, hipEventDisableTiming) != hipSuccess) return GPUDIFF_E_DEVICE;
+    return GPUDIFF_OK;
+}
+
+static bool image_ready(gpudiff_ctx* c, gpudiff_dbatch* d, uint64_t n) {
+    if ((c->flags & GPUDIFF_OPT_NO_IMAGE) || d->image_off || d->pool_borrowed) return false;
+    if (!d->image) {
+        const uint64_t cap = (d->image_cap_req == ~0ull ? d->pool_cap : d->image_cap_req) & ~127ull;
+        if (!cap || hipMalloc((void**)&d->image, cap) != hipSuccess) {
+            (void)hipGetLastError();
+            d->image = nullptr;
+            d->image_off = true;
+            return false;
+        }
+        d->image_cap = cap;
+    }
+    if (n > d->image_scan_n) {
+        if (d->image_scan) {
+            if (hipStreamSynchronize(c->stream) != hipSuccess) return false;
+            (void)hipFree(d->image_scan);
+            d->image_scan = nullptr;
+            d->image_scan_n = 0;
+        }
+        const uint64_t want = std::max<uint64_t>(n, 1u << 16);
+        if (hipMalloc((void**)&d->image_scan, image_scan_words((uint32_t)want) * sizeof(uint64_t)) != hipSuccess) {
+            (void)hipGetLastError();
+            d->image_scan = nullptr;
+            return false;
+        }
+        d->image_scan_n = want;
+    }
+    return true;
+}
+
+int gpudiff_dbatch_set_image_capacity(gpudiff_dbatch* d, uint64_t bytes) {
+    if (!d || d->base) return GPUDIFF_E_INVAL;
+    if (d->n_pairs || d->image) return GPUDIFF_E_STATE;
+    d->image_cap_req = bytes;
+    d->image_off = bytes < 128u;
+    return GPUDIFF_OK;
+}
+
+int gpudiff_dbatch_image_stats(const gpudiff_dbatch* d, gpudiff_image_stats* st) {
+    if (!d || !st) return GPUDIFF_E_INVAL;
+    if (d->base) d = d->base;
+    st->bytes_used = d->image_used;
+    st->capacity = d->image ? d->image_cap : 0u;
+    st->pairs = d->image_pairs;
     return GPUDIFF_OK;
 }
 
@@ -460,10 +510,21 @@
                           c->stream));
     if (hb->used) HIPCHK(hipEventRecord(hb->used, c->stream));
     HIPCHK(launch_rebase(c->stream, d->rows, begin, end, base, d->pair_ids, d->desc));
+    const bool imaging = image_ready(c, d, hb->n);
+    if (imaging)
+        HIPCHK(launch_image_build(c->stream, d->rows, begin, end, d->image_scan, d->image_cursor, d->image_cap, d->pool,
+                                  d->image, d->desc));
     uint64_t cb = 0, vb = 0;
     for (size_t i = 0; i < hb->n; i++) {
         const gpudiff_pair_row& r = hb->rows[i];
         cb += pair_compare_bytes(r);
+        if (imaging) {
+            gpudiff_pair_row rr = r;
+            rr.off_a += base, rr.off_b += base;
+            const uint64_t ib = 2u * gpudiff_pair_image_side(&rr);
+            if (ib && d->image_cursor + ib <= d->image_cap) d->image_used = d->image_cursor + ib, d->image_pairs++;
+            d->image_cursor += ib;
+        }
         if ((r.flags_a | r.flags_b) & GPUDIFF_OBJ_DECODE_ERR) continue;
         vb += blob_value_bytes(hb->pool + r.off_a, r.spec_l_a, r.spec_ar_a, r.stat_l_a) +
               blob_value_bytes(hb->pool + r.off_b, r.spec_l_b, r.spec_ar_b, r.stat_l_b);
@@ -485,6 +546,7 @@
     if (rc) return rc;
     HIPCHK(hipStreamSynchronize(c->stream));
     d->pool_used = d->n_pairs = d->leaves = d->compare_bytes = d->value_bytes = d->size_hint_bytes = 0;
+    d->image_cursor = d->image_used = d->image_pairs = 0;
     d->ticket = 0;
     d->rows_gen++;
     return GPUDIFF_OK;
@@ -553,7 +615,7 @@
     if (!d->summary_alt) {
         const uint64_t np = std::max<uint64_t>(d->max_pairs, 1);
         uint32_t *a = nullptr, *b = nullptr, *sm = nullptr;
-        if ((rc = dalloc(&a, np)) || (rc = dalloc(&b, np)) || (rc = dalloc(&sm, kSummaryWords))) {
+        if ((rc = dalloc(&a, np)) || (rc = dalloc(&b, np)) || (rc = dalloc(&sm, kSummaryAlloc))) {
             for (uint32_t* p : {a, b, sm})
                 if (p) (void)hipFree(p);
             return rc;
@@ -598,6 +660,14 @@
         r.flags_b &= ~GPUDIFF_OBJ_SPEC_SHAPE_EQ;
         sum += gpudiff_pair_stream_bytes(&r);
     }
+    *out = sum;
+    return GPUDIFF_OK;
+}
+
+int gpudiff_rows_image_read_bytes(const gpudiff_pair_row* rows, size_t n, uint64_t* out) {
+    if ((n && !rows) || !out) return GPUDIFF_E_INVAL;
+    uint64_t sum = 0;
+    for (size_t i = 0; i < n; i++) sum += gpudiff_pair_image_bytes(&rows[i]);
     *out = sum;
     return GPUDIFF_OK;
 }
@@ -1057,6 +1127,7 @@
             gpudiff_hbatch_free(c, hb);
             return rc;
         }
+        (void)gpudiff_dbatch_set_image_capacity(d, 0);
     }
     d->pool_used = d->n_pairs = d->leaves = d->compare_bytes = d->value_bytes = d->size_hint_bytes = 0;
     if ((rc = gpudiff_dbatch_append(c, d, hb)) || (rc = gpudiff_diff(c, d, ticket))) {
diff --git a/kcp_amd/csrc/encoder.cpp b/kcp_amd/csrc/encoder.cpp
--- a/kcp_amd/csrc/encoder.cpp
+++ b/kcp_amd/csrc/encoder.cpp
@@ -289,6 +289,11 @@
     bool shape_eq = keys_eq;
     for (size_t i = 0; shape_eq && i < fa->spec.size(); i++) shape_eq = fa->spec[i].meta == fb->spec[i].meta;
     if (shape_eq) row.flags_b |= GPUDIFF_OBJ_SPEC_SHAPE_EQ;
+    const bool both_status = (fa->flags & fb->flags & GPUDIFF_OBJ_HAS_STATUS) != 0u;
+    bool stat_eq = both_status && !fa->stat.empty() && fa->stat.size() == fb->stat.size();
+    for (size_t i = 0; stat_eq && i < fa->stat.size(); i++)
+        stat_eq = (uint32_t)fa->stat[i].h == (uint32_t)fb->stat[i].h && fa->stat[i].meta == fb->stat[i].meta;
+    if (stat_eq) row.flags_b |= GPUDIFF_OBJ_STAT_SHAPE_EQ;
 }
 
 void PairEncoder::encode_nodes(const Node* a, const Node* b, uint32_t pair_id, uint32_t cluster_id,
diff --git a/kcp_amd/csrc/engine.h b/kcp_amd/csrc/engine.h
--- a/kcp_amd/csrc/engine.h
+++ b/kcp_amd/csrc/engine.h
@@ -117,6 +117,11 @@
     uint64_t rows_gen = 0;
     uint4* desc = nullptr;
     uint64_t desc_gen = ~0ull;
+    uint8_t* image = nullptr;
+    uint64_t image_cap = 0, image_cap_req = ~0ull, image_cursor = 0, image_used = 0, image_pairs = 0;
+    bool image_off = false;
+    uint64_t* image_scan = nullptr;
+    uint64_t image_scan_n = 0;
     uint8_t* small_image = nullptr;
     bool small_pending = false;
     WaitedMark waited;
@@ -259,7 +264,10 @@
 
 inline void dfree_all(gpudiff_dbatch* d) {
     if (d->pool && !d->pool_borrowed) (void)hipFree(d->pool);
-    if (d->base) d->rows = nullptr, d->pair_ids = nullptr, d->desc = nullptr;
+    if (d->base) d->rows = nullptr, d->pair_ids = nullptr, d->desc = nullptr, d->image = nullptr;
+    if (d->image) (void)hipFree(d->image);
+    if (d->image_scan) (void)hipFree(d->image_scan);
+    d->image = nullptr, d->image_scan = nullptr;
     void* ps[] = {d->rows, d->pair_ids, d->desc, d->flags, d->caps, d->chunk_counts, d->summary, d->spec_ids,
                   d->status_ids, d->dirty_ids, d->dirty_idx, d->scratch_off, d->path_count, d->path_off,
                   d->tile_sums, d->path_src, d->path_cnt, d->arena_h, d->arena_k,
diff --git a/kcp_amd/csrc/kernels.h b/kcp_amd/csrc/kernels.h
--- a/kcp_amd/csrc/kernels.h
+++ b/kcp_amd/csrc/kernels.h
@@ -13,6 +13,7 @@
     const gpudiff_pair_row* rows;
     const uint4* desc;
     const uint8_t* pool;
+    const uint8_t* image = nullptr;
     const uint32_t* pair_ids;
     uint32_t n_pairs;
     uint8_t* flags;
@@ -64,12 +65,17 @@
 };
 
 constexpr uint32_t kK2TailCounters = 8, kSummaryWords = 8 + 2 * kK2TailCounters;
+constexpr uint32_t kSummaryImageDelta = 32, kSummaryAlloc = kSummaryImageDelta + 2;
+static_assert(kSummaryImageDelta % 32 == 0 && kSummaryImageDelta >= kSummaryWords, "the delta: an aligned u64, its own line");
 constexpr uint32_t kK2TailQuarters = 2;
 
 uint32_t k2_grid_waves(const DiffBuffers& b, uint32_t nchunks);
 
 hipError_t launch_rebase(hipStream_t s, gpudiff_pair_row* rows, uint32_t begin, uint32_t end, uint64_t base,
                          uint32_t* pair_ids, uint4* desc);
+inline uint64_t image_scan_words(uint32_t n) { return 2ull * n + 2u + (n + 1023u) / 1024u; }
+hipError_t launch_image_build(hipStream_t s, const gpudiff_pair_row* rows, uint32_t begin, uint32_t end, uint64_t* scan,
+                              uint64_t used, uint64_t cap, const uint8_t* pool, uint8_t* image, uint4* desc);
 struct BlobMove {
     uint64_t src, dst, bytes;
 };
diff --git a/kcp_amd/csrc/kernels.hip b/kcp_amd/csrc/kernels.hip
--- a/kcp_amd/csrc/kernels.hip
+++ b/kcp_amd/csrc/kernels.hip
@@ -4,6 +4,7 @@
 #include "../../include/gpudiff.h"
 #include "join_dev.h"
 #include "kernels.h"
+#include "scan64.h"
 #include "stream_paths.h"
 #include "wave_dev.h"
 #include "xxh64.h"
@@ -114,12 +115,18 @@
     uint32_t hole[64];
 };
 
+template <bool IMG>
 __device__ uint32_t stream_region(const RegionView& A, const RegionView& B, uint64_t seg, const uint32_t* ent,
                                   uint32_t c, uint32_t g0, uint32_t hole, uint8_t region_bit,
                                   uint64_t* __restrict__ out_h, uint8_t* __restrict__ out_k, uint32_t out_base,
                                   uint32_t lane, bool* weq_all) {
     const uint32_t nc = 4u * c;
-    const uint32_t e = lane < nc ? sp_entry_unhole(ent[lane >> 2] - sp_entry(g0, 0u), hole) : 0u;
+    uint32_t e = 0u;
+    if (lane < nc) {
+        const uint32_t e0 = ent[lane >> 2] - sp_entry(g0, 0u);
+        if (IMG && hole == kSpHoleImage) e = sp_entry_unimage(e0, A.L);
+        else e = sp_entry_unhole(e0, hole);
+    }
     const bool cand = lane < nc && ((sp_entry_dwords(e) >> (lane & 3u)) & 1u);
     const uint64_t b = sp_entry_byte(e, lane & 3u);
     const SpWhere w = sp_classify(b, A.L);
@@ -179,6 +186,7 @@
     return popc64(um);
 }
 
+template <bool IMG>
 __device__ uint32_t stream_pair(const gpudiff_pair_row& r, uint32_t f, const uint8_t* pool, uint64_t mask,
                                 uint64_t* out_h, uint8_t* out_k, uint32_t base, uint32_t lane, uint32_t* noop,
                                 const StreamLog* log, uint32_t k, bool log_ok, uint32_t* n_stream) {
@@ -191,8 +199,8 @@
         const uint32_t g0 = uni(log->first[k]);
         uint32_t got = kSpRefuse;
         if (c >= 1u && c <= kSpLogCap)
-            got = stream_region(A, B, seg_bytes(r.spec_l_a, r.spec_ar_a), log->ent[0][k], c, g0, uni(log->hole[k]), 0,
-                                out_h, out_k, base + n, lane, &spec_weq);
+            got = stream_region<IMG>(A, B, seg_bytes(r.spec_l_a, r.spec_ar_a), log->ent[0][k], c, g0, uni(log->hole[k]),
+                                     0, out_h, out_k, base + n, lane, &spec_weq);
         if (got == kSpRefuse) got = join_region<true>(A, B, 0, out_h, out_k, base + n, lane, &spec_weq);
         else (*n_stream)++;
         n += got;
@@ -203,9 +211,12 @@
         const uint32_t c = log_ok ? uni(log->cnt[1][k]) : 0u;
         const uint32_t g0 = uni(log->first[k]) + uni(log->n1[k]);
         uint32_t got = kSpRefuse;
+        uint32_t th = 0u;
+        if constexpr (IMG)
+            th = (uni(log->hole[k]) == kSpHoleImage && (r.flags_b & GPUDIFF_OBJ_STAT_SHAPE_EQ)) ? kSpHoleImage : 0u;
         if (c >= 1u && c <= kSpLogCap)
-            got = stream_region(A, B, seg_bytes(r.stat_l_a, r.stat_ar_a), log->ent[1][k], c, g0, 0u,
-                                GPUDIFF_PATH_REGION_STATUS, out_h, out_k, base + n, lane, &stat_weq);
+            got = stream_region<IMG>(A, B, seg_bytes(r.stat_l_a, r.stat_ar_a), log->ent[1][k], c, g0, th,
+                                     GPUDIFF_PATH_REGION_STATUS, out_h, out_k, base + n, lane, &stat_weq);
         if (got == kSpRefuse)
             got = join_region<true>(A, B, GPUDIFF_PATH_REGION_STATUS, out_h, out_k, base + n, lane, &stat_weq);
         else (*n_stream)++;
@@ -755,7 +766,8 @@
         uint32_t n1, n2, adj_a, adj_b;
         [[maybe_unused]] uint32_t hole = 0;
         [[maybe_unused]] uint32_t dbits = 0;
-        constexpr uint32_t kPdRow = 0x80u;
+        constexpr uint32_t kPdRow = 0x100u;
+        static_assert(kPdRow > GPUDIFF_PD_IMAGE, "the unpack's bits and this one share dbits");
         if constexpr (DESC) {
             gpudiff_pair_geom g = gpudiff_pair_desc_unpack(dv.x, dv.y, dv.z, dv.w);
             if (valid && gpudiff_pair_desc_is_escape(dv.w)) {
@@ -773,6 +785,12 @@
             off_b += (uint64_t)g.adj_b - (uint64_t)g.adj_a;
             adj_a = adj_b = g.adj_a;
             hole = sp_hole_word(g.hs, g.hl);
+            if (dbits & GPUDIFF_PD_IMAGE) {
+                const uint64_t dl = __hip_atomic_load((const uint64_t*)(summary + kSummaryImageDelta), __ATOMIC_RELAXED,
+                                                      __HIP_MEMORY_SCOPE_WAVEFRONT);
+                off_a += dl, off_b += dl;
+                hole = kSpHoleImage;
+            }
         } else {
             off_a = ((uint64_t)v0.y << 32) | v0.x, off_b = ((uint64_t)v0.w << 32) | v0.z;
             err = valid && ((v3.x | v3.y) & GPUDIFF_OBJ_DECODE_ERR) != 0u;
@@ -893,7 +911,7 @@
                 if (fk & (F_JSPEC | F_JSTAT)) {
                     const gpudiff_pair_row r = rows[p0 + k];
                     if constexpr (HELP) pc = join_pair<true>(r, fk, pool, mask, ah, ak, src, lane, &nb);
-                    else pc = stream_pair(r, fk, pool, mask, ah, ak, src, lane, &nb, slog, k, total < (1u << 28), &n_stream);
+                    else pc = stream_pair<DESC>(r, fk, pool, mask, ah, ak, src, lane, &nb, slog, k, total < (1u << 28), &n_stream);
                 } else if (fk & F_SENT) {
                     const uint32_t fa = (uint32_t)__builtin_amdgcn_readlane((int)v3.x, (int)k);
                     nb = sentinel_noop_bits(fa);
@@ -1119,6 +1137,54 @@
     }
 }
 
+__global__ __launch_bounds__(256) void k_image_sizes(const gpudiff_pair_row* __restrict__ rows, uint32_t begin,
+                                                     uint32_t end, uint64_t* __restrict__ sizes) {
+    const uint32_t i = begin + blockIdx.x * blockDim.x + threadIdx.x;
+    if (i >= end) return;
+    const gpudiff_pair_row r = rows[i];
+    sizes[i - begin] = 2ull * gpudiff_pair_image_side(&r);
+}
+__global__ __launch_bounds__(256) void k_image_build(const gpudiff_pair_row* __restrict__ rows, uint32_t begin,
+                                                     uint32_t end, const uint64_t* __restrict__ offsets, uint64_t used,
+                                                     uint64_t cap, const uint8_t* __restrict__ pool,
+                                                     uint8_t* __restrict__ image, uint4* __restrict__ desc) {
+    const uint32_t lane = lane_id();
+    const uint32_t nw = (gridDim.x * blockDim.x) >> 6;
+    for (uint32_t p = begin + uni((blockIdx.x * blockDim.x + threadIdx.x) >> 6); p < end; p += nw) {
+        const gpudiff_pair_row r = rows[p];
+        uint32_t s = 0, t = 0;
+        if (!gpudiff_pair_image_parts(&r, &s, &t)) continue;
+        const uint64_t side = ((uint64_t)s + t + 127u) & ~127ull;
+        const uint64_t o = used + offsets[p - begin];
+        if (o + 2u * side > cap) continue;
+        const uint32_t nv = sp_image_vals(r.spec_l_a), drop = r.spec_l_a - nv;
+        const bool tsh = t != 0u && (r.flags_b & GPUDIFF_OBJ_STAT_SHAPE_EQ) != 0u;
+        const uint32_t nvt = sp_image_vals(r.stat_l_a), tdrop = tsh ? r.stat_l_a - nvt : 0u;
+        const uint32_t cs = s >> 4, ct = t >> 4, cside = (uint32_t)(side >> 4);
+        const uint32_t seg_c = (uint32_t)(seg_bytes(r.spec_l_a, r.spec_ar_a) >> 4);
+        for (uint32_t x = 0; x < 2u; x++) {
+            const u32x4* src = (const u32x4*)(pool + (x ? r.off_b : r.off_a));
+            u32x4* dst = (u32x4*)(image + o + x * side);
+            for (uint32_t q = lane; q < cside; q += 64u) {
+                u32x4 v = {0u, 0u, 0u, 0u};
+                if (q < cs) {
+                    v = src[q < nv ? q : q + drop];
+                    if ((r.spec_l_a & 1u) && q == nv - 1u) v.z = v.w = 0u;
+                } else if (q - cs < ct) {
+                    const uint32_t k = q - cs;
+                    v = src[seg_c + ((tsh && k >= nvt) ? k + tdrop : k)];
+                    if (tsh && (r.stat_l_a & 1u) && k == nvt - 1u) v.z = v.w = 0u;
+                }
+                dst[q] = v;
+            }
+        }
+        if (lane == 0) {
+            const gpudiff_pair_desc d = gpudiff_pair_desc_pack_image(&r, o, o + side);
+            if (!gpudiff_pair_desc_is_escape(d.w[3])) desc[p] = make_uint4(d.w[0], d.w[1], d.w[2], d.w[3]);
+        }
+    }
+}
+
 static inline uint32_t grid_for(uint64_t waves_wanted, uint32_t cap_blocks) {
     uint64_t blocks = (waves_wanted + 3) / 4;
     if (blocks < 1) blocks = 1;
@@ -1135,6 +1201,23 @@
 }
 
 
+
+hipError_t launch_image_build(hipStream_t s, const gpudiff_pair_row* rows, uint32_t begin, uint32_t end, uint64_t* scan,
+                              uint64_t used, uint64_t cap, const uint8_t* pool, uint8_t* image, uint4* desc) {
+    if (end <= begin) return hipSuccess;
+    const uint32_t n = end - begin;
+    uint64_t* const sizes = scan;
+    uint64_t* const offsets = scan + n;
+    uint64_t* const tiles = offsets + n + 1u;
+    uint64_t* const total = tiles + scan64_tiles(n);
+    k_image_sizes<<<(n + 255u) / 256u, 256, 0, s>>>(rows, begin, end, sizes);
+    hipError_t e = hipGetLastError();
+    if (e != hipSuccess) return e;
+    if ((e = launch_scan64_sums(s, sizes, n, tiles, total)) != hipSuccess) return e;
+    if ((e = launch_scan64_offsets(s, sizes, n, tiles, offsets)) != hipSuccess) return e;
+    k_image_build<<<grid_for(n, kPersistBlocks), 256, 0, s>>>(rows, begin, end, offsets, used, cap, pool, image, desc);
+    return hipGetLastError();
+}
 
 hipError_t launch_move_blobs(hipStream_t s, const uint8_t* src, uint8_t* dst, const BlobMove* moves, uint32_t n) {
     if (!n) return hipSuccess;
@@ -1197,9 +1280,10 @@
 }
 
 __global__ __launch_bounds__(256) void k_pass_reset(uint32_t* __restrict__ summary, uint32_t nwords,
-                                                    uint4* __restrict__ cc, uint32_t ncc) {
+                                                    uint4* __restrict__ cc, uint32_t ncc, uint64_t image_delta) {
     const uint32_t i = blockIdx.x * 256u + threadIdx.x;
     if (summary && i < nwords) summary[i] = 0u;
+    if (summary && i == nwords) *(uint64_t*)(summary + kSummaryImageDelta) = image_delta;
     for (uint32_t j = i; j < ncc; j += gridDim.x * 256u) cc[j] = make_uint4(0u, 0u, 0u, 0u);
 }
 
@@ -1295,8 +1379,8 @@
     {
         const uint32_t z0 = sub ? 0u : lpt ? (((nch << sub) - lpt) >> sub) : nch - tail;
         const uint32_t ncc = nch - z0;
-        k_pass_reset<<<std::max(1u, std::min(1024u, (ncc + 255u) / 256u)), 256, 0, s>>>(b.summary, kSummaryWords,
-                                                                                        cc + z0, ncc);
+        k_pass_reset<<<std::max(1u, std::min(1024u, (ncc + 255u) / 256u)), 256, 0, s>>>(
+            b.summary, kSummaryWords, cc + z0, ncc, b.image ? (uint64_t)((uintptr_t)b.image - (uintptr_t)b.pool) : 0ull);
     }
     const uint32_t sub_arg = sub | (tq << 8) | (lpt ? kK2LptRounds << 20 | 1u << 22 : 0u);
     k2_kernel(v)<<<grid, 256, 0, s>>>(b.rows, b.pool, b.n_pairs, b.flags, b.caps, cc, 0u, nch, b.arena_h, b.arena_k, 0u,
diff --git a/kcp_amd/csrc/stream_paths.h b/kcp_amd/csrc/stream_paths.h
--- a/kcp_amd/csrc/stream_paths.h
+++ b/kcp_amd/csrc/stream_paths.h
@@ -26,6 +26,16 @@
 GD_SP_HD inline uint32_t sp_hole_bytes(uint32_t w) { return (w >> 16) << 7; }
 GD_SP_HD inline uint32_t sp_entry_unhole(uint32_t e, uint32_t w) {
     return e + ((e >> 4) >= sp_hole_start(w) ? sp_entry(sp_hole_chunks(w), 0u) : 0u);
+}
+
+constexpr uint32_t kSpHoleImage = 0xFFFFFFFFu;
+GD_SP_HD inline uint32_t sp_image_vals(uint32_t L) { return (L + 1u) >> 1; }
+GD_SP_HD inline uint32_t sp_image_chunk(uint32_t k, uint32_t L) { return k + (k >= sp_image_vals(L) ? L - sp_image_vals(L) : 0u); }
+GD_SP_HD inline uint32_t sp_image_of_chunk(uint32_t c, uint32_t L) {
+    return c < sp_image_vals(L) ? c : c >= L ? c - (L - sp_image_vals(L)) : kSpRefuse;
+}
+GD_SP_HD inline uint32_t sp_entry_unimage(uint32_t e, uint32_t L) {
+    return e + ((e >> 4) >= sp_image_vals(L) ? sp_entry(L - sp_image_vals(L), 0u) : 0u);
 }
 
 GD_SP_HD inline uint32_t sp_meta_arena(uint32_t m) {
diff --git a/kcp_amd/gpudiff.py b/kcp_amd/gpudiff.py
--- a/kcp_amd/gpudiff.py
+++ b/kcp_amd/gpudiff.py
@@ -26,6 +26,7 @@
 OPT_DEVICE_ENCODE = 0x2000000
 OPT_PATH_STRINGS = 0x8000000
 OPT_PATH_VALUES = 0x80000000
+OPT_NO_IMAGE = 0x20
 OPT_K2_ROWS = 0x40
 OPT_ARENA_SHIFT = 21
 OPT_SMALL_PASS = 0x20000000
@@ -36,6 +37,7 @@
 PATH_HASH_BITS = 32
 OBJ_HAS_STATUS, OBJ_DECODE_ERR, OBJ_FRESH, OBJ_SEED_SHIFT = 0x1, 0x2, 0x4, 8
 OBJ_SPEC_KEYS_EQ = 0x8
+OBJ_STAT_SHAPE_EQ = 0x20
 OBJ_SPEC_SHAPE_EQ = 0x10
 STORE_DEVICE_ENCODE = 0x1
 EXPORT_COUNTS, EXPORT_SPEC_IDS, EXPORT_STATUS_IDS, EXPORT_DIRTY_IDS, EXPORT_FLAGS = range(5)
@@ -330,6 +332,10 @@
 class BatchStats(C.Structure):
     _fields_ = [("n_pairs", C.c_uint64), ("pool_bytes", C.c_uint64), ("total_leaves", C.c_uint64),
                 ("compare_bytes", C.c_uint64), ("value_bytes", C.c_uint64)]
+
+
+class ImageStats(C.Structure):
+    _fields_ = [("bytes_used", C.c_uint64), ("capacity", C.c_uint64), ("pairs", C.c_uint64)]
 
 
 class Timings(C.Structure):
@@ -364,6 +370,9 @@
     ("gpudiff_shard_lpt", C.c_int, [C.c_void_p, C.c_uint32, C.c_uint32, C.c_void_p]),
     ("gpudiff_rows_stream_bytes", C.c_int, [C.c_void_p, C.c_size_t, C.POINTER(C.c_uint64)]),
     ("gpudiff_rows_read_bytes", C.c_int, [C.c_void_p, C.c_size_t, C.POINTER(C.c_uint64)]),
+    ("gpudiff_rows_image_read_bytes", C.c_int, [C.c_void_p, C.c_size_t, C.POINTER(C.c_uint64)]),
+    ("gpudiff_dbatch_set_image_capacity", C.c_int, [_P, C.c_uint64]),
+    ("gpudiff_dbatch_image_stats", C.c_int, [_P, C.POINTER(ImageStats)]),
     ("gpudiff_diff", C.c_int, [_P, _P, C.POINTER(C.c_uint64)]),
     ("gpudiff_wait", C.c_int, [_P, C.c_uint64, C.POINTER(Result)]),
     ("gpudiff_result_release", None, [_P, C.POINTER(Result)]),
@@ -547,6 +556,13 @@
     return int(out.value)
 
 
+def image_read_bytes(rows: np.ndarray) -> int:
+    rows = np.ascontiguousarray(rows, dtype=ROW_DTYPE)
+    out = C.c_uint64()
+    _chk(_lib.gpudiff_rows_image_read_bytes(rows.ctypes.data, rows.size, C.byref(out)), "gpudiff_rows_image_read_bytes")
+    return int(out.value)
+
+
 def shard_lpt(weights, world: int) -> np.ndarray:
     w = np.ascontiguousarray(weights, dtype=np.uint64)
     owner = np.zeros(w.size, dtype=np.int32)
@@ -708,6 +724,14 @@
 
     def reset(self):
         _chk(_lib.gpudiff_dbatch_reset(self.engine.ctx, self.h), "gpudiff_dbatch_reset")
+
+    def set_image_capacity(self, nbytes: int):
+        _chk(_lib.gpudiff_dbatch_set_image_capacity(self.h, nbytes), "gpudiff_dbatch_set_image_capacity")
+
+    def image_stats(self) -> ImageStats:
+        st = ImageStats()
+        _chk(_lib.gpudiff_dbatch_image_stats(self.h, C.byref(st)), "gpudiff_dbatch_image_stats")
+        return st
 
     def stats(self) -> BatchStats:
         st = BatchStats()
```

New measurement: 1.484 billion pairs/s, median of 6. 1.05x the previous value.
